# ForeverFancy/GVFDiffusion

Measured on AMD Instinct MI355X. Metric: 4D frames/sec (800x800x24f, 256k Gaussians) + DiT denoise steps/sec, higher is better.
Workload: dtype f32; 1 GPU; BASELINE configs[1]: single-GPU HIP rasteriser, one 4D sample per step = 24 frames x 800x800, 262144 Gaussians + per-frame deltas (fused activations), SH degree 2, mip 2D filter, white bg; gaussians=262144, resolution=800, sh_degree=2, parallelism=sample-sharded x1, samples_in_flight=2

## Files before the change

gvfdiffusion_amd/_lib.py:

```python
import ctypes
import os

_HERE = os.path.dirname(os.path.abspath(__file__))
LIB_PATH = os.path.join(_HERE, "libgvf_hip.so")

GVF_OK, GVF_EINVAL, GVF_ENOSPC, GVF_ELAUNCH = 0, -1, -2, -3
_ERR = {GVF_EINVAL: "GVF_EINVAL (bad argument)", GVF_ENOSPC: "GVF_ENOSPC (workspace too small)",
        GVF_ELAUNCH: "GVF_ELAUNCH (HIP launch/runtime failure)"}

RAST_MODE_MIP, RAST_MODE_DILATE = 0, 1
RAST_BIN_AUTO, RAST_BIN_RADIX, RAST_BIN_BUCKET = 0, 1, 2


class GvfError(RuntimeError):
    pass


class GvfRastFrame(ctypes.Structure):
    _fields_ = [("viewmatrix", ctypes.c_float * 16), ("projmatrix", ctypes.c_float * 16),
                ("campos", ctypes.c_float * 3), ("tanfovx", ctypes.c_float), ("tanfovy", ctypes.c_float),
                ("delta_index", ctypes.c_int32), ("reserved", ctypes.c_int32 * 2)]


class GvfRastSettings(ctypes.Structure):
    _fields_ = [("image_height", ctypes.c_int32), ("image_width", ctypes.c_int32), ("sh_degree", ctypes.c_int32),
                ("mode", ctypes.c_int32), ("kernel_size", ctypes.c_float), ("scale_modifier", ctypes.c_float),
                ("bg", ctypes.c_float * 3), ("prefiltered", ctypes.c_int32), ("debug", ctypes.c_int32),
                ("upstream_binning", ctypes.c_int32), ("bin_algo", ctypes.c_int32)]


class GvfGaussianActivation(ctypes.Structure):
    _fields_ = [("aabb", ctypes.c_float * 6), ("scale_bias", ctypes.c_float), ("opacity_bias", ctypes.c_float),
                ("min_kernel_size", ctypes.c_float), ("scaling_activation", ctypes.c_int32)]


class GvfRastPlan(ctypes.Structure):
    _fields_ = [(n, ctypes.c_int32) for n in ("bucket", "shared", "index_count", "morton", "slot_mode", "rec_gather", "wave_frames",
                                              "order_tiles", "upstream_binning", "n_slices", "layout", "gx", "gy", "ntiles", "nb", "nseg")] + \
               [(n, ctypes.c_int32 * 2) for n in ("pre_grid", "wf_grid", "bin_grid", "binx_grid")] + \
               [(n, ctypes.c_int32) for n in ("scan_blocks", "clear_blocks", "pre_lds_bytes", "wf_lds_bytes")]


_vp, _i, _i64, _sz, _f = ctypes.c_void_p, ctypes.c_int, ctypes.c_int64, ctypes.c_size_t, ctypes.c_float

SIGNATURES = {
    "gvf_version": (ctypes.c_char_p, []),
    "gvf_rast_workspace_bytes": (_i, [_i, _i, _i, _i, _i64, ctypes.POINTER(_sz)]),
    "gvf_rast_forward": (_i, [ctypes.POINTER(GvfRastSettings), ctypes.POINTER(GvfRastFrame), _i, _i,
                              _vp, _vp, _vp, _vp, _vp, _vp, _vp, _vp, _vp, _sz, _i64, _vp, _vp, _vp, _vp, _vp, _vp]),
    "gvf_rast_forward_batched": (_i, [ctypes.POINTER(GvfRastSettings), ctypes.POINTER(GvfRastFrame), _i,
                                      ctypes.POINTER(GvfGaussianActivation), _i, _i, _vp, _vp, _vp, _vp, _vp, _vp,
                                      _i, _vp, _sz, _i64, _vp, _vp, _vp, _vp, _vp, _vp]),
    "gvf_rast_forward_batched_u8": (_i, [ctypes.POINTER(GvfRastSettings), ctypes.POINTER(GvfRastFrame), _i,
                                         ctypes.POINTER(GvfGaussianActivation), _i, _i, _vp, _vp, _vp, _vp, _vp, _vp,
                                         _i, _vp, _sz, _i64, _vp, _vp, _vp]),
    "gvf_rast_backward_scratch_bytes": (_i, [_i, ctypes.POINTER(_sz)]),
    "gvf_rast_backward": (_i, [ctypes.POINTER(GvfRastSettings), ctypes.POINTER(GvfRastFrame), _i, _i,
                               _vp, _vp, _vp, _vp, _vp, _vp, _vp, _vp, _vp, _sz, _i64, _vp, _vp, _vp, _vp, _sz,
                               _vp, _vp, _vp, _vp, _vp, _vp, _vp, _vp, _vp]),
    "gvf_rast_backward_batched_scratch_bytes": (_i, [_i, _i, ctypes.POINTER(_sz)]),
    "gvf_rast_backward_batched": (_i, [ctypes.POINTER(GvfRastSettings), ctypes.POINTER(GvfRastFrame), _i,
                                       ctypes.POINTER(GvfGaussianActivation), _i, _i, _vp, _vp, _vp, _vp, _vp, _vp, _i,
                                       _vp, _sz, _i64, _vp, _vp, _vp, _vp, _sz, _vp, _vp, _vp, _vp, _vp, _vp, _vp]),
    "gvf_gaussian_activate": (_i, [ctypes.POINTER(GvfGaussianActivation), _i, _i, _vp, _vp, _vp, _vp, _vp, _vp,
                                   _vp, _vp, _vp, _vp, _vp, _vp]),
    "gvf_rgb_to_u8": (_i, [_vp, _vp, _i64, _vp]),
    "gvf_rast_sort_class_counts": (_i, [_vp, _sz, _i, _i, _i, _i, _i64, ctypes.POINTER(ctypes.c_uint32), _vp]),
    "gvf_rast_call_plan": (_i, [ctypes.POINTER(GvfRastSettings), ctypes.POINTER(GvfRastFrame), _i, _i, _i, _i, _i, _i, _i, _i, _i, _i64,
                                ctypes.POINTER(GvfRastPlan)]),
    "gvf_rast_bin_record_bytes": (_i, [ctypes.POINTER(GvfRastSettings), ctypes.POINTER(_i)]),
    "gvf_rast_slice_groups": (_i, [ctypes.POINTER(GvfRastFrame), _i, _i, _i, ctypes.POINTER(ctypes.c_int32), ctypes.POINTER(_i)]),
    "gvf_rast_profile_enable": (_i, [_i]),
    "gvf_rast_profile_read": (_i, [ctypes.POINTER(_f), ctypes.POINTER(_i)]),
    "gvf_rast_shared_activation_calls": (_i64, []),
    "gvf_sort_tmp_bytes": (_sz, [_i64]),
    "gvf_sort_pairs_u64": (_i, [_vp, _vp, _vp, _vp, _i64, _i, _vp, _sz, _vp]),
    "gvf_tile_sort_u64": (_i, [_vp, _vp, _i, _vp, _vp, _vp]),
}

_LIB = None


def register(signatures):
    SIGNATURES.update(signatures)
    if _LIB is not None:
        _bind(_LIB, signatures)


def _bind(lib, signatures):
    for name, (res, args) in signatures.items():
        fn = getattr(lib, name)
        fn.restype = res
        fn.argtypes = args


def lib():
    global _LIB
    if _LIB is None:
        if not os.path.exists(LIB_PATH):
            raise GvfError(f"{LIB_PATH} is missing: build it with `python -m gvfdiffusion_amd._build` "
                           "(hipcc, gfx950). There is no CPU fallback.")
        stamp = LIB_PATH + ".srchash"
        if os.path.exists(stamp) and os.environ.get("GVF_ALLOW_STALE_LIB") != "1":
            from . import _build
            if open(stamp).read().strip() != _build.source_hash():
                raise GvfError(f"{LIB_PATH} was built from different sources than the ones in csrc/ and include/: "
                               "rebuild with `python -m gvfdiffusion_amd._build`")
        import torch
        l = ctypes.CDLL(os.environ.get("GVF_LIB") or LIB_PATH)
        _bind(l, SIGNATURES)
        _LIB = l
    return _LIB


def check(rc: int, what: str):
    if rc != GVF_OK:
        raise GvfError(f"{what} failed: {_ERR.get(rc, rc)}")


def ptr(t):
    return None if t is None else ctypes.c_void_p(t.data_ptr())


def current_stream(device):
    import torch
    return ctypes.c_void_p(torch.cuda.current_stream(device).cuda_stream)


def require_cuda(*tensors):
    for t in tensors:
        if t is not None and not t.is_cuda:
            raise GvfError("gvfdiffusion_amd operators run on the MI355X only: got a CPU tensor "
                           "(there is no CPU fallback; the CPU oracle lives in oracle/ for tests)")
```

gvfdiffusion_amd/csrc/rast.hip:

```cpp
#include <atomic>
#include <cstdlib>
#include <vector>
#include "rast_common.h"
#include "gvf_sort.h"

namespace {

constexpr int PROF_MAX_CALLS = 256;
constexpr int PROF_EVENTS = GVF_RAST_NSTAGES + 1;
struct Profiler {
    bool on = false;
    std::atomic<int> calls{0};
    hipEvent_t ev[PROF_MAX_CALLS][PROF_EVENTS];
};
Profiler g_prof;
const hipEvent_t* prof_take_slot() {
    const int slot = g_prof.on ? g_prof.calls.fetch_add(1) : -1;
    return slot >= 0 && slot < PROF_MAX_CALLS ? g_prof.ev[slot] : nullptr;
}

std::atomic<long long> g_shared_calls{0};

bool switch_on(const char* name) {
    const char* v = getenv(name);
    return !(v && v[0] == '0');
}
RastSwitches switches_from_env() {
    RastSwitches sw;
    sw.shared_act = switch_on("GVF_RAST_SHARED_ACT");
    sw.slot_order = switch_on("GVF_RAST_SLOT_ORDER");
    sw.pre_wave_frames = switch_on("GVF_RAST_PRE_WAVE_FRAMES");
    sw.blend_order = switch_on("GVF_RAST_BLEND_ORDER");
    sw.bin_rec8 = switch_on("GVF_RAST_BIN_REC8");
    return sw;
}

int check_shape(const GvfRastSettings& st, int F, int P, int64_t max_rendered) {
    if (st.image_height <= 0 || st.image_width <= 0 || P < 0 || F <= 0 || max_rendered < 0 || max_rendered > 0xFFFFFFFFll) return GVF_EINVAL;
    if (st.sh_degree < 0 || st.sh_degree > 3) return GVF_EINVAL;
    if (st.mode != GVF_RAST_MODE_MIP && st.mode != GVF_RAST_MODE_DILATE) return GVF_EINVAL;
    return GVF_OK;
}

struct RastOutputs { float* color; float* alpha; float* depth; unsigned char* u8; };

int check_call(const RastCall& c, const RastOutputs& out, const void* workspace) {
    const GvfRastSettings& st = *c.st;
    if (check_shape(st, c.F, c.P, c.max_rendered) != GVF_OK) return GVF_EINVAL;
    if ((out.color == nullptr) == (out.u8 == nullptr) || !c.out_num_rendered || !c.frames_host || !workspace) return GVF_EINVAL;
    if (c.P > 0 && c.colors_precomp == nullptr) {
        if (c.sh == nullptr || c.M < (st.sh_degree + 1) * (st.sh_degree + 1) || c.M > MAX_SH_COEFFS) return GVF_EINVAL;
    }
    if ((((uintptr_t)c.sh) & 15) != 0 || (((uintptr_t)workspace) & 255) != 0) return GVF_EINVAL;
    return GVF_OK;
}

PlanInputs plan_inputs(const RastCall& c) {
    PlanInputs in;
    in.F = c.F; in.P = c.P; in.M = c.M; in.fused = c.fused;
    in.has_sh = c.sh != nullptr; in.has_colors_precomp = c.colors_precomp != nullptr; in.has_cov3D_precomp = c.cov3D_precomp != nullptr;
    in.has_delta = c.delta != nullptr; in.has_subpixel_offset = c.subpixel_offset != nullptr;
    in.max_rendered = c.max_rendered;
    return in;
}

int run_pipeline(const RastCall& c, void* workspace, size_t workspace_bytes, const RastOutputs& out, hipStream_t stream) {
    int rc = check_call(c, out, workspace);
    if (rc != GVF_OK) return rc;
    (void)hipGetLastError();
    const GvfRastSettings& st = *c.st;
    const Workspace w = carve(workspace, workspace_bytes, c.P, c.F, st.image_height, st.image_width, c.max_rendered);
    if (!w.ok) return GVF_ENOSPC;
    const RastPlan plan = plan_call(st, c.frames_host, plan_inputs(c), switches_from_env());
    const hipEvent_t* marks = prof_take_slot();
    if ((rc = upload_frames(stream, c, plan, w)) != GVF_OK) return rc;

    if (c.P == 0) {
        if (hipMemsetAsync(c.out_num_rendered, 0, sizeof(uint32_t) * c.F, stream) != hipSuccess) return GVF_ELAUNCH;
    } else {
        uint64_t* keys = w.keys;
        uint32_t* vals = nullptr;
        if (plan.shared) g_shared_calls.fetch_add(1, std::memory_order_relaxed);
        rc = plan.bucket ? front_end_bucket(stream, c, plan, w, marks) : front_end_radix(stream, c, plan, w, marks, &keys, &vals);
        if (rc != GVF_OK) return rc;
        if (c.max_rendered > 0 &&
            (rc = launch_tile_sort(stream, w.ranges, keys, vals, w.ids, w.cls, (uint32_t)plan.nseg, plan.bucket ? 2 : 1)) != GVF_OK)
            return rc;
    }
    rc = launch_blend(stream, st, c.P, c.F, w.ranges, w.ids, w.splats, c.subpixel_offset, out.color, out.alpha, out.depth, out.u8,
                      plan.slot_mode ? w.order_alt : nullptr, plan.order_tiles ? w.cursor : nullptr, marks != nullptr ? marks[6] : nullptr);
    if (rc != GVF_OK) return rc;
    prof_mark(stream, marks, 7);
    return GVF_OK;
}

int check_batched(const GvfRastSettings* st, const GvfRastFrame* frames_host, int F, const GvfGaussianActivation* act, int P,
                  const float* xyz_raw, const float* features_dc, const float* scaling_raw, const float* rotation_raw,
                  const float* opacity_raw, const float* delta, int n_delta) {
    if (!st || !frames_host || !act || F <= 0) return GVF_EINVAL;
    if (P > 0 && (!xyz_raw || !features_dc || !scaling_raw || !rotation_raw || !opacity_raw)) return GVF_EINVAL;
    if (act->scaling_activation != 0 && act->scaling_activation != 1) return GVF_EINVAL;
    for (int f = 0; f < F; ++f) {
        int di = frames_host[f].delta_index;
        if (di >= 0 && (delta == nullptr || di >= n_delta)) return GVF_EINVAL;
    }
    return GVF_OK;
}

}


Workspace gvf_rast::carve(void* ws, size_t bytes, int P, int F, int H, int W, int64_t max_rendered) {
    Workspace w;
    GvfCarver c(ws, bytes);
    const int nb = (P + PRE_THREADS - 1) / PRE_THREADS;
    const int ntiles = ((W + TILE - 1) / TILE) * ((H + TILE - 1) / TILE);
    const size_t FP = (size_t)F * (size_t)(P > 0 ? P : 1);
    const size_t D = (size_t)(max_rendered > 0 ? max_rendered : 1);
    w.frames = c.take<GvfRastFrame>(F);
    w.splats = c.take<float4>(4 * FP);
    w.tiles_touched = c.take<uint32_t>(FP);
    w.radii = c.take<int32_t>(FP);
    w.block_sums = c.take<uint32_t>((size_t)F * (nb > 0 ? nb : 1));
    w.frame_base = c.take<uint32_t>(F + 1);
    w.total = c.take<uint32_t>(1);
    w.keys = c.take<uint64_t>(D);
    w.keys_alt = c.take<uint64_t>(D);
    w.vals = c.take<uint32_t>(D);
    w.vals_alt = c.take<uint32_t>(D);
    w.ids = c.take<uint32_t>(D);
    w.ranges = c.take<uint2>((size_t)F * ntiles);
    w.cls = c.take<uint32_t>(2 + 2 * (size_t)F * ntiles);
    w.tile_count = c.take<uint32_t>((size_t)F * ntiles);
    w.cursor = c.take<uint32_t>((size_t)F * ntiles);
    w.partial = c.take<uint32_t>(((size_t)F * ntiles + SCAN_CHUNK - 1) / SCAN_CHUNK + 1);
    const size_t Pp = (size_t)(P > 0 ? P : 1);
    w.order = c.take<uint32_t>(Pp);
    w.order_alt = c.take<uint32_t>(Pp);
    w.mhist = c.take<uint32_t>(MORTON_BINS);
    w.mm = c.take<uint32_t>(8);
    w.binrec = c.take<uint4>(FP);
    w.sort_tmp_bytes = gvf_sort_tmp_bytes((int64_t)D);
    w.sort_tmp = c.take<char>(w.sort_tmp_bytes);
    w.bytes = gvf_align_up(c.off, 256);
    w.ok = c.ok;
    return w;
}

extern "C" int gvf_rast_workspace_bytes(int P, int F, int H, int W, int64_t max_rendered, size_t* bytes) {
    if (!bytes || P < 0 || F <= 0 || H <= 0 || W <= 0 || max_rendered < 0) return GVF_EINVAL;
    Workspace w = carve(nullptr, (size_t)-1, P, F, H, W, max_rendered);
    *bytes = w.bytes + 256;
    (void)tile_sort_set_lds_limit();
    return GVF_OK;
}

extern "C" int gvf_rast_forward(const GvfRastSettings* st, const GvfRastFrame* frame_host, int P, int M,
                                const float* means3D, const float* shs, const float* colors_precomp,
                                const float* opacities, const float* scales, const float* rotations,
                                const float* cov3D_precomp, const float* subpixel_offset, void* workspace,
                                size_t workspace_bytes, int64_t max_rendered, float* out_color, float* out_alpha,
                                float* out_depth, int32_t* out_radii, uint32_t* out_num_rendered, void* stream) {
    if (!st || !frame_host) return GVF_EINVAL;
    if (P > 0) {
        if (!means3D || !opacities) return GVF_EINVAL;
        if ((shs == nullptr) == (colors_precomp == nullptr)) return GVF_EINVAL;
        const bool have_sr = scales != nullptr && rotations != nullptr;
        if (have_sr == (cov3D_precomp != nullptr)) return GVF_EINVAL;
    }
    const RastCall c = {st, frame_host, 1, P, M, false, nullptr, means3D, scales, rotations, opacities, shs, colors_precomp, cov3D_precomp,
                        nullptr, 0, subpixel_offset, max_rendered, out_radii, out_num_rendered};
    return run_pipeline(c, workspace, workspace_bytes, {out_color, out_alpha, out_depth, nullptr}, (hipStream_t)stream);
}

extern "C" int gvf_rast_forward_batched(const GvfRastSettings* st, const GvfRastFrame* frames_host, int F,
                                        const GvfGaussianActivation* act, int P, int M, const float* xyz_raw,
                                        const float* features_dc, const float* scaling_raw,
                                        const float* rotation_raw, const float* opacity_raw, const float* delta,
                                        int n_delta, void* workspace, size_t workspace_bytes,
                                        int64_t max_rendered, float* out_color, float* out_alpha, float* out_depth,
                                        int32_t* out_radii, uint32_t* out_num_rendered, void* stream) {
    const int rc = check_batched(st, frames_host, F, act, P, xyz_raw, features_dc, scaling_raw, rotation_raw, opacity_raw, delta, n_delta);
    if (rc != GVF_OK) return rc;
    const RastCall c = {st, frames_host, F, P, M, true, act, xyz_raw, scaling_raw, rotation_raw, opacity_raw, features_dc, nullptr, nullptr,
                        delta, n_delta, nullptr, max_rendered, out_radii, out_num_rendered};
    return run_pipeline(c, workspace, workspace_bytes, {out_color, out_alpha, out_depth, nullptr}, (hipStream_t)stream);
}

extern "C" int gvf_rast_forward_batched_u8(const GvfRastSettings* st, const GvfRastFrame* frames_host, int F,
                                           const GvfGaussianActivation* act, int P, int M, const float* xyz_raw,
                                           const float* features_dc, const float* scaling_raw,
                                           const float* rotation_raw, const float* opacity_raw, const float* delta,
                                           int n_delta, void* workspace, size_t workspace_bytes,
                                           int64_t max_rendered, uint8_t* out_rgb_u8, uint32_t* out_num_rendered, void* stream) {
    if (!out_rgb_u8) return GVF_EINVAL;
    const int rc = check_batched(st, frames_host, F, act, P, xyz_raw, features_dc, scaling_raw, rotation_raw, opacity_raw, delta, n_delta);
    if (rc != GVF_OK) return rc;
    const RastCall c = {st, frames_host, F, P, M, true, act, xyz_raw, scaling_raw, rotation_raw, opacity_raw, features_dc, nullptr, nullptr,
                        delta, n_delta, nullptr, max_rendered, nullptr, out_num_rendered};
    return run_pipeline(c, workspace, workspace_bytes, {nullptr, nullptr, nullptr, out_rgb_u8}, (hipStream_t)stream);
}

extern "C" int gvf_rast_call_plan(const GvfRastSettings* st, const GvfRastFrame* frames_host, int F, int P, int M, int fused, int has_sh,
                                  int has_colors_precomp, int has_cov3D_precomp, int has_delta, int has_subpixel_offset,
                                  int64_t max_rendered, GvfRastPlan* out) {
    if (!st || !frames_host || !out || M < 0) return GVF_EINVAL;
    if (check_shape(*st, F, P, max_rendered) != GVF_OK) return GVF_EINVAL;
    PlanInputs in;
    in.F = F; in.P = P; in.M = M; in.fused = fused != 0;
    in.has_sh = has_sh != 0; in.has_colors_precomp = has_colors_precomp != 0; in.has_cov3D_precomp = has_cov3D_precomp != 0;
    in.has_delta = has_delta != 0; in.has_subpixel_offset = has_subpixel_offset != 0;
    in.max_rendered = max_rendered;
    *out = plan_call(*st, frames_host, in, switches_from_env());
    return GVF_OK;
}

extern "C" int gvf_rast_bin_record_bytes(const GvfRastSettings* st, int* bytes) {
    if (!st || !bytes) return GVF_EINVAL;
    if (check_shape(*st, 1, 0, 0) != GVF_OK) return GVF_EINVAL;
    const GvfRastFrame frame = {};
    PlanInputs in = {};
    in.F = 1;
    *bytes = plan_call(*st, &frame, in, switches_from_env()).rec8 ? 8 : 16;
    return GVF_OK;
}

extern "C" int gvf_rast_slice_groups(const GvfRastFrame* frames_host, int F, int has_delta, int max_slices, int32_t* table_host,
                                     int* n_slices) {
    if (!frames_host || !table_host || !n_slices || F <= 0) return GVF_EINVAL;
    std::vector<int32_t> slices, frame_slice;
    if (!group_slices(frames_host, F, has_delta != 0, max_slices, slices, frame_slice)) return GVF_ENOSPC;
    const std::vector<int32_t> tab = slice_table(slices, frame_slice);
    for (size_t k = 0; k < tab.size(); ++k) table_host[k] = tab[k];
    *n_slices = (int)slices.size();
    return GVF_OK;
}

extern "C" int gvf_rast_profile_enable(int on) {
    if (on && !g_prof.on) {
        for (int c = 0; c < PROF_MAX_CALLS; ++c)
            for (int k = 0; k < PROF_EVENTS; ++k)
                if (hipEventCreate(&g_prof.ev[c][k]) != hipSuccess) return GVF_ELAUNCH;
        g_prof.on = true;
        g_prof.calls = 0;
    } else if (!on && g_prof.on) {
        for (int c = 0; c < PROF_MAX_CALLS; ++c)
            for (int k = 0; k < PROF_EVENTS; ++k) (void)hipEventDestroy(g_prof.ev[c][k]);
        g_prof.on = false;
        g_prof.calls = 0;
    }
    return GVF_OK;
}

extern "C" int64_t gvf_rast_shared_activation_calls(void) { return (int64_t)g_shared_calls.load(std::memory_order_relaxed); }

extern "C" int gvf_rast_profile_read(float* ms_sum, int* calls) {
    if (!ms_sum || !calls) return GVF_EINVAL;
    for (int k = 0; k < GVF_RAST_NSTAGES; ++k) ms_sum[k] = 0.f;
    *calls = 0;
    if (!g_prof.on) return GVF_OK;
    const int n_calls = g_prof.calls.load() < PROF_MAX_CALLS ? g_prof.calls.load() : PROF_MAX_CALLS;
    for (int c = 0; c < n_calls; ++c) {
        if (hipEventSynchronize(g_prof.ev[c][PROF_EVENTS - 1]) != hipSuccess) return GVF_ELAUNCH;
        for (int k = 0; k < GVF_RAST_NSTAGES; ++k) {
            float ms = 0.f;
            if (hipEventElapsedTime(&ms, g_prof.ev[c][k], g_prof.ev[c][k + 1]) != hipSuccess) return GVF_ELAUNCH;
            ms_sum[k] += ms;
        }
    }
    *calls = n_calls;
    g_prof.calls = 0;
    return GVF_OK;
}

extern "C" int gvf_rast_sort_class_counts(const void* workspace, size_t workspace_bytes, int P, int F, int H, int W, int64_t max_rendered,
                                          uint32_t* counts_host, void* stream) {
    if (!workspace || !counts_host || H <= 0 || W <= 0 || P < 0 || F <= 0 || max_rendered < 0) return GVF_EINVAL;
    if ((((uintptr_t)workspace) & 255) != 0) return GVF_EINVAL;
    Workspace w = carve(const_cast<void*>(workspace), workspace_bytes, P, F, H, W, max_rendered);
    if (!w.ok) return GVF_ENOSPC;
    if (hipMemcpyAsync(counts_host, w.cls, 2 * sizeof(uint32_t), hipMemcpyDeviceToHost, (hipStream_t)stream) != hipSuccess) return GVF_ELAUNCH;
    if (hipStreamSynchronize((hipStream_t)stream) != hipSuccess) return GVF_ELAUNCH;
    return GVF_OK;
}

extern "C" const char* gvf_version(void) { return "gvf_hip 0.1.0 gfx950"; }
```

gvfdiffusion_amd/csrc/rast_blend.hip:

```cpp
#include "rast_common.h"

namespace {


__global__ __launch_bounds__(1024) void blend_order_kernel(const uint2* __restrict__ ranges, int ntiles, uint32_t* __restrict__ order) {
    __shared__ uint32_t hist[64];
    const int f = blockIdx.x, t = threadIdx.x;
    const uint2* r = ranges + (size_t)f * ntiles;
    if (t < 64) hist[t] = 0u;
    __syncthreads();
    for (int tile = t; tile < ntiles; tile += 1024) {
        const uint32_t n = r[tile].y - r[tile].x;
        atomicAdd(&hist[63u - min(63u, n >> 5)], 1u);
    }
    __syncthreads();
    const bool reorder = hist[0] != 0u;
    __syncthreads();
    if (!reorder) {
        for (int tile = t; tile < ntiles; tile += 1024) order[(size_t)f * ntiles + tile] = (uint32_t)tile;
        return;
    }
    if (t == 0) {
        uint32_t run = 0u;
        for (int c = 0; c < 64; ++c) { const uint32_t h = hist[c]; hist[c] = run; run += h; }
    }
    __syncthreads();
    for (int tile = t; tile < ntiles; tile += 1024) {
        const uint32_t n = r[tile].y - r[tile].x;
        order[(size_t)f * ntiles + atomicAdd(&hist[63u - min(63u, n >> 5)], 1u)] = (uint32_t)tile;
    }
}

#ifdef BLEND_TIMING
__device__ unsigned long long* g_blend_buf;
__device__ unsigned long long g_blend_cap;
extern "C" int gvf_debug_blend_timing(unsigned long long* device_buf, unsigned long long rows) {
    if (hipMemcpyToSymbol(HIP_SYMBOL(g_blend_buf), &device_buf, sizeof(device_buf)) != hipSuccess) return 1;
    if (hipMemcpyToSymbol(HIP_SYMBOL(g_blend_cap), &rows, sizeof(rows)) != hipSuccess) return 1;
    return 0;
}
#define BT_DECL unsigned long long bt_acc[12] = {}; unsigned long long bt_last = __builtin_amdgcn_s_memtime(); const unsigned long long bt_first = bt_last;
#define BT(i) do { const unsigned long long n_ = __builtin_amdgcn_s_memtime(); bt_acc[i] += n_ - bt_last; bt_last = n_; } while (0)
#define BT_VMWAIT() asm volatile("s_waitcnt vmcnt(0)" ::: "memory")
#else
#define BT_DECL
#define BT(i) do { } while (0)
#define BT_VMWAIT() do { } while (0)
#endif

#ifdef BLEND_CONSUMED
__device__ unsigned long long g_blend_cons[4][5];
extern "C" int gvf_debug_blend_consumed(unsigned long long* out12, int reset) {
    if (out12 && hipMemcpyFromSymbol(out12, HIP_SYMBOL(g_blend_cons), sizeof(g_blend_cons)) != hipSuccess) return 1;
    if (reset) { unsigned long long z[20] = {}; if (hipMemcpyToSymbol(HIP_SYMBOL(g_blend_cons), z, sizeof(z)) != hipSuccess) return 1; }
    return 0;
}
#endif


template <bool DEPTH>
__global__ __launch_bounds__(BLEND_THREADS) void blend_kernel(
    int P, int H, int W, int gx, int gy, float bg0, float bg1, float bg2, const uint2* __restrict__ ranges,
    const uint32_t* __restrict__ point_list, const float4* __restrict__ splats,
    const float* __restrict__ subpixel_offset, float* __restrict__ out_color,
    float* __restrict__ out_alpha, float* __restrict__ out_depth,
    const uint32_t* __restrict__ tile_order ,
    const uint32_t* __restrict__ rec_of ,
    unsigned char* __restrict__ out_u8 ) {
    __shared__ float4 sA[BLEND_THREADS];
    __shared__ float4 sB[BLEND_THREADS];
    __shared__ float4 sC[BLEND_THREADS];
    __shared__ unsigned char sMask[BLEND_THREADS];
    __shared__ unsigned sList[4][BLEND_THREADS];

    const int t = threadIdx.x, lane = t & 63, wave = t >> 6;
    const int f = blockIdx.y;
    const int tile = tile_order != nullptr ? (int)tile_order[(size_t)f * gridDim.x + blockIdx.x] : (int)blockIdx.x;
    const int tx = tile % gx, ty = tile / gx;
    const int px = tx * TILE + (wave & 1) * 8 + (lane & 7), py = ty * TILE + (wave >> 1) * 8 + (lane >> 3);
    const bool inside = px < W && py < H;
    const size_t pid = (size_t)py * W + px;
    float pxf = (float)px, pyf = (float)py;
    if (subpixel_offset != nullptr && inside) { pxf += subpixel_offset[2 * pid]; pyf += subpixel_offset[2 * pid + 1]; }

    const uint2 rng = ranges[(size_t)f * gx * gy + tile];
    const size_t gbase = (size_t)f * P;
    const int rounds = (int)((rng.y - rng.x + BLEND_THREADS - 1) / BLEND_THREADS);
    int todo = (int)(rng.y - rng.x);
    const uint64_t lt_mask = (1ull << lane) - 1ull;

    const float pxr = pxf - (float)(tx * TILE), pyr = pyf - (float)(ty * TILE);
    unsigned long long done_m = __builtin_amdgcn_ballot_w64(!inside);
    float T = 1.0f, C0 = 0.f, C1 = 0.f, C2 = 0.f, Dacc = 0.f;

    BT_DECL
#ifdef BLEND_CONSUMED
    int rounds_done = rounds;
#endif
    for (int r = 0; r < rounds; ++r, todo -= BLEND_THREADS) {
        BT(6);
#ifdef BLEND_CONSUMED
        if (r > 0 && __syncthreads_and(done_m == ~0ull)) { rounds_done = r; break; }
#else
        if (r > 0 && __syncthreads_and(done_m == ~0ull)) break;
#endif
        BT(0);
#ifdef BLEND_TIMING
        uint32_t id_ = 0;
        if (t < todo) id_ = point_list[rng.x + (uint32_t)r * BLEND_THREADS + t];
        if (t < todo && rec_of != nullptr) id_ = rec_of[id_];
        BT_VMWAIT(); BT(1);
        float4 a_ = {}, b_ = {}, c_ = {};
        if (t < todo) { const float4* rec = splats + 4 * (gbase + id_); a_ = rec[0]; c_ = rec[2]; b_ = rec[1]; }
        BT_VMWAIT(); BT(2);
        bt_acc[7] += 1;
#endif
        if (t < todo) {
#ifdef BLEND_TIMING
            const float4 a = a_, b = b_, c = c_;
#else
            uint32_t id = point_list[rng.x + (uint32_t)r * BLEND_THREADS + t];
            if (rec_of != nullptr) id = rec_of[id];
            const float4* rec = splats + 4 * (gbase + id);
            const float4 a = rec[0];
            const float4 c = rec[2];
            const float4 b = rec[1];
#endif
            const SplatChol ch = splat_cholesky(a.x, a.y, a.z, a.w, b.x, (float)(tx * TILE), (float)(ty * TILE));
            sA[t] = make_float4(ch.l11, ch.l12, ch.l22, ch.c1);
            sB[t] = make_float4(ch.c2, ch.ok ? __builtin_amdgcn_logf(b.y) : -__builtin_inff(), b.z, b.w);
            sC[t] = make_float4(c.x, c.y, 0.f, 0.f);
            sMask[t] = (unsigned char)quadrant_mask(a.x, a.y, a.z, a.w, b.x, b.y, c.z, (float)(tx * TILE), (float)(ty * TILE), subpixel_offset != nullptr);
#ifdef BLEND_CONSUMED
            {
                const unsigned n_ = rng.y - rng.x;
                const int cls_ = n_ <= 2048u ? 0 : n_ <= 4096u ? 1 : n_ <= 16384u ? 2 : 3;
                if (sMask[t] == 0) atomicAdd(&g_blend_cons[cls_][3], 1ull);
                atomicAdd(&g_blend_cons[cls_][4], (unsigned long long)__popc((unsigned)sMask[t]));
            }
#endif
        }
        BT(3);
        __syncthreads();
        BT(4);
        const int cnt = min(BLEND_THREADS, todo);
        if (done_m == ~0ull) continue;
        int n_w = 0;
#pragma unroll
        for (int k = 0; k < BLEND_THREADS / GVF_WAVE; ++k) {
            const int idx = k * GVF_WAVE + lane;
            const bool hit = idx < cnt && ((sMask[idx] >> wave) & 1u);
            const uint64_t bal = __ballot(hit);
            if (hit) sList[wave][n_w + __popcll(bal & lt_mask)] = (unsigned)idx * 16u;
            n_w += __popcll(bal);
        }
        __builtin_amdgcn_wave_barrier();
        BT(5);
#ifdef BLEND_TIMING
        bt_acc[8] += n_w;
#endif
#define GVF_BLEND_STEP(J)                                                                              \
        {                                                                                              \
            const float4 a = *reinterpret_cast<const float4*>(reinterpret_cast<const unsigned char*>(sA) + (J));          \
            const float4 b = *reinterpret_cast<const float4*>(reinterpret_cast<const unsigned char*>(sB) + (J));          \
            const float4 c4_ = *reinterpret_cast<const float4*>(reinterpret_cast<const unsigned char*>(sC) + (J));        \
            const float2 c = DEPTH ? make_float2(c4_.x, c4_.y) : make_float2(c4_.x, 0.f);              \
            const float nlog = splat_neg_exponent(a.x, a.y, a.z, a.w, b.x, pxr, pyr, b.y);    \
            const float alpha = fminf(0.99f, __builtin_amdgcn_exp2f(-nlog));                           \
            const float w_raw = alpha * T;                                                             \
            const float test_T = T - w_raw;         \
                              \
            const unsigned long long ok_m = __builtin_amdgcn_ballot_w64(!(alpha < 1.0f / 255.0f)) & ~done_m;   \
            const unsigned long long stop_m = ok_m & __builtin_amdgcn_ballot_w64(test_T < 0.0001f);    \
            done_m |= stop_m;                                                                          \
            const bool acc = __builtin_amdgcn_inverse_ballot_w64(ok_m ^ stop_m);                       \
            const float wgt = acc ? w_raw : 0.0f;                                                      \
            C0 = __builtin_fmaf(b.z, wgt, C0);                                                         \
            C1 = __builtin_fmaf(b.w, wgt, C1);                                                         \
            C2 = __builtin_fmaf(c.x, wgt, C2);                                                         \
            if (DEPTH) Dacc = __builtin_fmaf(c.y, wgt, Dacc);                                          \
            T = acc ? test_T : T;                                                                      \
        }
        int jj = 0;
        for (; jj + 3 < n_w; jj += 4) {
            if (done_m == ~0ull) break;
            const unsigned j0 = sList[wave][jj], j1 = sList[wave][jj + 1], j2 = sList[wave][jj + 2], j3 = sList[wave][jj + 3];
            GVF_BLEND_STEP(j0)
            GVF_BLEND_STEP(j1)
            __builtin_amdgcn_sched_barrier(0);
            GVF_BLEND_STEP(j2)
            GVF_BLEND_STEP(j3)
        }
        for (; jj < n_w; ++jj) {
            if (done_m == ~0ull) break;
            const unsigned j0 = sList[wave][jj];
            GVF_BLEND_STEP(j0)
        }
#undef GVF_BLEND_STEP
    }
#ifdef BLEND_CONSUMED
    if (t == 0) {
        const unsigned n = rng.y - rng.x, used = min(n, (unsigned)rounds_done * BLEND_THREADS);
        const int cls = n <= 2048u ? 0 : n <= 4096u ? 1 : n <= 16384u ? 2 : 3;
        atomicAdd(&g_blend_cons[cls][0], 1ull); atomicAdd(&g_blend_cons[cls][1], (unsigned long long)n); atomicAdd(&g_blend_cons[cls][2], (unsigned long long)used);
    }
#endif
    if (inside) {
        const size_t hw = (size_t)H * W;
        const float r0 = __builtin_fmaf(T, bg0, C0), r1 = __builtin_fmaf(T, bg1, C1), r2 = __builtin_fmaf(T, bg2, C2);
        if (out_u8 != nullptr) {
            unsigned char* ob = out_u8 + (size_t)f * 3 * hw;
            ob[0 * hw + pid] = (unsigned char)(fminf(fmaxf(r0, 0.f), 1.f) * 255.0f);
            ob[1 * hw + pid] = (unsigned char)(fminf(fmaxf(r1, 0.f), 1.f) * 255.0f);
            ob[2 * hw + pid] = (unsigned char)(fminf(fmaxf(r2, 0.f), 1.f) * 255.0f);
        } else {
            float* oc = out_color + (size_t)f * 3 * hw;
            oc[0 * hw + pid] = r0;
            oc[1 * hw + pid] = r1;
            oc[2 * hw + pid] = r2;
        }
        if (out_alpha != nullptr) out_alpha[(size_t)f * hw + pid] = 1.0f - T;
        if (out_depth != nullptr) out_depth[(size_t)f * hw + pid] = Dacc;
    }
#ifdef BLEND_TIMING
    BT(6);
    BT_VMWAIT(); BT(11);
    bt_acc[9] = 1; bt_acc[10] = bt_last - bt_first;
    const unsigned long long wid = ((unsigned long long)f * gridDim.x + tile) * 4 + wave;
    if (lane == 0 && g_blend_buf != nullptr && wid < g_blend_cap)
        for (int i = 0; i < 12; ++i) g_blend_buf[wid * 12 + i] = bt_acc[i];
#endif
}

__global__ __launch_bounds__(256) void rgb_to_u8_kernel(const float4* __restrict__ src, uchar4* __restrict__ dst,
                                                        long long n4, const float* __restrict__ tail_src,
                                                        unsigned char* __restrict__ tail_dst, int tail) {
    for (long long i = blockIdx.x * (long long)blockDim.x + threadIdx.x; i < n4; i += (long long)gridDim.x * blockDim.x) {
        const float4 v = src[i];
        uchar4 o;
        o.x = (unsigned char)(fminf(fmaxf(v.x, 0.f), 1.f) * 255.0f);
        o.y = (unsigned char)(fminf(fmaxf(v.y, 0.f), 1.f) * 255.0f);
        o.z = (unsigned char)(fminf(fmaxf(v.z, 0.f), 1.f) * 255.0f);
        o.w = (unsigned char)(fminf(fmaxf(v.w, 0.f), 1.f) * 255.0f);
        dst[i] = o;
    }
    if (blockIdx.x == 0 && (int)threadIdx.x < tail)
        tail_dst[threadIdx.x] = (unsigned char)(fminf(fmaxf(tail_src[threadIdx.x], 0.f), 1.f) * 255.0f);
}

}

int gvf_rast::launch_blend(hipStream_t stream, const GvfRastSettings& st, int P, int F, const uint2* ranges, const uint32_t* point_list,
                           const float4* splats, const float* subpixel_offset, float* out_color, float* out_alpha, float* out_depth,
                           unsigned char* out_u8, const uint32_t* rec_of, uint32_t* tile_order, hipEvent_t ordered) {
    const int H = st.image_height, W = st.image_width;
    const int gx = (W + TILE - 1) / TILE, gy = (H + TILE - 1) / TILE, ntiles = gx * gy;
    if (tile_order != nullptr) hipLaunchKernelGGL(blend_order_kernel, dim3(F), dim3(1024), 0, stream, ranges, ntiles, tile_order);
    if (ordered != nullptr) (void)hipEventRecord(ordered, stream);
    hipLaunchKernelGGL(out_depth != nullptr ? blend_kernel<true> : blend_kernel<false>, dim3(ntiles, F), dim3(BLEND_THREADS), 0, stream, P, H, W,
                       gx, gy, st.bg[0], st.bg[1], st.bg[2], ranges, point_list, splats, subpixel_offset, out_color, out_alpha, out_depth,
                       tile_order, rec_of, out_u8);
    GVF_CHECK_LAUNCH();
    return GVF_OK;
}

extern "C" int gvf_rgb_to_u8(const float* rgb, uint8_t* out, int64_t n, void* stream) {
    if (n < 0) return GVF_EINVAL;
    if (n == 0) return GVF_OK;
    if (!rgb || !out || (((uintptr_t)rgb) & 15) || (((uintptr_t)out) & 3)) return GVF_EINVAL;
    (void)hipGetLastError();
    const long long n4 = n / 4;
    long long blocks = (n4 + 255) / 256;
    if (blocks < 1) blocks = 1;
    if (blocks > 8192) blocks = 8192;
    hipLaunchKernelGGL(rgb_to_u8_kernel, dim3((unsigned)blocks), dim3(256), 0, (hipStream_t)stream,
                       reinterpret_cast<const float4*>(rgb), reinterpret_cast<uchar4*>(out), n4, rgb + n4 * 4,
                       out + n4 * 4, (int)(n - n4 * 4));
    GVF_CHECK_LAUNCH();
    return GVF_OK;
}
```

gvfdiffusion_amd/csrc/rast_common.h:

```cpp
#pragma once
#include "gvf_common.h"
#include "../../include/gvf_rast.h"
#include "rast_plan.h"
using namespace gvf_rast;
static_assert(WAVE == GVF_WAVE, "rast_plan.h sizes its grids for this wave width");

namespace {

constexpr int BLEND_THREADS = TILE * TILE;
constexpr int MAX_SH_COEFFS = 16;
constexpr float CONIC_K1 = -0.7213475204444817f;
constexpr float CONIC_K2 = -1.4426950408889634f;
constexpr float CONIC_IK1 = -1.3862943611198906f;
constexpr float CONIC_IK2 = -0.6931471805599453f;
struct SplatChol { float l11, l12, l22, c1, c2; bool ok; };
__device__ __forceinline__ SplatChol splat_cholesky(float x, float y, float ap, float bp, float cp, float tile_x0, float tile_y0) {
    SplatChol r;
    const float m11 = -ap, m12 = -0.5f * bp, m22 = -cp;
    const float il = __builtin_amdgcn_rsqf(m11);
    r.l11 = m11 * il;
    r.l12 = m12 * il;
    const float d = m22 - r.l12 * r.l12;
    r.l22 = __builtin_amdgcn_sqrtf(d);
    r.ok = m11 > 0.0f && d > 0.0f && m11 < __builtin_inff() && d < __builtin_inff();
    if (!r.ok) { r.l11 = 0.f; r.l12 = 0.f; r.l22 = 0.f; }
    const float xr = x - tile_x0, yr = y - tile_y0;
    r.c1 = r.ok ? __builtin_fmaf(r.l11, xr, r.l12 * yr) : 0.f;
    r.c2 = r.ok ? r.l22 * yr : 0.f;
    return r;
}
__device__ __forceinline__ float splat_neg_exponent(float l11, float l12, float l22, float c1, float c2, float px, float py, float lo = 0.0f) {
    const float s1 = __builtin_fmaf(-l11, px, __builtin_fmaf(-l12, py, c1));
    const float s2 = __builtin_fmaf(-l22, py, c2);
    return __builtin_fmaf(s2, s2, __builtin_fmaf(s1, s1, -lo));
}

__constant__ float SH_C0 = 0.28209479177387814f;
__constant__ float SH_C1 = 0.4886025119029199f;
__constant__ float SH_C2[5] = {1.0925484305920792f, -1.0925484305920792f, 0.31539156525252005f,
                               -1.0925484305920792f, 0.5462742152960396f};
__constant__ float SH_C3[7] = {-0.5900435899266435f, 2.890611442640554f, -0.4570457994644658f,
                               0.3731763325901154f, -0.4570457994644658f, 1.445305721320277f,
                               -0.5900435899266435f};

__device__ __forceinline__ float act_expf(float x) {
    if (x != x) return x;
    if (x > 88.72283f) return __builtin_inff();
    if (x < -103.97208f) return 0.0f;
    const float kf = x * 1.44269502f + (x < 0.0f ? -0.5f : 0.5f);
    const int k = (int)kf;
    const float t = (float)k;
    float r = __builtin_fmaf(t, -0.693145751953125f, x);
    r = __builtin_fmaf(t, -1.42860677e-6f, r);
    float p = 1.98412698e-4f;
    p = __builtin_fmaf(p, r, 1.38888889e-3f);
    p = __builtin_fmaf(p, r, 8.33333377e-3f);
    p = __builtin_fmaf(p, r, 4.16666679e-2f);
    p = __builtin_fmaf(p, r, 1.66666672e-1f);
    p = __builtin_fmaf(p, r, 0.5f);
    p = __builtin_fmaf(p, r, 1.0f);
    p = __builtin_fmaf(p, r, 1.0f);
    const int k1 = k / 2, k2 = k - k1;
    return (p * __uint_as_float((uint32_t)(k1 + 127) << 23)) * __uint_as_float((uint32_t)(k2 + 127) << 23);
}
__device__ __forceinline__ float act_log1pf(float y) {
    if (!(y >= 5.9604645e-8f)) return y;
    if (y > 3.4028235e38f) return y;
    int k = 0;
    float c = 0.0f, f = y;
    if (y >= 0.41421354f) {
        const float u = 1.0f + y;
        uint32_t iu = __float_as_uint(u) + (0x3f800000u - 0x3f3504f3u);
        k = (int)(iu >> 23) - 127;
        if (k < 25) c = (k >= 2 ? 1.0f - (u - y) : y - (u - 1.0f)) / u;
        iu = (iu & 0x007fffffu) + 0x3f3504f3u;
        f = __uint_as_float(iu) - 1.0f;
    }
    const float s = f / (2.0f + f);
    const float z = s * s, w = z * z;
    const float t1 = w * (0.40000972152f + w * 0.24279078841f);
    const float t2 = z * (0.66666662693f + w * 0.28498786688f);
    const float R = t2 + t1;
    const float hfsq = (0.5f * f) * f;
    const float dk = (float)k;
    float acc = s * (hfsq + R);
    acc = acc + (dk * 9.0580006145e-6f + c);
    acc = acc - hfsq;
    acc = acc + f;
    return acc + dk * 6.9313812256e-1f;
}
__device__ __forceinline__ float act_scale(float x, const GvfGaussianActivation& a) {
    float s = a.scaling_activation == 0 ? act_expf(x) : (x > 20.0f ? x : act_log1pf(act_expf(x)));
    return sqrtf(s * s + a.min_kernel_size * a.min_kernel_size);
}

struct ActGaussian {
    float p[3], s[3], q[4], op, drgb[3];
};

struct ActRaw {
    float p[3], s[3], q[4], op;
};
__device__ __forceinline__ ActRaw activate_raw(int i, const GvfGaussianActivation& a,
                                               const float* __restrict__ xyz_raw,
                                               const float* __restrict__ scaling_raw,
                                               const float* __restrict__ rotation_raw,
                                               const float* __restrict__ opacity_raw) {
    ActRaw r;
#pragma unroll
    for (int k = 0; k < 3; ++k) r.p[k] = xyz_raw[3 * (size_t)i + k] * a.aabb[3 + k] + a.aabb[k];
#pragma unroll
    for (int k = 0; k < 3; ++k) r.s[k] = scaling_raw[3 * (size_t)i + k] + a.scale_bias;
#pragma unroll
    for (int k = 0; k < 4; ++k) r.q[k] = rotation_raw[4 * (size_t)i + k] + (k == 0 ? 1.0f : 0.0f);
    r.op = opacity_raw[i] + a.opacity_bias;
    return r;
}
__device__ __forceinline__ ActGaussian activate_finish(const ActRaw& r, const GvfGaussianActivation& a, const float (&dl)[14], bool d) {
    ActGaussian g;
#pragma unroll
    for (int k = 0; k < 3; ++k) g.p[k] = d ? r.p[k] + dl[k] : r.p[k];
#pragma unroll
    for (int k = 0; k < 3; ++k) {
        float x = r.s[k];
        if (d) x = x + dl[3 + k];
        g.s[k] = act_scale(x, a);
    }
    float q[4];
#pragma unroll
    for (int k = 0; k < 4; ++k) {
        q[k] = r.q[k];
        if (d) q[k] = q[k] + dl[6 + k];
    }
    float n = sqrtf(q[0] * q[0] + q[1] * q[1] + q[2] * q[2] + q[3] * q[3]);
    n = fmaxf(n, 1e-12f);
#pragma unroll
    for (int k = 0; k < 4; ++k) g.q[k] = q[k] / n;
    float x = r.op;
    if (d) x = x + dl[13];
    g.op = 1.0f / (1.0f + act_expf(-x));
    g.drgb[0] = dl[10]; g.drgb[1] = dl[11]; g.drgb[2] = dl[12];
    return g;
}
__device__ __forceinline__ ActGaussian activate_vals(int i, const GvfGaussianActivation& a,
                                                     const float* __restrict__ xyz_raw,
                                                     const float* __restrict__ scaling_raw,
                                                     const float* __restrict__ rotation_raw,
                                                     const float* __restrict__ opacity_raw,
                                                     const float (&dl)[14], bool d) {
    return activate_finish(activate_raw(i, a, xyz_raw, scaling_raw, rotation_raw, opacity_raw), a, dl, d);
}
__device__ __forceinline__ ActGaussian activate_one(int i, const GvfGaussianActivation& a,
                                                    const float* __restrict__ xyz_raw,
                                                    const float* __restrict__ scaling_raw,
                                                    const float* __restrict__ rotation_raw,
                                                    const float* __restrict__ opacity_raw,
                                                    const float* __restrict__ d ) {
    float dl[14];
#pragma unroll
    for (int k = 0; k < 14; ++k) dl[k] = d ? d[k] : 0.0f;
    return activate_vals(i, a, xyz_raw, scaling_raw, rotation_raw, opacity_raw, dl, d != nullptr);
}

__device__ __forceinline__ void xform43(const float* m, const float* p, float* o) {
    o[0] = m[0] * p[0] + m[4] * p[1] + m[8] * p[2] + m[12];
    o[1] = m[1] * p[0] + m[5] * p[1] + m[9] * p[2] + m[13];
    o[2] = m[2] * p[0] + m[6] * p[1] + m[10] * p[2] + m[14];
}
__device__ __forceinline__ void xform44(const float* m, const float* p, float* o) {
    o[0] = m[0] * p[0] + m[4] * p[1] + m[8] * p[2] + m[12];
    o[1] = m[1] * p[0] + m[5] * p[1] + m[9] * p[2] + m[13];
    o[2] = m[2] * p[0] + m[6] * p[1] + m[10] * p[2] + m[14];
    o[3] = m[3] * p[0] + m[7] * p[1] + m[11] * p[2] + m[15];
}

__device__ __forceinline__ void cov3d_from_scale_rot(const float* s, float mod, const float* q, float* c6) {
    float sx = mod * s[0], sy = mod * s[1], sz = mod * s[2];
    float r = q[0], x = q[1], y = q[2], z = q[3];
    float R00 = 1.f - 2.f * (y * y + z * z), R01 = 2.f * (x * y - r * z), R02 = 2.f * (x * z + r * y);
    float R10 = 2.f * (x * y + r * z), R11 = 1.f - 2.f * (x * x + z * z), R12 = 2.f * (y * z - r * x);
    float R20 = 2.f * (x * z - r * y), R21 = 2.f * (y * z + r * x), R22 = 1.f - 2.f * (x * x + y * y);
    float L00 = R00 * sx, L01 = R01 * sy, L02 = R02 * sz;
    float L10 = R10 * sx, L11 = R11 * sy, L12 = R12 * sz;
    float L20 = R20 * sx, L21 = R21 * sy, L22 = R22 * sz;
    c6[0] = L00 * L00 + L01 * L01 + L02 * L02;
    c6[1] = L00 * L10 + L01 * L11 + L02 * L12;
    c6[2] = L00 * L20 + L01 * L21 + L02 * L22;
    c6[3] = L10 * L10 + L11 * L11 + L12 * L12;
    c6[4] = L10 * L20 + L11 * L21 + L12 * L22;
    c6[5] = L20 * L20 + L21 * L21 + L22 * L22;
}

__device__ __forceinline__ void sh_to_rgb(int deg, const float* sh, const float* dadd, const float* p,
                                          const float* cam, float* rgb) {
    float dx = p[0] - cam[0], dy = p[1] - cam[1], dz = p[2] - cam[2];
    float len = sqrtf(dx * dx + dy * dy + dz * dz);
    float x = dx / len, y = dy / len, z = dz / len;
#pragma unroll
    for (int c = 0; c < 3; ++c) {
        const float da = dadd[c];
        float res = SH_C0 * (sh[0 * 3 + c] + da);
        if (deg > 0) {
            res = res - SH_C1 * y * (sh[1 * 3 + c] + da) + SH_C1 * z * (sh[2 * 3 + c] + da) -
                  SH_C1 * x * (sh[3 * 3 + c] + da);
            if (deg > 1) {
                float xx = x * x, yy = y * y, zz = z * z, xy = x * y, yz = y * z, xz = x * z;
                res = res + SH_C2[0] * xy * (sh[4 * 3 + c] + da) + SH_C2[1] * yz * (sh[5 * 3 + c] + da) +
                      SH_C2[2] * (2.0f * zz - xx - yy) * (sh[6 * 3 + c] + da) +
                      SH_C2[3] * xz * (sh[7 * 3 + c] + da) + SH_C2[4] * (xx - yy) * (sh[8 * 3 + c] + da);
                if (deg > 2) {
                    res = res + SH_C3[0] * y * (3.0f * xx - yy) * (sh[9 * 3 + c] + da) +
                          SH_C3[1] * xy * z * (sh[10 * 3 + c] + da) +
                          SH_C3[2] * y * (4.0f * zz - xx - yy) * (sh[11 * 3 + c] + da) +
                          SH_C3[3] * z * (2.0f * zz - 3.0f * xx - 3.0f * yy) * (sh[12 * 3 + c] + da) +
                          SH_C3[4] * x * (4.0f * zz - xx - yy) * (sh[13 * 3 + c] + da) +
                          SH_C3[5] * z * (xx - yy) * (sh[14 * 3 + c] + da) +
                          SH_C3[6] * x * (xx - 3.0f * yy) * (sh[15 * 3 + c] + da);
                }
            }
        }
        res += 0.5f;
        rgb[c] = res < 0.f ? 0.f : res;
    }
}

struct TileRect { int x0, y0, x1, y1; };
__device__ __forceinline__ TileRect get_rect(float px, float py, float radius, int gx, int gy) {
    TileRect r;
    r.x0 = min(gx, max(0, (int)((px - radius) / (float)TILE)));
    r.y0 = min(gy, max(0, (int)((py - radius) / (float)TILE)));
    r.x1 = min(gx, max(0, (int)((px + radius + (float)(TILE - 1)) / (float)TILE)));
    r.y1 = min(gy, max(0, (int)((py + radius + (float)(TILE - 1)) / (float)TILE)));
    return r;
}

#ifndef GVF_SORT_SMALL_N
#define GVF_SORT_SMALL_N 1536
#endif
constexpr int SORT_SMALL_N = GVF_SORT_SMALL_N;
static_assert(SORT_SMALL_N == 1536 || SORT_SMALL_N == 2048, "register class of the per-tile sort: 6 or 8 keys per thread");
constexpr int SORT_LARGE_N = 16384;
constexpr int SORT_LARGE_BLOCKS = 256, SORT_HUGE_BLOCKS = 64;
constexpr int SORT_MEDIUM_N = 4096, SORT_MEDIUM_BLOCKS = 768;

__device__ __forceinline__ float edge_max(float qa, float qb, float qc, float kv, float fixed, float lo, float hi) {
    const float t = fminf(fmaxf(kv * fixed, lo), hi);
    return __builtin_fmaf(__builtin_fmaf(qc, t, qb * fixed), t, (qa * fixed) * fixed);
}
__device__ __forceinline__ unsigned quadrant_mask(float x, float y, float ap, float bp, float cp, float op, float hx,
                                                  float tile_x0, float tile_y0, bool no_cull) {
    if (hx < 0.0f) return 0u;
    if (no_cull || !(hx < __builtin_inff())) return 0xFu;
    const float lim = -(__log2f(255.0f * op) + 0.02f);
    const float kx = -0.5f * bp * __builtin_amdgcn_rcpf(cp), ky = -0.5f * bp * __builtin_amdgcn_rcpf(ap);
    const float xr = x - tile_x0, yr = y - tile_y0;
    unsigned m = 0u;
#pragma unroll
    for (int q = 0; q < 4; ++q) {
        const float ox = (float)((q & 1) * 8), oy = (float)((q >> 1) * 8);
        const float dxl = xr - (ox + 7.0f), dxh = xr - ox, dyl = yr - (oy + 7.0f), dyh = yr - oy;
        const bool inside = dxl <= 0.0f && dxh >= 0.0f && dyl <= 0.0f && dyh >= 0.0f;
        float e = edge_max(ap, bp, cp, kx, dxl, dyl, dyh);
        e = fmaxf(e, edge_max(ap, bp, cp, kx, dxh, dyl, dyh));
        e = fmaxf(e, edge_max(cp, bp, ap, ky, dyl, dxl, dxh));
        e = fmaxf(e, edge_max(cp, bp, ap, ky, dyh, dxl, dxh));
        m |= (inside || e >= lim) ? (1u << q) : 0u;
    }
    return m;
}

constexpr int BWD_ACC = 10;

}

namespace gvf_rast {

struct Workspace {
    GvfRastFrame* frames;
    float4* splats;
    uint32_t* tiles_touched; int32_t* radii;
    uint32_t* block_sums; uint32_t* frame_base; uint32_t* total;
    uint64_t* keys; uint64_t* keys_alt; uint32_t* vals; uint32_t* vals_alt; uint32_t* ids;
    uint2* ranges; uint32_t* cls;
    uint32_t* tile_count; uint32_t* cursor;
    uint32_t* partial;
    uint32_t* order; uint32_t* order_alt; uint32_t* mhist; uint32_t* mm;
    uint4* binrec;
    void* sort_tmp; size_t sort_tmp_bytes;
    size_t bytes; bool ok;
};

Workspace carve(void* ws, size_t bytes, int P, int F, int H, int W, int64_t max_rendered);

struct RastCall {
    const GvfRastSettings* st; const GvfRastFrame* frames_host; int F, P, M;
    bool fused; const GvfGaussianActivation* act;
    const float *a0, *a1, *a2, *a3, *sh, *colors_precomp, *cov3D_precomp, *delta; int n_delta;
    const float* subpixel_offset;
    int64_t max_rendered;
    int32_t* out_radii; uint32_t* out_num_rendered;
};

inline void prof_mark(hipStream_t s, const hipEvent_t* marks, int k) {
    if (marks != nullptr) (void)hipEventRecord(marks[k], s);
}

int upload_frames(hipStream_t stream, const RastCall& c, const RastPlan& plan, const Workspace& w);
int front_end_bucket(hipStream_t stream, const RastCall& c, const RastPlan& plan, const Workspace& w, const hipEvent_t* marks);
int front_end_radix(hipStream_t stream, const RastCall& c, const RastPlan& plan, const Workspace& w, const hipEvent_t* marks,
                    uint64_t** keys_sorted, uint32_t** vals_by_tile);

int launch_tile_sort(hipStream_t stream, const uint2* ranges, uint64_t* keys, const uint32_t* vals, uint32_t* ids, uint32_t* cls,
                     uint32_t nseg, int cls_state);
int tile_sort_set_lds_limit();

int launch_blend(hipStream_t stream, const GvfRastSettings& st, int P, int F, const uint2* ranges, const uint32_t* point_list,
                 const float4* splats, const float* subpixel_offset, float* out_color, float* out_alpha, float* out_depth,
                 unsigned char* out_u8, const uint32_t* rec_of, uint32_t* tile_order, hipEvent_t ordered);
}
using namespace gvf_rast;
```

gvfdiffusion_amd/csrc/rast_front.hip:

```cpp
#include "rast_common.h"
#include "gvf_sort.h"

namespace {


struct PreParams {
    int P, M, deg, H, W, mode;
    int gx, gy;
    float kernel_size, scale_modifier;
    int fused;
    GvfGaussianActivation act;
    int n_delta;
    int upstream_binning;
    int F;
    int delta_lds;
};

__global__ __launch_bounds__(256) void activate_kernel(GvfGaussianActivation a, int P, int M,
                                                       const float* __restrict__ xyz_raw,
                                                       const float* __restrict__ features_dc,
                                                       const float* __restrict__ scaling_raw,
                                                       const float* __restrict__ rotation_raw,
                                                       const float* __restrict__ opacity_raw,
                                                       const float* __restrict__ delta, float* __restrict__ means3D,
                                                       float* __restrict__ scales, float* __restrict__ rotations,
                                                       float* __restrict__ shs, float* __restrict__ opacities) {
    int i = blockIdx.x * blockDim.x + threadIdx.x;
    if (i >= P) return;
    const float* d = delta ? delta + 14 * (size_t)i : nullptr;
    ActGaussian g = activate_one(i, a, xyz_raw, scaling_raw, rotation_raw, opacity_raw, d);
    for (int k = 0; k < 3; ++k) { means3D[3 * (size_t)i + k] = g.p[k]; scales[3 * (size_t)i + k] = g.s[k]; }
    for (int k = 0; k < 4; ++k) rotations[4 * (size_t)i + k] = g.q[k];
    opacities[i] = g.op;
    for (int m = 0; m < M; ++m)
        for (int c = 0; c < 3; ++c) {
            float v = features_dc[((size_t)i * M + m) * 3 + c];
            shs[((size_t)i * M + m) * 3 + c] = d ? v + g.drgb[c] : v;
        }
}

struct ActSlices { int n; int di[ACT_MAX_SLICES]; };
__global__ __launch_bounds__(256) void activate_cov_kernel(GvfGaussianActivation a, float scale_modifier, int P, ActSlices sl,
                                                           const float* __restrict__ xyz_raw, const float* __restrict__ scaling_raw,
                                                           const float* __restrict__ rotation_raw, const float* __restrict__ opacity_raw,
                                                           const float* __restrict__ delta, float4* __restrict__ rec3d,
                                                           const uint32_t* __restrict__ slot_of ,
                                                           const float* __restrict__ sh, int sh_floats, float* __restrict__ sh_by_slot) {
    const int i = blockIdx.x * blockDim.x + threadIdx.x;
    if (i >= P) return;
    const size_t dst = slot_of != nullptr ? (size_t)slot_of[i] : (size_t)i;
    if (sh_by_slot != nullptr && blockIdx.y == 0)
        for (int k = 0; k < sh_floats; ++k) sh_by_slot[dst * sh_floats + k] = sh[(size_t)i * sh_floats + k];
    const int di = sl.di[blockIdx.y];
    const float* d = (delta != nullptr && di >= 0) ? delta + ((size_t)di * P + i) * 14 : nullptr;
    const ActGaussian g = activate_one(i, a, xyz_raw, scaling_raw, rotation_raw, opacity_raw, d);
    float c6[6];
    cov3d_from_scale_rot(g.s, scale_modifier, g.q, c6);
    float4* r = rec3d + 4 * ((size_t)blockIdx.y * P + dst);
    r[0] = make_float4(g.p[0], g.p[1], g.p[2], g.op);
    r[1] = make_float4(c6[0], c6[1], c6[2], c6[3]);
    r[2] = make_float4(c6[4], c6[5], g.drgb[0], g.drgb[1]);
    r[3] = make_float4(g.drgb[2], 0.f, 0.f, 0.f);
}

__device__ __forceinline__ float ln_upper(float z) {
    const uint32_t b = __float_as_uint(z);
    const int e = (int)(b >> 23) - 127;
    const float m = __uint_as_float((b & 0x7fffffu) | 0x3f800000u);
    float L = (m - 1.0f) * 1.4426951f;
    L = fminf(L, 0.32192809f + (m - 1.25f) * 1.1541561f);
    L = fminf(L, 0.5849625f + (m - 1.5f) * 0.96179669f);
    L = fminf(L, 0.80735492f + (m - 1.75f) * 0.8243972f);
    L = fminf(L, 1.0f + (m - 2.0f) * 0.72134752f);
    return ((float)e + (L + 1e-5f)) * 0.69314724f;
}

__device__ __forceinline__ float2 cull_extent(float ca, float cb, float cc, float op) {
    if (op < 1.0f / 255.0f) return make_float2(-1.0f, -1.0f);
    const float det = ca * cc - cb * cb;
    const float inf = __builtin_inff();
    if (!(det > 0.0f) || !(ca > 0.0f) || !(cc > 0.0f)) return make_float2(inf, inf);
    const float tau = 2.0f * ln_upper(255.0f * op) * 1.001f + 1e-3f;
    const float inv = 1.0f / det;
    return make_float2(sqrtf(tau * cc * inv) * 1.001f + 0.01f, sqrtf(tau * ca * inv) * 1.001f + 0.01f);
}

__device__ __forceinline__ void tight_range(float c, float h, int lo, int hi, int n, int& t0, int& t1) {
    if (h < 0.0f) { t0 = lo; t1 = lo; return; }
    const float a = fminf(fmaxf(ceilf((c - h - (float)(TILE - 1)) / (float)TILE), 0.0f), (float)n);
    const float b = fminf(fmaxf(floorf((c + h) / (float)TILE) + 1.0f, 0.0f), (float)n);
    t0 = max((int)a, lo);
    t1 = min((int)b, hi);
    if (t1 < t0) t1 = t0;
}

__device__ __forceinline__ TileRect tight_rect(TileRect r, float px, float py, float hx, float hy, int gx, int gy) {
    TileRect t;
    tight_range(px, hx, r.x0, r.x1, gx, t.x0, t.x1);
    tight_range(py, hy, r.y0, r.y1, gy, t.y0, t.y1);
    return t;
}

typedef uint4 BinRec16;
typedef uint2 BinRec8;
template <typename REC> __device__ __forceinline__ REC binrec_pack(TileRect r, uint32_t depth_bits);
template <> __device__ __forceinline__ BinRec16 binrec_pack<BinRec16>(TileRect r, uint32_t depth_bits) {
    return make_uint4((uint32_t)r.x0 | ((uint32_t)r.y0 << 16), (uint32_t)r.x1 | ((uint32_t)r.y1 << 16), depth_bits, 0u);
}
template <> __device__ __forceinline__ BinRec8 binrec_pack<BinRec8>(TileRect r, uint32_t depth_bits) {
    return make_uint2((uint32_t)r.x0 | ((uint32_t)r.y0 << 8) | ((uint32_t)r.x1 << 16) | ((uint32_t)r.y1 << 24), depth_bits);
}
__device__ __forceinline__ TileRect binrec_rect16(uint32_t w0, uint32_t w1) {
    return TileRect{(int)(w0 & 0xffffu), (int)(w0 >> 16), (int)(w1 & 0xffffu), (int)(w1 >> 16)};
}
__device__ __forceinline__ TileRect binrec_rect8(uint32_t w) {
    return TileRect{(int)(w & 0xffu), (int)((w >> 8) & 0xffu), (int)((w >> 16) & 0xffu), (int)(w >> 24)};
}
__device__ __forceinline__ TileRect binrec_rect(const BinRec16& b) { return binrec_rect16(b.x, b.y); }
__device__ __forceinline__ TileRect binrec_rect(const BinRec8& b) { return binrec_rect8(b.x); }
__device__ __forceinline__ uint32_t binrec_depth(const BinRec16& b) { return b.z; }
__device__ __forceinline__ uint32_t binrec_depth(const BinRec8& b) { return b.y; }

template <bool SHARED, bool WAVE_FRAMES = false, typename REC = BinRec16>
__global__ __launch_bounds__(PRE_THREADS) void preprocess_kernel(
    PreParams pp, const GvfRastFrame* __restrict__ frames, const float* __restrict__ a0,
    const float* __restrict__ a1, const float* __restrict__ a2, const float* __restrict__ a3,
    const float* __restrict__ sh, const float* __restrict__ colors_precomp,
    const float* __restrict__ cov3D_precomp, const float* __restrict__ delta, float4* __restrict__ splats,
    uint32_t* __restrict__ tiles_touched,
    int32_t* __restrict__ radii, uint32_t* __restrict__ block_sums, REC* __restrict__ binrec,
    const uint32_t* __restrict__ bin_slot ) {
    static_assert(!(SHARED && WAVE_FRAMES), "the shared-activation launch keeps the 256-Gaussian mapping");
    extern __shared__ __attribute__((aligned(16))) float sh_lds[];
    constexpr int PRE_GPB = WAVE_FRAMES ? GVF_WAVE : PRE_THREADS;
    const int t = threadIdx.x;
    const int P = pp.P, M = pp.M;
    const int nbx = (P + PRE_THREADS - 1) / PRE_THREADS;
    const int bx = blockIdx.x, by = blockIdx.y;
    const int row = WAVE_FRAMES ? (t & (GVF_WAVE - 1)) : t;
    const int i = bx * PRE_GPB + row;

    const int sh_stride = M * 3;
    if (sh != nullptr) {
        const size_t span0 = (size_t)bx * PRE_GPB * sh_stride;
        const int nvalid = min(PRE_GPB, P - bx * PRE_GPB);
        const int total = nvalid * sh_stride;
        const float4* src4 = reinterpret_cast<const float4*>(sh + span0);
        float4* dst4 = reinterpret_cast<float4*>(sh_lds);
        const int n4 = total >> 2;
        for (int k = t; k < n4; k += PRE_THREADS) dst4[k] = src4[k];
        for (int k = (n4 << 2) + t; k < total; k += PRE_THREADS) sh_lds[k] = sh[span0 + k];
    }
    __syncthreads();

  const uint32_t my_slot = (bin_slot != nullptr && i < P) ? bin_slot[i] : (uint32_t)i;
  ActRaw raw = {};
  if (WAVE_FRAMES && pp.fused && i < P) raw = activate_raw(i, pp.act, a0, a1, a2, a3);
  const int f_first = WAVE_FRAMES ? by * (PRE_WAVES * PRE_WAVE_FB) + __builtin_amdgcn_readfirstlane(t >> 6) : by * PRE_FB;
  constexpr int F_STEP = WAVE_FRAMES ? PRE_WAVES : 1, F_COUNT = WAVE_FRAMES ? PRE_WAVE_FB : PRE_FB;
#pragma unroll 1
  for (int ff = 0; ff < F_COUNT; ++ff) {
    const int f = f_first + ff * F_STEP;
    if (f >= pp.F) break;
    const GvfRastFrame* fr = frames + f;
    uint32_t touched = 0;
    int radius_out = 0;
    float4 gA = make_float4(0.f, 0.f, 0.f, 0.f), gB = gA, gC = gA;
    TileRect rect = {0, 0, 0, 0};

    if (i < P) {
        float p[3], s[3], q[4], op, dadd[3] = {0.f, 0.f, 0.f};
        float c6s[6];
        if (SHARED) {
            const float4* r3 = reinterpret_cast<const float4*>(a0) + 4 * ((size_t)fr->reserved[0] * P + i);
            const float4 r0 = r3[0], r1 = r3[1], r2 = r3[2], r3v = r3[3];
            p[0] = r0.x; p[1] = r0.y; p[2] = r0.z; op = r0.w;
            c6s[0] = r1.x; c6s[1] = r1.y; c6s[2] = r1.z; c6s[3] = r1.w; c6s[4] = r2.x; c6s[5] = r2.y;
            dadd[0] = r2.z; dadd[1] = r2.w; dadd[2] = r3v.x;
        } else if (pp.fused) {
            const int di = fr->delta_index;
            const float* d = (delta != nullptr && di >= 0) ? delta + ((size_t)di * P + i) * 14 : nullptr;
            ActGaussian g;
            if (WAVE_FRAMES) {
                float dl[14];
#pragma unroll
                for (int k = 0; k < 14; ++k) dl[k] = d ? d[k] : 0.0f;
                g = activate_finish(raw, pp.act, dl, d != nullptr);
            } else {
                g = activate_one(i, pp.act, a0, a1, a2, a3, d);
            }
#pragma unroll
            for (int k = 0; k < 3; ++k) { p[k] = g.p[k]; s[k] = g.s[k]; dadd[k] = g.drgb[k]; }
#pragma unroll
            for (int k = 0; k < 4; ++k) q[k] = g.q[k];
            op = g.op;
        } else {
#pragma unroll
            for (int k = 0; k < 3; ++k) p[k] = a0[3 * (size_t)i + k];
            if (cov3D_precomp == nullptr) {
#pragma unroll
                for (int k = 0; k < 3; ++k) s[k] = a1[3 * (size_t)i + k];
#pragma unroll
                for (int k = 0; k < 4; ++k) q[k] = a2[4 * (size_t)i + k];
            }
            op = a3[i];
        }

        float pv[3];
        xform43(fr->viewmatrix, p, pv);
        bool vis = pv[2] > 0.2f;
        if (vis) {
            float ph[4];
            xform44(fr->projmatrix, p, ph);
            float pw = 1.0f / (ph[3] + 0.0000001f);
            float projx = ph[0] * pw, projy = ph[1] * pw;

            float c6[6];
            if (SHARED) {
#pragma unroll
                for (int k = 0; k < 6; ++k) c6[k] = c6s[k];
            } else if (!pp.fused && cov3D_precomp != nullptr) {
#pragma unroll
                for (int k = 0; k < 6; ++k) c6[k] = cov3D_precomp[6 * (size_t)i + k];
            } else {
                cov3d_from_scale_rot(s, pp.scale_modifier, q, c6);
            }

            const float tanfovx = fr->tanfovx, tanfovy = fr->tanfovy;
            float focal_x = (float)pp.W / (2.0f * tanfovx);
            float focal_y = (float)pp.H / (2.0f * tanfovy);
            float limx = 1.3f * tanfovx, limy = 1.3f * tanfovy;
            float txtz = pv[0] / pv[2], tytz = pv[1] / pv[2];
            float tx = fminf(limx, fmaxf(-limx, txtz)) * pv[2];
            float ty = fminf(limy, fmaxf(-limy, tytz)) * pv[2];
            float tz = pv[2];
            float J00 = focal_x / tz, J02 = -(focal_x * tx) / (tz * tz);
            float J11 = focal_y / tz, J12 = -(focal_y * ty) / (tz * tz);
            float A0[3], A1[3];
#pragma unroll
            for (int c = 0; c < 3; ++c) {
                float w0 = fr->viewmatrix[c * 4 + 0], w1 = fr->viewmatrix[c * 4 + 1], w2 = fr->viewmatrix[c * 4 + 2];
                A0[c] = J00 * w0 + J02 * w2;
                A1[c] = J11 * w1 + J12 * w2;
            }
            float S[3][3] = {{c6[0], c6[1], c6[2]}, {c6[1], c6[3], c6[4]}, {c6[2], c6[4], c6[5]}};
            float B0[3], B1[3];
#pragma unroll
            for (int c = 0; c < 3; ++c) {
                B0[c] = A0[0] * S[0][c] + A0[1] * S[1][c] + A0[2] * S[2][c];
                B1[c] = A1[0] * S[0][c] + A1[1] * S[1][c] + A1[2] * S[2][c];
            }
            float cxx = B0[0] * A0[0] + B0[1] * A0[1] + B0[2] * A0[2];
            float cxy = B0[0] * A1[0] + B0[1] * A1[1] + B0[2] * A1[2];
            float cyy = B1[0] * A1[0] + B1[1] * A1[1] + B1[2] * A1[2];

            float coef = 1.0f;
            if (pp.mode == GVF_RAST_MODE_MIP) {
                float det0 = fmaxf(1e-6f, cxx * cyy - cxy * cxy);
                float det1 = fmaxf(1e-6f, (cxx + pp.kernel_size) * (cyy + pp.kernel_size) - cxy * cxy);
                coef = sqrtf(det0 / (det1 + 1e-6f) + 1e-6f);
                if (det0 <= 1e-6f || det1 <= 1e-6f) coef = 0.0f;
                cxx += pp.kernel_size;
                cyy += pp.kernel_size;
            } else {
                cxx += 0.3f;
                cyy += 0.3f;
            }
            float det = cxx * cyy - cxy * cxy;
            if (det != 0.0f) {
                float det_inv = 1.f / det;
                float ca = cyy * det_inv, cb = -cxy * det_inv, cc = cxx * det_inv;
                float mid = 0.5f * (cxx + cyy);
                float lam1 = mid + sqrtf(fmaxf(0.1f, mid * mid - det));
                float lam2 = mid - sqrtf(fmaxf(0.1f, mid * mid - det));
                float my_radius = ceilf(3.f * sqrtf(fmaxf(lam1, lam2)));
                float px = ((projx + 1.0f) * (float)pp.W - 1.0f) * 0.5f;
                float py = ((projy + 1.0f) * (float)pp.H - 1.0f) * 0.5f;
                TileRect r = get_rect(px, py, my_radius, pp.gx, pp.gy);
                uint32_t cnt = (uint32_t)((r.x1 - r.x0) * (r.y1 - r.y0));
                if (cnt != 0) {
                    float rgb[3];
                    if (colors_precomp != nullptr) {
                        rgb[0] = colors_precomp[3 * (size_t)i + 0];
                        rgb[1] = colors_precomp[3 * (size_t)i + 1];
                        rgb[2] = colors_precomp[3 * (size_t)i + 2];
                    } else {
                        sh_to_rgb(pp.deg, sh_lds + row * sh_stride, dadd, p, fr->campos, rgb);
                    }
                    radius_out = (int)my_radius;
                    const float2 ext = cull_extent(ca, cb, cc, op * coef);
                    if (!pp.upstream_binning) {
                        r = tight_rect(r, px, py, ext.x, ext.y, pp.gx, pp.gy);
                        cnt = (uint32_t)((r.x1 - r.x0) * (r.y1 - r.y0));
                    }
                    touched = cnt;
                    rect = r;
                    gA = make_float4(px, py, ca * CONIC_K1, cb * CONIC_K2);
                    gB = make_float4(cc * CONIC_K1, op * coef, rgb[0], rgb[1]);
                    gC = make_float4(rgb[2], pv[2], ext.x, ext.y);
                }
            }
        }
        const size_t o = (size_t)f * P + i;
        if (!WAVE_FRAMES && tiles_touched != nullptr) tiles_touched[o] = touched;
        if (radii != nullptr) {
            const uint32_t* gid_of = SHARED ? reinterpret_cast<const uint32_t*>(a1) : nullptr;
            radii[gid_of != nullptr ? (size_t)f * P + gid_of[i] : o] = radius_out;
        }
        if (binrec != nullptr) binrec[(size_t)f * P + my_slot] = binrec_pack<REC>(rect, __float_as_uint(gC.y));
    }

    const int lj = t & 3;
    float4* qbase = splats + 4 * ((size_t)f * P + (size_t)(i & ~3));
#define GVF_QB(v_, k_) __builtin_bit_cast(float, __builtin_amdgcn_mov_dpp(__builtin_bit_cast(int, (v_)), (k_) * 0x55, 0xF, 0xF, true))
#define GVF_QSTORE(k_)                                                                                          \
    {                                                                                                       \
        const int tk = __builtin_amdgcn_mov_dpp((int)touched, (k_) * 0x55, 0xF, 0xF, true);                 \
        float4 o4;                                                                                          \
        { const float a = GVF_QB(gA.x, k_), b = GVF_QB(gB.x, k_), c = GVF_QB(gC.x, k_); o4.x = lj == 0 ? a : (lj == 1 ? b : (lj == 2 ? c : 0.f)); } \
        { const float a = GVF_QB(gA.y, k_), b = GVF_QB(gB.y, k_), c = GVF_QB(gC.y, k_); o4.y = lj == 0 ? a : (lj == 1 ? b : (lj == 2 ? c : 0.f)); } \
        { const float a = GVF_QB(gA.z, k_), b = GVF_QB(gB.z, k_), c = GVF_QB(gC.z, k_); o4.z = lj == 0 ? a : (lj == 1 ? b : (lj == 2 ? c : 0.f)); } \
        { const float a = GVF_QB(gA.w, k_), b = GVF_QB(gB.w, k_), c = GVF_QB(gC.w, k_); o4.w = lj == 0 ? a : (lj == 1 ? b : (lj == 2 ? c : 0.f)); } \
        if (tk != 0) qbase[4 * (k_) + lj] = o4;                                                             \
    }
    GVF_QSTORE(0) GVF_QSTORE(1) GVF_QSTORE(2) GVF_QSTORE(3)
#undef GVF_QSTORE
#undef GVF_QB

    if (!WAVE_FRAMES && block_sums != nullptr) {
        const unsigned lane = t & 63, w = t >> 6;
        uint32_t incl = gvf_wave_incl_scan(touched, lane);
        __shared__ uint32_t wsum[PRE_THREADS / GVF_WAVE];
        __syncthreads();
        if (lane == 63) wsum[w] = incl;
        __syncthreads();
        if (t == 0) block_sums[(size_t)f * nbx + bx] = wsum[0] + wsum[1] + wsum[2] + wsum[3];
    }
  }
}

__global__ __launch_bounds__(1024) void scan_sums_kernel(uint32_t* __restrict__ block_sums, int nb, int F,
                                                         uint32_t* __restrict__ frame_base ,
                                                         uint32_t* __restrict__ num_rendered ,
                                                         uint32_t* __restrict__ total_out, uint32_t max_rendered) {
    __shared__ uint32_t wsum[16];
    __shared__ uint32_t carry_s;
    const int t = threadIdx.x;
    const unsigned lane = t & 63, w = t >> 6;
    const int n = nb * F;
    if (t == 0) carry_s = 0;
    __syncthreads();
    for (int base = 0; base < n; base += 1024) {
        int j = base + t;
        uint32_t v = j < n ? block_sums[j] : 0u;
        uint32_t incl = gvf_wave_incl_scan(v, lane);
        if (lane == 63) wsum[w] = incl;
        __syncthreads();
        uint32_t wbase = 0, tot = 0;
        for (unsigned k = 0; k < 16; ++k) { if (k < w) wbase += wsum[k]; tot += wsum[k]; }
        uint32_t carry = carry_s;
        uint32_t excl = carry + wbase + incl - v;
        if (j < n) {
            block_sums[j] = excl;
            if (j % nb == 0) frame_base[j / nb] = excl;
        }
        __syncthreads();
        if (t == 0) carry_s = carry + tot;
        __syncthreads();
    }
    if (t == 0) { frame_base[F] = carry_s; *total_out = carry_s > max_rendered ? 0u : carry_s; }
    __syncthreads();
    for (int f = t; f < F; f += 1024) num_rendered[f] = frame_base[f + 1] - frame_base[f];
}

__global__ __launch_bounds__(PRE_THREADS) void duplicate_kernel(
    int P, int gx, int gy, const float4* __restrict__ splats,
    const uint32_t* __restrict__ tiles_touched, const int32_t* __restrict__ radii_ws,
    const uint32_t* __restrict__ block_base, uint64_t* __restrict__ keys, uint32_t* __restrict__ vals,
    uint32_t max_rendered, int upstream_binning) {
    __shared__ uint32_t wsum[PRE_THREADS / GVF_WAVE];
    const int t = threadIdx.x, f = blockIdx.y;
    const int i = blockIdx.x * PRE_THREADS + t;
    const unsigned lane = t & 63, w = t >> 6;
    const size_t o = (size_t)f * P + i;
    uint32_t touched = i < P ? tiles_touched[o] : 0u;
    uint32_t incl = gvf_wave_incl_scan(touched, lane);
    if (lane == 63) wsum[w] = incl;
    __syncthreads();
    uint32_t wbase = 0;
    for (unsigned k = 0; k < w; ++k) wbase += wsum[k];
    uint32_t off = block_base[(size_t)f * gridDim.x + blockIdx.x] + wbase + incl - touched;
    if (touched == 0) return;
    if ((uint64_t)off + touched > (uint64_t)max_rendered) return;
    const float4 a = splats[4 * o];
    const float4 c = splats[4 * o + 2];
    const float depth = c.y;
    TileRect r = get_rect(a.x, a.y, (float)radii_ws[o], gx, gy);
    if (!upstream_binning) r = tight_rect(r, a.x, a.y, c.z, c.w, gx, gy);
    const uint64_t tile0 = (uint64_t)f * (uint32_t)(gx * gy);
    const uint32_t dbits = __float_as_uint(depth);
    for (int y = r.y0; y < r.y1; ++y)
        for (int x = r.x0; x < r.x1; ++x) {
            uint64_t key = ((tile0 + (uint32_t)(y * gx + x)) << 32) | dbits;
            keys[off] = key;
            vals[off] = (uint32_t)i;
            ++off;
        }
}

__device__ __forceinline__ uint32_t float_ordered(float f) {
    const uint32_t u = __float_as_uint(f);
    return (u & 0x80000000u) ? ~u : (u | 0x80000000u);
}
__device__ __forceinline__ float float_unordered(uint32_t o) {
    return __uint_as_float((o & 0x80000000u) ? (o & 0x7fffffffu) : ~o);
}

__global__ __launch_bounds__(1024) void seg_sums_kernel(const uint32_t* __restrict__ cnt, int n, uint32_t* __restrict__ partial) {
    __shared__ uint32_t wsum[16];
    const int t = threadIdx.x, j0 = blockIdx.x * SCAN_CHUNK + 4 * t;
    uint32_t s = 0;
#pragma unroll
    for (int k = 0; k < 4; ++k) s += j0 + k < n ? cnt[j0 + k] : 0u;
#pragma unroll
    for (int d = 32; d >= 1; d >>= 1) s += __shfl_xor(s, d, 64);
    if ((t & 63) == 0) wsum[t >> 6] = s;
    __syncthreads();
    if (t == 0) { uint32_t tot = 0; for (int k = 0; k < 16; ++k) tot += wsum[k]; partial[blockIdx.x] = tot; }
}

__global__ __launch_bounds__(1024) void seg_scan_kernel(const uint32_t* __restrict__ cnt, int n, int ntiles, int F,
                                                        const uint32_t* __restrict__ partial, int nblocks,
                                                        uint2* __restrict__ ranges, uint32_t* __restrict__ cursor,
                                                        uint32_t* __restrict__ frame_base ,
                                                        uint32_t* __restrict__ num_rendered ,
                                                        uint32_t* __restrict__ total_out, uint32_t max_rendered,
                                                        uint32_t* __restrict__ cls ) {
    __shared__ uint32_t wsum[16], wtot[16];
    __shared__ uint32_t s_base, s_total;
    const int t = threadIdx.x;
    const unsigned lane = t & 63, w = t >> 6;
    uint32_t before = 0, all = 0;
    for (int k = t; k < nblocks; k += 1024) { const uint32_t p = partial[k]; all += p; if (k < (int)blockIdx.x) before += p; }
#pragma unroll
    for (int d = 32; d >= 1; d >>= 1) { before += __shfl_xor(before, d, 64); all += __shfl_xor(all, d, 64); }
    if (lane == 0) { wsum[w] = before; wtot[w] = all; }
    __syncthreads();
    if (t == 0) {
        uint32_t b = 0, a = 0;
        for (int k = 0; k < 16; ++k) { b += wsum[k]; a += wtot[k]; }
        s_base = b; s_total = a;
    }
    __syncthreads();
    const uint32_t total = s_total;
    const bool overflow = total > max_rendered;
    const int j0 = blockIdx.x * SCAN_CHUNK + 4 * t;
    uint32_t c[4], s = 0;
#pragma unroll
    for (int k = 0; k < 4; ++k) { c[k] = j0 + k < n ? cnt[j0 + k] : 0u; s += c[k]; }
    const uint32_t incl = gvf_wave_incl_scan(s, lane);
    __syncthreads();
    if (lane == 63) wsum[w] = incl;
    __syncthreads();
    uint32_t run = s_base + incl - s;
    for (unsigned k = 0; k < w; ++k) run += wsum[k];
#pragma unroll
    for (int k = 0; k < 4; ++k) {
        const int j = j0 + k;
        if (j < n) {
            ranges[j] = overflow ? make_uint2(0u, 0u) : make_uint2(run, run + c[k]);
            cursor[j] = run;
            if (!overflow && c[k] > (uint32_t)SORT_SMALL_N) {
                if (c[k] > (uint32_t)SORT_LARGE_N) cls[2 + n + atomicAdd(&cls[1], 1u)] = (uint32_t)j;
                else cls[2 + atomicAdd(&cls[0], 1u)] = (uint32_t)j | (c[k] > (uint32_t)SORT_MEDIUM_N ? 0x80000000u : 0u);
            }
            if (j % ntiles == 0) frame_base[j / ntiles] = run;
        }
        run += c[k];
    }
    if (blockIdx.x == 0 && t == 0) { frame_base[F] = total; *total_out = overflow ? 0u : total; }
}

__global__ void frame_counts_kernel(const uint32_t* __restrict__ frame_base, int F, uint32_t* __restrict__ num_rendered) {
    const int f = blockIdx.x * blockDim.x + threadIdx.x;
    if (f < F) num_rendered[f] = frame_base[f + 1] - frame_base[f];
}

constexpr int WIN_MAX = 2048;

template <bool SCATTER, typename REC>
__global__ __launch_bounds__(PRE_THREADS) void bin_kernel(int P, int gx, int gy, const REC* __restrict__ binrec,
                                                          const uint32_t* __restrict__ order,
                                                          uint32_t* __restrict__ tile_count ,
                                                          uint32_t* __restrict__ cursor ,
                                                          const uint32_t* __restrict__ total,
                                                          uint64_t* __restrict__ payload,
                                                          const uint32_t* __restrict__ frame_base, uint32_t* __restrict__ num_rendered,
                                                          int rec_by_id, int xcd_frames, int F) {
    __shared__ uint32_t s_tab[WIN_MAX];
    __shared__ uint32_t s_run[SCATTER ? WIN_MAX : 1];
    __shared__ int s_box[4];
    int blk = (int)blockIdx.x, f = (int)blockIdx.y;
    if (xcd_frames) {
        const int nblk = (P + BIN_SLOTS - 1) / BIN_SLOTS, k = (int)(blockIdx.x >> 3);
        f = (k / nblk) * 8 + (int)(blockIdx.x & 7u);
        blk = k - (k / nblk) * nblk;
        if (f >= F) return;
    }
    if (SCATTER && num_rendered != nullptr && blk == 0 && threadIdx.x == 0)
        num_rendered[f] = frame_base[f + 1] - frame_base[f];
    if (SCATTER && *total == 0u) return;
    const int t = threadIdx.x, lane = t & 63;
    if (t == 0) { s_box[0] = 0x7fffffff; s_box[1] = 0x7fffffff; s_box[2] = 0; s_box[3] = 0; }
    int x0[BIN_SPT], y0[BIN_SPT], x1[BIN_SPT], y1[BIN_SPT];
    uint64_t key[BIN_SPT];
    int bx0 = 0x7fffffff, by0 = 0x7fffffff, bx1 = 0, by1 = 0;
#pragma unroll
    for (int k = 0; k < BIN_SPT; ++k) {
        const int s = blk * BIN_SLOTS + k * PRE_THREADS + t;
        x0[k] = y0[k] = x1[k] = y1[k] = 0; key[k] = 0;
        if (s < P) {
            const uint32_t id = order != nullptr ? order[s] : (uint32_t)s;
            const REC br = binrec[(size_t)f * P + (rec_by_id ? id : (uint32_t)s)];
            const TileRect r = binrec_rect(br);
            x0[k] = r.x0; y0[k] = r.y0; x1[k] = r.x1; y1[k] = r.y1;
            key[k] = ((uint64_t)binrec_depth(br) << 32) | id;
            if (x1[k] > x0[k] && y1[k] > y0[k]) {
                bx0 = min(bx0, x0[k]); by0 = min(by0, y0[k]); bx1 = max(bx1, x1[k]); by1 = max(by1, y1[k]);
            } else {
                x1[k] = x0[k];
            }
        }
    }
#pragma unroll
    for (int d = 32; d >= 1; d >>= 1) {
        bx0 = min(bx0, __shfl_xor(bx0, d, 64)); by0 = min(by0, __shfl_xor(by0, d, 64));
        bx1 = max(bx1, __shfl_xor(bx1, d, 64)); by1 = max(by1, __shfl_xor(by1, d, 64));
    }
    __syncthreads();
    if (lane == 0 && bx1 > bx0) {
        atomicMin(&s_box[0], bx0); atomicMin(&s_box[1], by0); atomicMax(&s_box[2], bx1); atomicMax(&s_box[3], by1);
    }
    __syncthreads();
    const int wx0 = s_box[0], wy0 = s_box[1], ww = s_box[2] - s_box[0], wh = s_box[3] - s_box[1];
    if (ww <= 0 || wh <= 0) return;
    uint32_t* gtab = (SCATTER ? cursor : tile_count) + (size_t)f * gx * gy;
    if (ww * wh <= WIN_MAX) {
        const int area = ww * wh;
        for (int e = t; e < area; e += PRE_THREADS) { s_tab[e] = 0u; if (SCATTER) s_run[e] = 0u; }
        __syncthreads();
#pragma unroll
        for (int k = 0; k < BIN_SPT; ++k)
            for (int y = y0[k]; y < y1[k]; ++y)
                for (int x = x0[k]; x < x1[k]; ++x) atomicAdd(&s_tab[(y - wy0) * ww + (x - wx0)], 1u);
        __syncthreads();
        for (int e = t; e < area; e += PRE_THREADS) {
            const uint32_t c = s_tab[e];
            if (c != 0u) {
                const int seg = (wy0 + e / ww) * gx + wx0 + e % ww;
                if (SCATTER) s_tab[e] = atomicAdd(&gtab[seg], c);
                else atomicAdd(&gtab[seg], c);
            }
        }
        if (SCATTER) {
            __syncthreads();
#pragma unroll
            for (int k = 0; k < BIN_SPT; ++k)
                for (int y = y0[k]; y < y1[k]; ++y)
                    for (int x = x0[k]; x < x1[k]; ++x) {
                        const int e = (y - wy0) * ww + (x - wx0);
                        payload[s_tab[e] + atomicAdd(&s_run[e], 1u)] = key[k];
                    }
        }
    } else {
#pragma unroll
        for (int k = 0; k < BIN_SPT; ++k)
            for (int y = y0[k]; y < y1[k]; ++y)
                for (int x = x0[k]; x < x1[k]; ++x) {
                    const uint32_t pos = atomicAdd(&gtab[y * gx + x], 1u);
                    if (SCATTER) payload[pos] = key[k];
                }
    }
}

constexpr int BINX_THREADS = 512;
constexpr int BINX_SPT = 4;

__device__ __forceinline__ void binx_count(uint32_t* s_tab, int gx, TileRect r) {
    for (int y = r.y0; y < r.y1; ++y)
        for (int x = r.x0; x < r.x1; ++x) atomicAdd(&s_tab[y * gx + x], 1u);
}

template <typename REC>
__global__ __launch_bounds__(BINX_THREADS) void bin_index_kernel(int P, int gx, const REC* __restrict__ binrec,
                                                                 uint32_t* __restrict__ tile_count,
                                                                 uint32_t* __restrict__ cursor,
                                                                 const uint32_t* __restrict__ total,
                                                                 uint64_t* __restrict__ payload, int ntiles,
                                                                 const uint32_t* __restrict__ frame_base, uint32_t* __restrict__ num_rendered) {
    __shared__ uint32_t s_tab[BINX_TAB];
    const int t = threadIdx.x, f = blockIdx.y;
    const int g0 = (int)blockIdx.x * BINX_PER_WG, g1 = min(P, g0 + BINX_PER_WG);
    for (int e = t; e < ntiles; e += BINX_THREADS) s_tab[e] = 0u;
    __syncthreads();
    if constexpr (sizeof(REC) == 16) {
        const uint4* rec = binrec + (size_t)f * P;
        for (int base = g0; base < g1; base += BINX_SPT * BINX_THREADS) {
            uint4 br[BINX_SPT];
#pragma unroll
            for (int k = 0; k < BINX_SPT; ++k) {
                const int s = base + k * BINX_THREADS + t;
                br[k] = s < g1 ? rec[s] : make_uint4(0u, 0u, 0u, 0u);
            }
#pragma unroll
            for (int k = 0; k < BINX_SPT; ++k) binx_count(s_tab, gx, binrec_rect16(br[k].x, br[k].y));
        }
    } else {
        const size_t a0 = (size_t)f * P + g0, a1 = (size_t)f * P + g1;
        const uint4* pairs = reinterpret_cast<const uint4*>(binrec);
        for (size_t jbase = a0 >> 1; 2 * jbase < a1; jbase += BINX_SPT * BINX_THREADS) {
            uint4 br[BINX_SPT];
#pragma unroll
            for (int k = 0; k < BINX_SPT; ++k) {
                const size_t j = jbase + k * BINX_THREADS + t;
                br[k] = 2 * j < a1 ? pairs[j] : make_uint4(0u, 0u, 0u, 0u);
            }
#pragma unroll
            for (int k = 0; k < BINX_SPT; ++k) {
                const size_t a = 2 * (jbase + k * BINX_THREADS + t);
                binx_count(s_tab, gx, binrec_rect8(a >= a0 ? br[k].x : 0u));
                binx_count(s_tab, gx, binrec_rect8(a + 1 < a1 ? br[k].z : 0u));
            }
        }
    }
    __syncthreads();
    uint32_t* gtab = tile_count + (size_t)f * ntiles;
    for (int e = t; e < ntiles; e += BINX_THREADS) {
        const uint32_t c = s_tab[e];
        if (c != 0u) atomicAdd(&gtab[e], c);
    }
}

__global__ __launch_bounds__(256) void bbox_kernel(int P, const float* __restrict__ xyz, uint32_t* __restrict__ mm) {
    __shared__ uint32_t s_mm[6];
    if (threadIdx.x < 6) s_mm[threadIdx.x] = threadIdx.x < 3 ? 0xffffffffu : 0u;
    __syncthreads();
    uint32_t lo[3] = {0xffffffffu, 0xffffffffu, 0xffffffffu}, hi[3] = {0u, 0u, 0u};
    for (int i = blockIdx.x * blockDim.x + threadIdx.x; i < P; i += gridDim.x * blockDim.x) {
#pragma unroll
        for (int k = 0; k < 3; ++k) {
            const float v = xyz[3 * (size_t)i + k];
            if (v == v && fabsf(v) < 3.0e38f) {
                const uint32_t o = float_ordered(v);
                lo[k] = min(lo[k], o); hi[k] = max(hi[k], o);
            }
        }
    }
#pragma unroll
    for (int k = 0; k < 3; ++k) {
#pragma unroll
        for (int d = 32; d >= 1; d >>= 1) {
            lo[k] = min(lo[k], (uint32_t)__shfl_xor((int)lo[k], d, 64));
            hi[k] = max(hi[k], (uint32_t)__shfl_xor((int)hi[k], d, 64));
        }
        if ((threadIdx.x & 63) == 0) { atomicMin(&s_mm[k], lo[k]); atomicMax(&s_mm[3 + k], hi[k]); }
    }
    __syncthreads();
    if (threadIdx.x < 3) atomicMin(&mm[threadIdx.x], s_mm[threadIdx.x]);
    else if (threadIdx.x < 6) atomicMax(&mm[threadIdx.x], s_mm[threadIdx.x]);
}

__device__ __forceinline__ uint32_t spread5(uint32_t v) {
    return (v & 1u) | ((v & 2u) << 2) | ((v & 4u) << 4) | ((v & 8u) << 6) | ((v & 16u) << 8);
}


__device__ __forceinline__ uint32_t morton15(int i, const float* __restrict__ xyz, const uint32_t* __restrict__ mm) {
    uint32_t code = 0;
#pragma unroll
    for (int k = 0; k < 3; ++k) {
        const float lo = float_unordered(mm[k]), hi = float_unordered(mm[3 + k]);
        const float v = xyz[3 * (size_t)i + k];
        float q = (v - lo) / fmaxf(hi - lo, 1e-30f) * 32.0f;
        q = (q == q) ? fminf(fmaxf(q, 0.0f), 31.0f) : 0.0f;
        code |= spread5((uint32_t)q) << k;
    }
    return code;
}

__global__ __launch_bounds__(256) void morton_count_kernel(int P, const float* __restrict__ xyz,
                                                           const uint32_t* __restrict__ mm, uint32_t* __restrict__ codes,
                                                           uint32_t* __restrict__ hist) {
    const int i = blockIdx.x * blockDim.x + threadIdx.x;
    if (i >= P) return;
    const uint32_t c = morton15(i, xyz, mm);
    codes[i] = c;
    atomicAdd(&hist[c], 1u);
}

__global__ __launch_bounds__(1024) void morton_scan_kernel(uint32_t* __restrict__ hist) {
    __shared__ uint32_t wsum[16];
    const int t = threadIdx.x;
    const unsigned lane = t & 63, w = t >> 6;
    constexpr int PER = MORTON_BINS / 1024;
    uint32_t v[PER], s = 0;
#pragma unroll
    for (int k = 0; k < PER; ++k) { v[k] = hist[t * PER + k]; s += v[k]; }
    const uint32_t incl = gvf_wave_incl_scan(s, lane);
    if (lane == 63) wsum[w] = incl;
    __syncthreads();
    uint32_t run = incl - s;
    for (unsigned k = 0; k < w; ++k) run += wsum[k];
#pragma unroll
    for (int k = 0; k < PER; ++k) { hist[t * PER + k] = run; run += v[k]; }
}

__global__ __launch_bounds__(256) void morton_scatter_kernel(int P, uint32_t* codes_rank, uint32_t* __restrict__ hist,
                                                             uint32_t* __restrict__ order) {
    const int i = blockIdx.x * blockDim.x + threadIdx.x;
    if (i >= P) return;
    const uint32_t slot = atomicAdd(&hist[codes_rank[i]], 1u);
    order[slot] = (uint32_t)i;
    codes_rank[i] = slot;
}

__global__ __launch_bounds__(256) void ranges_kernel(const uint64_t* __restrict__ keys,
                                                     const uint32_t* __restrict__ n_ptr, uint32_t n_cap,
                                                     uint2* __restrict__ ranges, uint32_t n_ranges) {
    uint32_t n = *n_ptr;
    n = n < n_cap ? n : n_cap;
    for (uint32_t k = blockIdx.x * blockDim.x + threadIdx.x; k < n; k += gridDim.x * blockDim.x) {
        uint32_t cur = (uint32_t)(keys[k] >> 32);
        if (cur >= n_ranges) continue;
        if (k == 0) ranges[cur].x = 0;
        else {
            uint32_t prev = (uint32_t)(keys[k - 1] >> 32);
            if (cur != prev) { if (prev < n_ranges) ranges[prev].y = k; ranges[cur].x = k; }
        }
        if (k == n - 1) ranges[cur].y = n;
    }
}

struct FrameChunk { GvfRastFrame f[16]; };
struct CallTables {
    uint32_t* ranges; uint32_t n_ranges;
    uint32_t* tile_count; uint32_t n_tile_count;
    uint32_t* mhist; uint32_t n_mhist;
    uint32_t* cls;
    uint32_t* mm;
    uint32_t layout;
};
__global__ void upload_frames_kernel(FrameChunk c, int count, GvfRastFrame* __restrict__ dst, CallTables tab) {
    if (blockIdx.x == 0) {
        const int words = (int)(sizeof(GvfRastFrame) / 4) * count;
        const uint32_t* src = reinterpret_cast<const uint32_t*>(&c);
        for (int k = threadIdx.x; k < words; k += blockDim.x) reinterpret_cast<uint32_t*>(dst)[k] = src[k];
        if (tab.cls != nullptr && threadIdx.x < 2) tab.cls[threadIdx.x] = 0u;
        if (tab.mm != nullptr && threadIdx.x < 6) tab.mm[threadIdx.x] = threadIdx.x < 3 ? 0xffffffffu : 0u;
        if (tab.mm != nullptr && threadIdx.x == LAYOUT_WORD) tab.mm[LAYOUT_WORD] = tab.layout;
        return;
    }
    const uint32_t t = (blockIdx.x - 1) * blockDim.x + threadIdx.x, nt = (gridDim.x - 1) * blockDim.x;
    for (uint32_t k = t; k < tab.n_ranges; k += nt) tab.ranges[k] = 0u;
    for (uint32_t k = t; k < tab.n_tile_count; k += nt) tab.tile_count[k] = 0u;
    for (uint32_t k = t; k < tab.n_mhist; k += nt) tab.mhist[k] = 0u;
}

PreParams pre_params(const RastCall& c, const RastPlan& plan) {
    const GvfRastSettings& st = *c.st;
    PreParams pp;
    pp.P = c.P; pp.M = c.colors_precomp ? 0 : c.M; pp.deg = st.sh_degree; pp.H = st.image_height; pp.W = st.image_width; pp.mode = st.mode;
    pp.gx = plan.gx; pp.gy = plan.gy; pp.kernel_size = st.kernel_size; pp.scale_modifier = st.scale_modifier;
    pp.fused = c.fused ? 1 : 0; pp.n_delta = c.n_delta; pp.F = c.F;
    pp.upstream_binning = plan.upstream_binning;
    if (c.fused) pp.act = *c.act; else pp.act = GvfGaussianActivation{};
    pp.delta_lds = 0;
    return pp;
}

struct PreArgs {
    const float *a0 = nullptr, *a1 = nullptr, *a2 = nullptr, *a3 = nullptr;
    const float *sh = nullptr, *colors_precomp = nullptr, *cov3D_precomp = nullptr, *delta = nullptr;
    uint32_t* tiles_touched = nullptr;
    int32_t* radii = nullptr;
    uint32_t* block_sums = nullptr;
    uint4* binrec = nullptr;
    const uint32_t* bin_slot = nullptr;
};
template <bool SHARED, bool WAVE_FRAMES = false>
void launch_preprocess(hipStream_t stream, const RastPlan& plan, const PreParams& pp, const Workspace& w, const PreArgs& a) {
    const int32_t* g = WAVE_FRAMES ? plan.wf_grid : plan.pre_grid;
    const size_t lds = (size_t)(WAVE_FRAMES ? plan.wf_lds_bytes : plan.pre_lds_bytes);
    if (plan.rec8)
        hipLaunchKernelGGL((preprocess_kernel<SHARED, WAVE_FRAMES, BinRec8>), dim3(g[0], g[1]), dim3(PRE_THREADS), lds, stream, pp, w.frames,
                           a.a0, a.a1, a.a2, a.a3, a.sh, a.colors_precomp, a.cov3D_precomp, a.delta, w.splats, a.tiles_touched, a.radii,
                           a.block_sums, reinterpret_cast<BinRec8*>(a.binrec), a.bin_slot);
    else
        hipLaunchKernelGGL((preprocess_kernel<SHARED, WAVE_FRAMES, BinRec16>), dim3(g[0], g[1]), dim3(PRE_THREADS), lds, stream, pp, w.frames,
                           a.a0, a.a1, a.a2, a.a3, a.sh, a.colors_precomp, a.cov3D_precomp, a.delta, w.splats, a.tiles_touched, a.radii,
                           a.block_sums, a.binrec, a.bin_slot);
}

template <typename REC>
void launch_bin_count(hipStream_t stream, const RastCall& c, const RastPlan& plan, const Workspace& w, const uint32_t* order) {
    const REC* rec = reinterpret_cast<const REC*>(w.binrec);
    const int gather = plan.rec_gather ? 1 : 0;
    if (plan.index_count)
        hipLaunchKernelGGL((bin_index_kernel<REC>), dim3(plan.binx_grid[0], plan.binx_grid[1]), dim3(BINX_THREADS), 0, stream, c.P, plan.gx, rec,
                           w.tile_count, w.cursor, w.total, w.keys, plan.ntiles, nullptr, nullptr);
    else
        hipLaunchKernelGGL((bin_kernel<false, REC>), dim3(plan.bin_grid[0], plan.bin_grid[1]), dim3(PRE_THREADS), 0, stream, c.P, plan.gx, plan.gy,
                           rec, order, w.tile_count, w.cursor, w.total, w.keys, nullptr, nullptr, gather, gather, c.F);
}
template <typename REC>
void launch_bin_scatter(hipStream_t stream, const RastCall& c, const RastPlan& plan, const Workspace& w, const uint32_t* order) {
    const int gather = plan.rec_gather ? 1 : 0;
    hipLaunchKernelGGL((bin_kernel<true, REC>), dim3(plan.bin_grid[0], plan.bin_grid[1]), dim3(PRE_THREADS), 0, stream, c.P, plan.gx, plan.gy,
                       reinterpret_cast<const REC*>(w.binrec), order, w.tile_count, w.cursor, w.total, w.keys, w.frame_base,
                       c.out_num_rendered, gather, gather, c.F);
}

PreArgs input_args(const RastCall& c) {
    PreArgs a;
    a.a0 = c.a0; a.a1 = c.a1; a.a2 = c.a2; a.a3 = c.a3;
    a.sh = c.colors_precomp ? nullptr : c.sh; a.colors_precomp = c.colors_precomp; a.cov3D_precomp = c.cov3D_precomp; a.delta = c.delta;
    return a;
}

void launch_morton_order(hipStream_t stream, const RastCall& c, const Workspace& w) {
    int bb = (c.P + 255) / 256; if (bb > 128) bb = 128;
    const int pb = (c.P + 255) / 256;
    hipLaunchKernelGGL(bbox_kernel, dim3(bb), dim3(256), 0, stream, c.P, c.a0, w.mm);
    hipLaunchKernelGGL(morton_count_kernel, dim3(pb), dim3(256), 0, stream, c.P, c.a0, w.mm, w.order_alt, w.mhist);
    hipLaunchKernelGGL(morton_scan_kernel, dim3(1), dim3(1024), 0, stream, w.mhist);
    hipLaunchKernelGGL(morton_scatter_kernel, dim3(pb), dim3(256), 0, stream, c.P, w.order_alt, w.mhist, w.order);
}

void launch_shared_preprocess(hipStream_t stream, const RastCall& c, const RastPlan& plan, const PreParams& pp, const Workspace& w,
                              const uint32_t* order) {
    const int P = c.P;
    ActSlices slices;
    slices.n = plan.n_slices;
    for (int k = 0; k < plan.n_slices; ++k) slices.di[k] = plan.di[k];
    float4* rec3d = reinterpret_cast<float4*>(w.keys_alt);
    float* sh_by_slot = plan.slot_mode ? reinterpret_cast<float*>(rec3d + 4 * (size_t)plan.n_slices * (size_t)P) : nullptr;
    hipLaunchKernelGGL(activate_cov_kernel, dim3((P + 255) / 256, plan.n_slices), dim3(256), 0, stream, *c.act, c.st->scale_modifier, P, slices,
                       c.a0, c.a1, c.a2, c.a3, c.delta, rec3d, plan.slot_mode ? w.order_alt : nullptr, c.sh, pp.M * 3, sh_by_slot);
    PreArgs a;
    a.a0 = reinterpret_cast<const float*>(rec3d);
    a.radii = c.out_radii == nullptr ? nullptr : w.radii;
    a.binrec = w.binrec;
    if (plan.slot_mode) {
        a.a1 = reinterpret_cast<const float*>(order);
        a.sh = sh_by_slot;
    } else {
        a.sh = c.colors_precomp ? nullptr : c.sh;
        a.colors_precomp = c.colors_precomp;
        a.bin_slot = order != nullptr ? w.order_alt : nullptr;
    }
    launch_preprocess<true>(stream, plan, pp, w, a);
}

int key_end_bit(int F, int ntiles) {
    uint64_t m = (uint64_t)F * (uint64_t)ntiles;
    int bits = 0;
    while (((uint64_t)1 << bits) < m) ++bits;
    return 32 + bits;
}

}

int gvf_rast::upload_frames(hipStream_t stream, const RastCall& c, const RastPlan& plan, const Workspace& w) {
    for (int f0 = 0; f0 < c.F; f0 += 16) {
        FrameChunk ch;
        const int cnt = c.F - f0 < 16 ? c.F - f0 : 16;
        for (int k = 0; k < cnt; ++k) {
            ch.f[k] = c.frames_host[f0 + k];
            ch.f[k].reserved[0] = plan.frame_slice[(size_t)(f0 + k)];
        }
        CallTables tab = {};
        if (f0 == 0) {
            tab.ranges = reinterpret_cast<uint32_t*>(w.ranges); tab.n_ranges = 2u * (uint32_t)plan.nseg;
            tab.tile_count = w.tile_count; tab.n_tile_count = (uint32_t)plan.nseg;
            tab.mhist = w.mhist; tab.n_mhist = plan.morton ? (uint32_t)MORTON_BINS : 0u;
            tab.cls = w.cls; tab.mm = w.mm; tab.layout = (uint32_t)plan.layout;
        }
        hipLaunchKernelGGL(upload_frames_kernel, dim3(1 + (f0 == 0 ? plan.clear_blocks : 0)), dim3(256), 0, stream, ch, cnt, w.frames + f0, tab);
    }
    GVF_CHECK_LAUNCH();
    return GVF_OK;
}

int gvf_rast::front_end_bucket(hipStream_t stream, const RastCall& c, const RastPlan& plan, const Workspace& w, const hipEvent_t* marks) {
    const int P = c.P, F = c.F;
    prof_mark(stream, marks, 0);
    const uint32_t* order = nullptr;
    if (plan.morton) {
        launch_morton_order(stream, c, w);
        order = w.order;
        GVF_CHECK_LAUNCH();
    }
    prof_mark(stream, marks, 1);
    const PreParams pp = pre_params(c, plan);
    if (plan.shared) {
        launch_shared_preprocess(stream, c, plan, pp, w, order);
    } else {
        PreArgs a = input_args(c);
        a.radii = c.out_radii == nullptr ? nullptr : w.radii;
        a.binrec = w.binrec;
        if (plan.wave_frames) launch_preprocess<false, true>(stream, plan, pp, w, a);
        else launch_preprocess<false>(stream, plan, pp, w, a);
    }
    if (plan.rec8) launch_bin_count<BinRec8>(stream, c, plan, w, order);
    else launch_bin_count<BinRec16>(stream, c, plan, w, order);
    GVF_CHECK_LAUNCH();
    prof_mark(stream, marks, 2);
    hipLaunchKernelGGL(seg_sums_kernel, dim3(plan.scan_blocks), dim3(1024), 0, stream, w.tile_count, plan.nseg, w.partial);
    hipLaunchKernelGGL(seg_scan_kernel, dim3(plan.scan_blocks), dim3(1024), 0, stream, w.tile_count, plan.nseg, plan.ntiles, F,
                       w.partial, plan.scan_blocks, w.ranges, w.cursor, w.frame_base, c.out_num_rendered, w.total,
                       (uint32_t)c.max_rendered, w.cls);
    if (c.max_rendered <= 0)
        hipLaunchKernelGGL(frame_counts_kernel, dim3((F + 63) / 64), dim3(64), 0, stream, w.frame_base, F, c.out_num_rendered);
    GVF_CHECK_LAUNCH();
    prof_mark(stream, marks, 3);
    if (c.max_rendered > 0) {
        if (plan.rec8) launch_bin_scatter<BinRec8>(stream, c, plan, w, order);
        else launch_bin_scatter<BinRec16>(stream, c, plan, w, order);
        GVF_CHECK_LAUNCH();
    }
    if (c.out_radii != nullptr &&
        hipMemcpyAsync(c.out_radii, w.radii, sizeof(int32_t) * (size_t)F * P, hipMemcpyDeviceToDevice, stream) != hipSuccess)
        return GVF_ELAUNCH;
    prof_mark(stream, marks, 4);
    prof_mark(stream, marks, 5);
    return GVF_OK;
}

int gvf_rast::front_end_radix(hipStream_t stream, const RastCall& c, const RastPlan& plan, const Workspace& w, const hipEvent_t* marks,
                              uint64_t** keys_sorted, uint32_t** vals_by_tile) {
    const int P = c.P, F = c.F;
    prof_mark(stream, marks, 0);
    prof_mark(stream, marks, 1);
    const PreParams pp = pre_params(c, plan);
    PreArgs a = input_args(c);
    a.tiles_touched = w.tiles_touched; a.radii = w.radii; a.block_sums = w.block_sums;
    launch_preprocess<false>(stream, plan, pp, w, a);
    GVF_CHECK_LAUNCH();
    prof_mark(stream, marks, 2);
    hipLaunchKernelGGL(scan_sums_kernel, dim3(1), dim3(1024), 0, stream, w.block_sums, plan.nb, F, w.frame_base,
                       c.out_num_rendered, w.total, (uint32_t)c.max_rendered);
    GVF_CHECK_LAUNCH();
    prof_mark(stream, marks, 3);
    if (c.max_rendered > 0) {
        hipLaunchKernelGGL(duplicate_kernel, dim3(plan.nb, F), dim3(PRE_THREADS), 0, stream, P, plan.gx, plan.gy, w.splats,
                           w.tiles_touched, w.radii, w.block_sums, w.keys, w.vals, (uint32_t)c.max_rendered, pp.upstream_binning);
        GVF_CHECK_LAUNCH();
    }
    if (c.out_radii != nullptr &&
        hipMemcpyAsync(c.out_radii, w.radii, sizeof(int32_t) * (size_t)F * P, hipMemcpyDeviceToDevice, stream) != hipSuccess)
        return GVF_ELAUNCH;
    prof_mark(stream, marks, 4);
    *keys_sorted = w.keys; *vals_by_tile = w.vals;
    if (c.max_rendered > 0) {
        int in_alt = 0;
        const int rc = gvf_sort_pairs_device_n(w.keys, w.keys_alt, w.vals, w.vals_alt, w.total, c.max_rendered, 32,
                                               key_end_bit(F, plan.ntiles), w.sort_tmp, w.sort_tmp_bytes, stream, &in_alt);
        if (rc != GVF_OK) return rc;
        if (in_alt) { *keys_sorted = w.keys_alt; *vals_by_tile = w.vals_alt; }
        int rblocks = (int)((c.max_rendered + 255) / 256);
        if (rblocks > 4096) rblocks = 4096;
        hipLaunchKernelGGL(ranges_kernel, dim3(rblocks), dim3(256), 0, stream, *keys_sorted, w.total, (uint32_t)c.max_rendered, w.ranges,
                           (uint32_t)plan.nseg);
        GVF_CHECK_LAUNCH();
    }
    prof_mark(stream, marks, 5);
    return GVF_OK;
}

extern "C" int gvf_gaussian_activate(const GvfGaussianActivation* act, int P, int M, const float* xyz_raw,
                                     const float* features_dc, const float* scaling_raw, const float* rotation_raw,
                                     const float* opacity_raw, const float* delta, float* means3D, float* scales,
                                     float* rotations, float* shs, float* opacities, void* stream) {
    if (!act || P < 0 || M < 1) return GVF_EINVAL;
    if (P == 0) return GVF_OK;
    if (!xyz_raw || !features_dc || !scaling_raw || !rotation_raw || !opacity_raw || !means3D || !scales ||
        !rotations || !shs || !opacities)
        return GVF_EINVAL;
    (void)hipGetLastError();
    hipLaunchKernelGGL(activate_kernel, dim3((P + 255) / 256), dim3(256), 0, (hipStream_t)stream, *act, P, M, xyz_raw,
                       features_dc, scaling_raw, rotation_raw, opacity_raw, delta, means3D, scales, rotations, shs,
                       opacities);
    GVF_CHECK_LAUNCH();
    return GVF_OK;
}
```

gvfdiffusion_amd/csrc/rast_plan.h:

```cpp
#pragma once
#include <cstddef>
#include <cstdint>
#include <vector>
#include "../../include/gvf_rast.h"

namespace gvf_rast {

constexpr int TILE = GVF_TILE;
constexpr int WAVE = 64;
constexpr int PRE_THREADS = 256;
#ifndef GVF_PRE_FB
#define GVF_PRE_FB 4
#endif
constexpr int PRE_FB = GVF_PRE_FB;
#ifndef GVF_PRE_WAVE_FB
#define GVF_PRE_WAVE_FB 6
#endif
constexpr int PRE_WAVES = PRE_THREADS / WAVE;
constexpr int PRE_WAVE_FB = GVF_PRE_WAVE_FB;
constexpr int ACT_MAX_SLICES = 16;
constexpr int SCAN_CHUNK = 4096;
constexpr int BIN_SPT = 4;
constexpr int BIN_SLOTS = PRE_THREADS * BIN_SPT;
constexpr int BINX_TAB = 4096;
constexpr int BINX_PER_WG = 8192;
constexpr int BIN_REC8_MAX_GRID = 255;
constexpr int MORTON_BINS = 1 << 15;
constexpr int ORDER_TILES_MIN_SEGS = 2048;

constexpr int LAYOUT_WORD = 6;
constexpr uint32_t LAYOUT_SLOT_ORDER = 1u;

inline bool group_slices(const GvfRastFrame* frames_host, int F, bool has_delta, int cap, std::vector<int32_t>& slices,
                         std::vector<int32_t>& frame_slice) {
    slices.clear();
    frame_slice.assign((size_t)(F > 0 ? F : 0), 0);
    for (int f = 0; f < F; ++f) {
        const int32_t di = (has_delta && frames_host[f].delta_index >= 0) ? frames_host[f].delta_index : -1;
        size_t k = 0;
        while (k < slices.size() && slices[k] != di) ++k;
        if (k == slices.size()) {
            if (cap > 0 && (int)slices.size() == cap) return false;
            slices.push_back(di);
        }
        frame_slice[(size_t)f] = (int32_t)k;
    }
    return true;
}

inline std::vector<int32_t> slice_table(const std::vector<int32_t>& slices, const std::vector<int32_t>& frame_slice) {
    const size_t F = frame_slice.size(), ns = slices.size();
    std::vector<int32_t> tab, starts;
    tab.reserve(F + 2 * ns + 1);
    for (size_t k = 0; k < ns; ++k) {
        starts.push_back((int32_t)tab.size());
        for (size_t f = 0; f < F; ++f)
            if (frame_slice[f] == (int32_t)k) tab.push_back((int32_t)f);
    }
    starts.push_back((int32_t)tab.size());
    tab.insert(tab.end(), starts.begin(), starts.end());
    tab.insert(tab.end(), slices.begin(), slices.end());
    return tab;
}

struct RastSwitches {
    bool shared_act = true;
    bool slot_order = true;
    bool pre_wave_frames = true;
    bool blend_order = true;
    bool bin_rec8 = true;
};

struct PlanInputs {
    int F, P, M;
    bool fused, has_sh, has_colors_precomp, has_cov3D_precomp, has_delta, has_subpixel_offset;
    int64_t max_rendered;
};

struct RastPlan : GvfRastPlan {
    int32_t di[ACT_MAX_SLICES];
    std::vector<int32_t> frame_slice;
    bool rec8;
};

inline int ceil_div(int a, int b) { return (a + b - 1) / b; }
inline int pre_lds_bytes(int rows, int M) { return (int)(((size_t)rows * M * 3 * sizeof(float) + 15) / 16 * 16 + 16); }

inline RastPlan plan_call(const GvfRastSettings& st, const GvfRastFrame* frames_host, const PlanInputs& in, const RastSwitches& sw) {
    RastPlan p = {};
    const int F = in.F, P = in.P;
    const size_t room = (size_t)(in.max_rendered > 0 ? in.max_rendered : 0) * 8u;
    p.gx = ceil_div(st.image_width, TILE); p.gy = ceil_div(st.image_height, TILE); p.ntiles = p.gx * p.gy;
    p.nb = ceil_div(P, PRE_THREADS);
    p.nseg = (int32_t)((size_t)F * p.ntiles);
    p.bucket = st.bin_algo != GVF_RAST_BIN_RADIX;
    p.upstream_binning = st.upstream_binning != 0 || in.has_subpixel_offset;

    std::vector<int32_t> slices;
    const bool few = group_slices(frames_host, F, in.has_delta, ACT_MAX_SLICES, slices, p.frame_slice);
    p.n_slices = (int32_t)slices.size();
    for (size_t k = 0; k < slices.size(); ++k) p.di[k] = slices[k];
    const size_t rec_bytes = (size_t)p.n_slices * (size_t)P * 64u;
    p.shared = sw.shared_act && in.fused && !in.has_cov3D_precomp && p.bucket && P > 0 && F >= 2 && few && F >= 2 * p.n_slices &&
               rec_bytes <= room;
    if (!p.shared) p.frame_slice.assign((size_t)F, 0);

    p.index_count = p.bucket && !p.shared && p.ntiles <= BINX_TAB;
    p.morton = p.bucket && F >= 4 && P >= 4096;
    const int M = in.has_colors_precomp ? 0 : in.M;
    p.slot_mode = p.shared && sw.slot_order && p.morton && p.nb > 0 && !in.has_colors_precomp && in.has_sh &&
                  rec_bytes + (size_t)P * (size_t)M * 3u * 4u <= room;
    p.layout = p.slot_mode ? LAYOUT_SLOT_ORDER : 0u;
    p.rec_gather = p.bucket && !p.shared && p.morton;
    p.wave_frames = !p.shared && p.bucket && sw.pre_wave_frames;
    p.rec8 = p.bucket && sw.bin_rec8 && p.gx <= BIN_REC8_MAX_GRID && p.gy <= BIN_REC8_MAX_GRID;
    p.order_tiles = sw.blend_order && P > 0 && p.nb > 0 && in.max_rendered > 0 && (size_t)F * p.ntiles >= (size_t)ORDER_TILES_MIN_SEGS;

    p.pre_grid[0] = p.nb; p.pre_grid[1] = ceil_div(F, PRE_FB);
    p.wf_grid[0] = ceil_div(P, WAVE); p.wf_grid[1] = ceil_div(F, PRE_WAVES * PRE_WAVE_FB);
    p.pre_lds_bytes = pre_lds_bytes(PRE_THREADS, M);
    p.wf_lds_bytes = pre_lds_bytes(WAVE, M);
    const int bnb = ceil_div(P, BIN_SLOTS);
    p.bin_grid[0] = p.rec_gather ? ceil_div(F, 8) * 8 * bnb : bnb; p.bin_grid[1] = p.rec_gather ? 1 : F;
    p.binx_grid[0] = ceil_div(P, BINX_PER_WG); p.binx_grid[1] = F;
    p.scan_blocks = (int32_t)(((size_t)p.nseg + SCAN_CHUNK - 1) / SCAN_CHUNK);
    const size_t clear_words = 2 * (size_t)p.nseg + (size_t)p.nseg + (p.morton ? (size_t)MORTON_BINS : 0u);
    const size_t clear_blocks = (clear_words + 4095) / 4096;
    p.clear_blocks = (int32_t)(clear_blocks < 256 ? clear_blocks : 256);
    return p;
}

}
```

gvfdiffusion_amd/csrc/rast_sort.hip:

```cpp
#include "rast_common.h"

namespace {

template <typename Ptr>
__device__ __forceinline__ void bitonic_sort_asc(Ptr keys, int n, int tid, int nthreads) {
    int npad = 2;
    while (npad < n) npad <<= 1;
    const int half = npad >> 1;
    for (int k = 2; k <= npad; k <<= 1) {
        for (int i = tid; i < half; i += nthreads) {
            const int blk = i / (k >> 1), off = i % (k >> 1);
            const int lo = blk * k + off, hi = blk * k + k - 1 - off;
            if (hi < n) {
                const uint64_t a = keys[lo], b = keys[hi];
                if (a > b) { keys[lo] = b; keys[hi] = a; }
            }
        }
        __syncthreads();
        for (int j = k >> 2; j > 0; j >>= 1) {
            for (int i = tid; i < half; i += nthreads) {
                const int lo = 2 * i - (i & (j - 1));
                const int hi = lo + j;
                if (hi < n) {
                    const uint64_t a = keys[lo], b = keys[hi];
                    if (a > b) { keys[lo] = b; keys[hi] = a; }
                }
            }
            __syncthreads();
        }
    }
}

template <int E, int NP, bool OUT_LDS = false>
__device__ __forceinline__ void tile_sort_regs(const uint64_t* __restrict__ k, const uint32_t* __restrict__ v,
                                               uint32_t* __restrict__ ids, int n, uint64_t* __restrict__ lds) {
    const int tid = threadIdx.x;
    const bool live = (tid & ~63) * E < n;
    uint64_t key[E];
#pragma unroll
    for (int r = 0; r < E; ++r) {
        const int e = tid * E + r;
        key[r] = e < n ? (v != nullptr ? ((k[e] << 32) | v[e]) : k[e]) : ~0ull;
    }
#pragma unroll
    for (int k2 = 2; k2 <= NP; k2 <<= 1) {
#pragma unroll
        for (int step = 0, j = k2 >> 1; j > 0; ++step, j >>= 1) {
            const int m = step == 0 ? k2 - 1 : j;
            const int mr = m & (E - 1), mt = m / E;
            if (mt == 0) {
                if (live) {
#pragma unroll
                    for (int r = 0; r < E; ++r) {
                        if (r < (r ^ mr)) {
                            const uint64_t a = key[r], b = key[r ^ mr];
                            if (a > b) { key[r] = b; key[r ^ mr] = a; }
                        }
                    }
                }
            } else if (mt < 64) {
                if (live) {
                    const int hb = step == 0 ? (k2 / E) >> 1 : mt;
                    const bool lower = (tid & hb) == 0;
                    uint64_t other[E];
#pragma unroll
                    for (int r = 0; r < E; ++r) {
                        const uint64_t src = key[r ^ mr];
                        const unsigned lo = __shfl_xor((unsigned)src, mt, 64);
                        const unsigned hi = __shfl_xor((unsigned)(src >> 32), mt, 64);
                        other[r] = ((uint64_t)hi << 32) | lo;
                    }
#pragma unroll
                    for (int r = 0; r < E; ++r)
                        key[r] = lower ? (other[r] < key[r] ? other[r] : key[r]) : (other[r] > key[r] ? other[r] : key[r]);
                }
            } else {
                __syncthreads();
                if (live) {
#pragma unroll
                    for (int r = 0; r < E; ++r) lds[tid * E + r] = key[r];
                }
                __syncthreads();
                if (live) {
#pragma unroll
                    for (int r = 0; r < E; ++r) {
                        const int e = tid * E + r, pe = e ^ m;
                        if (pe < n) {
                            const uint64_t other = lds[pe];
                            key[r] = e < pe ? (other < key[r] ? other : key[r]) : (other > key[r] ? other : key[r]);
                        }
                    }
                }
            }
        }
    }
    if (OUT_LDS) {
        __syncthreads();
#pragma unroll
        for (int r = 0; r < E; ++r) {
            const int e = tid * E + r;
            if (e < n) lds[e] = key[r];
        }
        return;
    }
#pragma unroll
    for (int r = 0; r < E; ++r) {
        const int e = tid * E + r;
        if (e < n) ids[e] = (uint32_t)key[r];
    }
}

constexpr int BKT_MAX_RUN = 40;
constexpr int BKT_AUX = 64;
constexpr int BKT_LARGE_NB = 4096;

#ifdef SORT_STATS
__device__ unsigned long long g_sort_stats[16];
extern "C" int gvf_debug_sort_stats(unsigned long long* out16, int reset) {
    if (out16 != nullptr && hipMemcpyFromSymbol(out16, HIP_SYMBOL(g_sort_stats), sizeof(g_sort_stats)) != hipSuccess) return 1;
    if (reset) { unsigned long long z[16] = {}; if (hipMemcpyToSymbol(HIP_SYMBOL(g_sort_stats), z, sizeof(z)) != hipSuccess) return 1; }
    return 0;
}
#endif
template <int E, int T, int C>
__device__ __forceinline__ bool tile_sort_buckets(const uint64_t* __restrict__ k, const uint32_t* __restrict__ v,
                                                  uint32_t* __restrict__ ids, int n, uint64_t* __restrict__ s_keys ,
                                                  uint32_t* __restrict__ s_hist ) {
    constexpr int NB = T * C, NW = T / 64;
    const int tid = threadIdx.x, lane = tid & 63, wave = tid >> 6;
    uint32_t* s_aux = s_hist + NB + 1;
    uint64_t key[E];
    uint32_t dmin = ~0u, dmax = 0u;
#pragma unroll
    for (int r = 0; r < E; ++r) {
        const int e = tid + T * r;
        key[r] = e < n ? (v != nullptr ? ((k[e] << 32) | v[e]) : k[e]) : 0ull;
        if (e < n) {
            const uint32_t d = (uint32_t)(key[r] >> 32);
            dmin = min(dmin, d);
            dmax = max(dmax, d);
        }
    }
#pragma unroll
    for (int i = 0; i < C; ++i) s_hist[tid + T * i] = 0u;
    dmin = gvf_wave_umin(dmin);
    dmax = gvf_wave_umax(dmax);
    if (lane == 0) { s_aux[wave] = dmin; s_aux[NW + wave] = dmax; }
    __syncthreads();
#pragma unroll
    for (int w = 0; w < NW; ++w) { dmin = min(dmin, s_aux[w]); dmax = max(dmax, s_aux[NW + w]); }
    const float scale = dmax > dmin ? (float)NB / (float)(dmax - dmin) : 0.0f;
    uint32_t bkt[E], slot[E];
#pragma unroll
    for (int r = 0; r < E; ++r) {
        if (tid + T * r < n) {
            bkt[r] = (uint32_t)min(NB - 1, (int)((float)((uint32_t)(key[r] >> 32) - dmin) * scale));
            slot[r] = atomicAdd(&s_hist[bkt[r]], 1u);
        }
    }
    __syncthreads();
    uint32_t cnt[C], tot = 0u, run = 0u;
#pragma unroll
    for (int i = 0; i < C; ++i) {
        cnt[i] = s_hist[tid * C + i];
        tot += cnt[i];
        run = max(run, cnt[i]);
    }
    const uint32_t incl = gvf_wave_incl_scan_dpp(tot);
    run = gvf_wave_umax(run);
    if (lane == 63) s_aux[2 * NW + wave] = incl;
    if (lane == 0) s_aux[3 * NW + wave] = run;
    __syncthreads();
    uint32_t base = incl - tot, longest = 0u;
#pragma unroll
    for (int w = 0; w < NW; ++w) {
        base += w < wave ? s_aux[2 * NW + w] : 0u;
        longest = max(longest, s_aux[3 * NW + w]);
    }
#ifdef SORT_STATS
    if (tid == 0) {
        atomicAdd(&g_sort_stats[0], 1ull); atomicAdd(&g_sort_stats[2], (unsigned long long)n);
        if (longest > (uint32_t)BKT_MAX_RUN) { atomicAdd(&g_sort_stats[1], 1ull); atomicAdd(&g_sort_stats[3], (unsigned long long)n); }
        atomicAdd(&g_sort_stats[4 + min(11u, longest >> 3)], 1ull);
    }
#endif
    if (longest > (uint32_t)BKT_MAX_RUN) return false;
#pragma unroll
    for (int i = 0; i < C; ++i) {
        s_hist[tid * C + i] = base;
        base += cnt[i];
    }
    if (tid == T - 1) s_hist[NB] = (uint32_t)n;
    __syncthreads();
#pragma unroll
    for (int r = 0; r < E; ++r)
        if (tid + T * r < n) s_keys[s_hist[bkt[r]] + slot[r]] = key[r];
    __syncthreads();
#pragma unroll
    for (int r = 0; r < E; ++r) {
        const int p = tid + T * r;
        if (p < n) {
            const uint64_t mine = s_keys[p];
            const int b = min(NB - 1, (int)((float)((uint32_t)(mine >> 32) - dmin) * scale));
            const uint32_t lo = s_hist[b], hi = s_hist[b + 1];
            uint32_t rank = lo;
#pragma unroll
            for (uint32_t j = 0; j < 4; ++j)
                rank += (lo + j < hi && s_keys[min(lo + j, (uint32_t)(T * E) - 1u)] < mine) ? 1u : 0u;
            for (uint32_t j = lo + 4; j < hi; ++j) rank += s_keys[j] < mine ? 1u : 0u;
            ids[rank] = (uint32_t)mine;
        }
    }
    return true;
}

__device__ __forceinline__ int lower_bound_u64(const uint64_t* a, int n, uint64_t x) {
    int lo = 0, hi = n;
    while (lo < hi) {
        const int mid = (lo + hi) >> 1;
        if (a[mid] < x) lo = mid + 1; else hi = mid;
    }
    return lo;
}

__global__ __launch_bounds__(256) void classify_kernel(const uint2* __restrict__ ranges, uint32_t nseg,
                                                       uint32_t* __restrict__ cls ) {
    const uint32_t i = blockIdx.x * blockDim.x + threadIdx.x;
    if (i >= nseg) return;
    const uint2 r = ranges[i];
    const uint32_t n = r.y - r.x;
    if (n > (uint32_t)SORT_LARGE_N) cls[2 + nseg + atomicAdd(&cls[1], 1u)] = i;
    else if (n > (uint32_t)SORT_SMALL_N) cls[2 + atomicAdd(&cls[0], 1u)] = i | (n > (uint32_t)SORT_MEDIUM_N ? 0x80000000u : 0u);
}

template <int MODE>
__global__ __launch_bounds__(MODE == 3 ? 512 : 1024, MODE == 3 ? 2 : 1) void tile_sort_kernel(const uint2* __restrict__ ranges, uint64_t* __restrict__ keys,
                                 const uint32_t* __restrict__ vals, uint32_t* __restrict__ ids,
                                 const uint32_t* __restrict__ cls, uint32_t nseg, uint32_t split = 0u ) {
    __shared__ uint64_t s_small[MODE == 0 ? SORT_SMALL_N : 1];
    __shared__ uint32_t s_hist[MODE == 0 ? SORT_SMALL_N + 1 + BKT_AUX : (MODE == 1 || MODE == 3 ? BKT_LARGE_NB + 1 + BKT_AUX : 1)];
    extern __shared__ __attribute__((aligned(16))) uint64_t s_large[];
    if (MODE == 0) {
        const uint2 rng = ranges[blockIdx.x];
        const int n = (int)(rng.y - rng.x);
        if (n <= 0 || n > SORT_SMALL_N) return;
        const uint64_t* k = keys + rng.x;
        const uint32_t* v = vals != nullptr ? vals + rng.x : nullptr;
        uint32_t* o = ids + rng.x;
        if (n > 128) {
            bool done;
            if (n <= 256) done = tile_sort_buckets<1, 256, 1>(k, v, o, n, s_small, s_hist);
            else if (n <= 512) done = tile_sort_buckets<2, 256, 2>(k, v, o, n, s_small, s_hist);
            else if (n <= 768) done = tile_sort_buckets<3, 256, 3>(k, v, o, n, s_small, s_hist);
            else if (n <= 1024) done = tile_sort_buckets<4, 256, 4>(k, v, o, n, s_small, s_hist);
            else if (n <= 1280) done = tile_sort_buckets<5, 256, 5>(k, v, o, n, s_small, s_hist);
            else if (n <= 1536 || SORT_SMALL_N == 1536) done = tile_sort_buckets<6, 256, 6>(k, v, o, n, s_small, s_hist);
            else done = tile_sort_buckets<SORT_SMALL_N / 256, 256, SORT_SMALL_N / 256>(k, v, o, n, s_small, s_hist);
            if (done) return;
            __syncthreads();
        }
        if (n <= 64) tile_sort_regs<1, 64>(k, v, o, n, s_small);
        else if (n <= 128) tile_sort_regs<1, 128>(k, v, o, n, s_small);
        else if (n <= 256) tile_sort_regs<1, 256>(k, v, o, n, s_small);
        else if (n <= 512) tile_sort_regs<2, 512>(k, v, o, n, s_small);
        else if (n <= 1024) tile_sort_regs<4, 1024>(k, v, o, n, s_small);
        else {
            const int nb = n - 1024;
            const uint32_t* vb = v != nullptr ? v + 1024 : nullptr;
            tile_sort_regs<4, 1024, true>(k, v, o, 1024, s_small);
            if (nb <= 64) tile_sort_regs<1, 64, true>(k + 1024, vb, o, nb, s_small + 1024);
            else if (nb <= 128) tile_sort_regs<1, 128, true>(k + 1024, vb, o, nb, s_small + 1024);
            else if (nb <= 256) tile_sort_regs<1, 256, true>(k + 1024, vb, o, nb, s_small + 1024);
            else if (nb <= 512 || SORT_SMALL_N == 1536) tile_sort_regs<2, 512, true>(k + 1024, vb, o, nb, s_small + 1024);
            else tile_sort_regs<4, 1024, true>(k + 1024, vb, o, nb, s_small + 1024);
            __syncthreads();
            for (int e = threadIdx.x; e < n; e += 256) {
                const uint64_t key = s_small[e];
                const int pos = e < 1024 ? e + lower_bound_u64(s_small + 1024, nb, key)
                                         : (e - 1024) + lower_bound_u64(s_small, 1024, key);
                o[pos] = (uint32_t)key;
            }
        }
        return;
    }
    const bool huge = MODE == 2 || (MODE == 1 && blockIdx.x >= (uint32_t)SORT_LARGE_BLOCKS);
    const uint32_t bid = (MODE == 1 && huge) ? blockIdx.x - SORT_LARGE_BLOCKS : blockIdx.x;
    const uint32_t stride = MODE == 1 ? (huge ? (uint32_t)SORT_HUGE_BLOCKS : (uint32_t)SORT_LARGE_BLOCKS) : gridDim.x;
    const uint32_t count = cls[huge ? 1 : 0];
    const uint32_t* list = cls + 2 + (huge ? nseg : 0u);
    const int tid = threadIdx.x, nt = blockDim.x;
    for (uint32_t li = bid; li < count; li += stride) {
        const uint32_t ent = list[li];
        const bool upper = !huge && (ent >> 31) != 0u;
        if (!huge && ((MODE == 3 && upper) || (MODE == 1 && split != 0u && !upper))) continue;
        const uint2 rng = ranges[huge ? ent : (ent & 0x7fffffffu)];
        const int n = (int)(rng.y - rng.x);
        uint64_t* k = keys + rng.x;
        const uint32_t* v = vals != nullptr ? vals + rng.x : nullptr;
        if (huge) {
            if (v != nullptr)
                for (int i = tid; i < n; i += nt) k[i] = (k[i] << 32) | v[i];
            __syncthreads();
            bitonic_sort_asc(k, n, tid, nt);
            for (int i = tid; i < n; i += nt) ids[rng.x + i] = (uint32_t)k[i];
        } else {
            if (MODE == 3) {
                const bool sorted = tile_sort_buckets<8, 512, BKT_LARGE_NB / 512>(k, v, ids + rng.x, n, s_large, s_hist);
                __syncthreads();
                if (sorted) continue;
            }
            if (MODE == 1) {
                bool sorted;
                if (n <= 4096) sorted = tile_sort_buckets<4, 1024, BKT_LARGE_NB / 1024>(k, v, ids + rng.x, n, s_large, s_hist);
                else if (n <= 8192) sorted = tile_sort_buckets<8, 1024, BKT_LARGE_NB / 1024>(k, v, ids + rng.x, n, s_large, s_hist);
                else sorted = tile_sort_buckets<16, 1024, BKT_LARGE_NB / 1024>(k, v, ids + rng.x, n, s_large, s_hist);
                __syncthreads();
                if (sorted) continue;
            }
            for (int i = tid; i < n; i += nt) s_large[i] = v != nullptr ? ((k[i] << 32) | v[i]) : k[i];
            __syncthreads();
            bitonic_sort_asc(s_large, n, tid, nt);
            for (int i = tid; i < n; i += nt) ids[rng.x + i] = (uint32_t)s_large[i];
        }
        __syncthreads();
    }
}

}

int gvf_rast::tile_sort_set_lds_limit() {
    static GvfPerDeviceOnce once;
    return gvf_once_per_device(once, [] {
        return hipFuncSetAttribute(reinterpret_cast<const void*>(&tile_sort_kernel<1>), hipFuncAttributeMaxDynamicSharedMemorySize, SORT_LARGE_N * 8) ==
               hipSuccess;
    }) ? GVF_OK : GVF_ELAUNCH;
}

int gvf_rast::launch_tile_sort(hipStream_t stream, const uint2* ranges, uint64_t* keys, const uint32_t* vals, uint32_t* ids, uint32_t* cls,
                               uint32_t nseg, int cls_state) {
    if (cls_state == 0 && hipMemsetAsync(cls, 0, 2 * sizeof(uint32_t), stream) != hipSuccess) return GVF_ELAUNCH;
    if (cls_state < 2)
        hipLaunchKernelGGL(classify_kernel, dim3((nseg + 255) / 256), dim3(256), 0, stream, ranges, nseg, cls);
    hipLaunchKernelGGL(tile_sort_kernel<0>, dim3(nseg), dim3(256), 0, stream, ranges, keys, vals, ids, cls, nseg);
    if (tile_sort_set_lds_limit() != GVF_OK) return GVF_ELAUNCH;
    hipLaunchKernelGGL(tile_sort_kernel<3>, dim3(SORT_MEDIUM_BLOCKS), dim3(512), SORT_MEDIUM_N * 8, stream, ranges, keys, vals, ids, cls,
                       nseg, 0u);
    hipLaunchKernelGGL(tile_sort_kernel<1>, dim3(SORT_LARGE_BLOCKS + SORT_HUGE_BLOCKS), dim3(1024), SORT_LARGE_N * 8, stream, ranges, keys,
                       vals, ids, cls, nseg, 1u);
    GVF_CHECK_LAUNCH();
    return GVF_OK;
}

extern "C" int gvf_tile_sort_u64(uint64_t* keys, const uint32_t* ranges, int nseg, uint32_t* ids, uint32_t* scratch, void* stream) {
    if (nseg < 0) return GVF_EINVAL;
    if (nseg == 0) return GVF_OK;
    if (!keys || !ranges || !ids || !scratch) return GVF_EINVAL;
    (void)hipGetLastError();
    return launch_tile_sort((hipStream_t)stream, reinterpret_cast<const uint2*>(ranges), keys, nullptr, ids, scratch, (uint32_t)nseg, 0);
}
```

gvfdiffusion_amd/rasterizer.py:

```python
import ctypes
import os
from typing import Optional

import torch

from . import _lib

_WORKSPACES = {}


def _workspace(device, nbytes: int) -> torch.Tensor:
    dev_index = device.index if device.index is not None else torch.cuda.current_device()
    key = (dev_index, int(torch.cuda.current_stream(device).cuda_stream))
    ws = _WORKSPACES.get(key)
    if ws is None or ws.numel() < nbytes:
        ws = None
        _WORKSPACES.pop(key, None)
        ws = torch.empty(int(nbytes * 1.25) + 4096, dtype=torch.uint8, device=device)
        _WORKSPACES[key] = ws
    return ws


def workspace_bytes(P: int, F: int, H: int, W: int, max_rendered: int) -> int:
    out = ctypes.c_size_t(0)
# ... 65 lines not shown
        raise Exception("Please provide excatly one of either SHs or precomputed colors!")
    if ((scales is None or rotations is None) and cov3D_precomp is None) or \
            ((scales is not None or rotations is not None) and cov3D_precomp is not None):
        raise Exception("Please provide exactly one of either scale/rotation pair or precomputed 3D covariance!")
    dev = means3D.device
    means3D = _f32c(means3D, "means3D")
    P = means3D.shape[0]
    opacities = _f32c(opacities, "opacities").reshape(-1)
    shs = _f32c(shs, "shs")
    M = 0 if shs is None else shs.shape[1]
    colors_precomp = _f32c(colors_precomp, "colors_precomp")
    scales, rotations = _f32c(scales, "scales"), _f32c(rotations, "rotations")
    cov3D_precomp = _f32c(cov3D_precomp, "cov3D_precomp")
    if subpixel_offset is not None:
        subpixel_offset = _f32c(subpixel_offset, "subpixel_offset")
    H, W = settings.image_height, settings.image_width

    color = torch.empty((3, H, W), dtype=torch.float32, device=dev)
    alpha = torch.empty((H, W), dtype=torch.float32, device=dev) if want_alpha_depth else None
    depth = torch.empty((H, W), dtype=torch.float32, device=dev) if want_alpha_depth else None
    radii = torch.empty((P,), dtype=torch.int32, device=dev)
    nr = torch.zeros((1,), dtype=torch.int32, device=dev)

    key = (P, H, W, 1)
    cap = _CAP_HINT.get(key, max(4 * P, 1 << 16))
    while True:
        nbytes = workspace_bytes(P, 1, H, W, cap)
        ws = torch.empty(nbytes + 256, dtype=torch.uint8, device=dev) if private_workspace else _workspace(dev, nbytes + 256)
        base = (ws.data_ptr() + 255) // 256 * 256
        rc = _lib.lib().gvf_rast_forward(
            ctypes.byref(settings), ctypes.byref(frame), P, M, _lib.ptr(means3D), _lib.ptr(shs),
            _lib.ptr(colors_precomp), _lib.ptr(opacities), _lib.ptr(scales), _lib.ptr(rotations),
            _lib.ptr(cov3D_precomp), _lib.ptr(subpixel_offset), ctypes.c_void_p(base), nbytes, cap,
            _lib.ptr(color), _lib.ptr(alpha), _lib.ptr(depth), _lib.ptr(radii), _lib.ptr(nr),
            _lib.current_stream(dev))
        _lib.check(rc, "gvf_rast_forward")
        n = int(nr.item()) & 0xFFFFFFFF
        if n <= cap:
            break
        cap = int(n * 1.25) + 1024
    _CAP_HINT[key] = cap
    out = dict(color=color, alpha=alpha, depth=depth, radii=radii, num_rendered=n)
    if private_workspace:
        out.update(workspace=ws, workspace_bytes=nbytes, max_rendered=cap)
    return out


class _RasterizeFn(torch.autograd.Function):

    @staticmethod
    def forward(ctx, settings, frame, want_ad, subpixel_offset, means3D, means2D, shs, colors_precomp, opacities, scales,
                rotations, cov3D_precomp):
        ctx.in_dtypes = tuple(None if t is None else t.dtype for t in
                              (means3D, means2D, shs, colors_precomp, opacities, scales, rotations, cov3D_precomp))
        means3D, shs, colors_precomp, opacities, scales, rotations, cov3D_precomp = (
            _f32c(t, "input") for t in (means3D, shs, colors_precomp, opacities, scales, rotations, cov3D_precomp))
        out = _rasterize_impl(settings, frame, means3D, opacities, shs, colors_precomp, scales, rotations, cov3D_precomp,
                              subpixel_offset, want_ad, private_workspace=True)
        ctx.settings, ctx.frame, ctx.want_ad = settings, frame, want_ad
        ctx.ws, ctx.ws_bytes, ctx.cap = out["workspace"], out["workspace_bytes"], out["max_rendered"]
        ctx.has = (shs is not None, colors_precomp is not None, scales is not None, cov3D_precomp is not None,
                   means2D is not None)
        ctx.save_for_backward(*[t if t is not None else torch.empty(0) for t in
                                (means3D, shs, colors_precomp, opacities, scales, rotations, cov3D_precomp, subpixel_offset)])
        ctx.shapes = (opacities.shape, None if means2D is None else means2D.shape)
        dev = means3D.device
        H, W = settings.image_height, settings.image_width
        alpha = out["alpha"] if want_ad else torch.zeros((H, W), device=dev)
        depth = out["depth"] if want_ad else torch.zeros((H, W), device=dev)
        ctx.mark_non_differentiable(out["radii"])
        ctx.num_rendered = out["num_rendered"]
        return out["color"], alpha, depth, out["radii"]

    @staticmethod
    def backward(ctx, g_color, g_alpha, g_depth, _g_radii):
        means3D, shs, colors_precomp, opacities, scales, rotations, cov3D_precomp, sub = \
            [t if t.numel() > 0 or k == 0 else None for k, t in enumerate(ctx.saved_tensors)]
        has_shs, has_col, has_sr, has_cov, has_m2 = ctx.has
        shs = shs if has_shs else None
        colors_precomp = colors_precomp if has_col else None
        scales, rotations = (scales, rotations) if has_sr else (None, None)
        cov3D_precomp = cov3D_precomp if has_cov else None
        sub = sub if (sub is not None and sub.numel() > 0) else None
        dev = means3D.device
        P = means3D.shape[0]
        M = 0 if shs is None else shs.shape[1]
        f32 = dict(dtype=torch.float32, device=dev)
        g_color = _f32c(g_color if g_color is not None else torch.zeros((3, ctx.settings.image_height, ctx.settings.image_width), **f32), "g")
        g_alpha = _f32c(g_alpha, "g") if ctx.want_ad and g_alpha is not None else None
        g_depth = _f32c(g_depth, "g") if ctx.want_ad and g_depth is not None else None
        nb = ctypes.c_size_t(0)
        _lib.check(_lib.lib().gvf_rast_backward_scratch_bytes(P, ctypes.byref(nb)), "gvf_rast_backward_scratch_bytes")
        scratch = torch.empty(int(nb.value) + 16, dtype=torch.uint8, device=dev)
        sbase = (scratch.data_ptr() + 15) // 16 * 16
        d_m3 = torch.empty((P, 3), **f32)
        d_m2 = torch.empty((P, 2), **f32)
        d_shs = torch.empty((P, M, 3), **f32) if shs is not None else None
        d_col = torch.empty((P, 3), **f32) if colors_precomp is not None else None
        d_op = torch.empty((P,), **f32)
        d_sc = torch.empty((P, 3), **f32) if scales is not None else None
        d_ro = torch.empty((P, 4), **f32) if rotations is not None else None
        d_c6 = torch.empty((P, 6), **f32) if cov3D_precomp is not None else None
        base = (ctx.ws.data_ptr() + 255) // 256 * 256
        rc = _lib.lib().gvf_rast_backward(
            ctypes.byref(ctx.settings), ctypes.byref(ctx.frame), P, M, _lib.ptr(means3D), _lib.ptr(shs), _lib.ptr(colors_precomp),
            _lib.ptr(opacities), _lib.ptr(scales), _lib.ptr(rotations), _lib.ptr(cov3D_precomp), _lib.ptr(sub),
            ctypes.c_void_p(base), ctx.ws_bytes, ctx.cap, _lib.ptr(g_color), _lib.ptr(g_alpha), _lib.ptr(g_depth),
            ctypes.c_void_p(sbase), int(nb.value), _lib.ptr(d_m3), _lib.ptr(d_m2), _lib.ptr(d_shs), _lib.ptr(d_col),
            _lib.ptr(d_op), _lib.ptr(d_sc), _lib.ptr(d_ro), _lib.ptr(d_c6), _lib.current_stream(dev))
        _lib.check(rc, "gvf_rast_backward")
        op_shape, m2_shape = ctx.shapes
        g_m2 = None
        if has_m2:
            g_m2 = torch.zeros(m2_shape, **f32)
            g_m2[:, :2] = d_m2
        grads = (d_m3, g_m2, d_shs, d_col, d_op.reshape(op_shape), d_sc, d_ro, d_c6)
        grads = tuple(g if g is None or dt is None or g.dtype == dt else g.to(dt) for g, dt in zip(grads, ctx.in_dtypes))
        return (None, None, None, None) + grads


def rasterize_batched(settings, frames, act, xyz_raw, features_dc, scaling_raw, rotation_raw, opacity_raw,
                      delta=None, want_alpha_depth=False, want_radii=False, max_rendered=None, sync=True, color_u8=False):
    diff = (torch.is_grad_enabled() and not color_u8 and
            any(t is not None and t.requires_grad for t in (xyz_raw, features_dc, scaling_raw, rotation_raw, opacity_raw, delta)))
    if diff:
        _lib.require_cuda(xyz_raw, features_dc, scaling_raw, rotation_raw, opacity_raw, delta)
        arr = (_lib.GvfRastFrame * len(frames))(*frames)
        color, alpha, depth, radii, nr, cap = _RasterizeBatchedFn.apply(
            settings, arr, act, bool(want_alpha_depth), bool(want_radii), max_rendered,
            xyz_raw, features_dc, scaling_raw, rotation_raw, opacity_raw, delta)
        return dict(color=color, alpha=alpha if want_alpha_depth else None, depth=depth if want_alpha_depth else None,
                    radii=radii if want_radii else None, num_rendered=nr, max_rendered=int(cap))
    return _rasterize_batched_impl(settings, frames, act, xyz_raw, features_dc, scaling_raw, rotation_raw, opacity_raw, delta,
                                   want_alpha_depth, want_radii, max_rendered, sync, color_u8)


def _rasterize_batched_impl(settings, frames, act, xyz_raw, features_dc, scaling_raw, rotation_raw, opacity_raw,
                            delta=None, want_alpha_depth=False, want_radii=False, max_rendered=None, sync=True, color_u8=False,
                            private_workspace=False):
    _lib.require_cuda(xyz_raw, features_dc, scaling_raw, rotation_raw, opacity_raw, delta)
    dev = xyz_raw.device
    xyz_raw, features_dc = _f32c(xyz_raw, "xyz"), _f32c(features_dc, "features_dc")
    scaling_raw, rotation_raw = _f32c(scaling_raw, "scaling"), _f32c(rotation_raw, "rotation")
    opacity_raw = _f32c(opacity_raw, "opacity").reshape(-1)
    P, M = xyz_raw.shape[0], features_dc.shape[1]
    n_delta = 0
    if delta is not None:
        delta = _f32c(delta, "delta")
        if delta.dim() == 2:
            delta = delta[None]
        assert delta.shape[1] == P and delta.shape[2] == 14, "delta must be (n,P,14) [xyz3|scale3|rot4|rgb3|op1]"
        n_delta = delta.shape[0]
    F = len(frames)
    arr = frames if isinstance(frames, ctypes.Array) else (_lib.GvfRastFrame * F)(*frames)
    H, W = settings.image_height, settings.image_width
    if color_u8 and (want_alpha_depth or want_radii):
        raise _lib.GvfError("color_u8: the uint8 entry point has no alpha / depth / radii outputs")
    color = torch.empty((F, 3, H, W), dtype=torch.uint8 if color_u8 else torch.float32, device=dev)
    alpha = torch.empty((F, H, W), dtype=torch.float32, device=dev) if want_alpha_depth else None
    depth = torch.empty((F, H, W), dtype=torch.float32, device=dev) if want_alpha_depth else None
    radii = torch.empty((F, P), dtype=torch.int32, device=dev) if want_radii else None
    nr = torch.zeros((F,), dtype=torch.int32, device=dev)
    key = (P, H, W, F)
    cap = max_rendered if max_rendered is not None else _CAP_HINT.get(key, max(4 * P * F, 1 << 16))
    while True:
        nbytes = workspace_bytes(P, F, H, W, cap)
        ws = torch.empty(nbytes + 256, dtype=torch.uint8, device=dev) if private_workspace else _workspace(dev, nbytes + 256)
        base = (ws.data_ptr() + 255) // 256 * 256
        if color_u8:
            rc = _lib.lib().gvf_rast_forward_batched_u8(
                ctypes.byref(settings), arr, F, ctypes.byref(act), P, M, _lib.ptr(xyz_raw), _lib.ptr(features_dc),
                _lib.ptr(scaling_raw), _lib.ptr(rotation_raw), _lib.ptr(opacity_raw), _lib.ptr(delta), n_delta,
                ctypes.c_void_p(base), nbytes, cap, _lib.ptr(color), _lib.ptr(nr), _lib.current_stream(dev))
        else:
            rc = _lib.lib().gvf_rast_forward_batched(
                ctypes.byref(settings), arr, F, ctypes.byref(act), P, M, _lib.ptr(xyz_raw), _lib.ptr(features_dc),
                _lib.ptr(scaling_raw), _lib.ptr(rotation_raw), _lib.ptr(opacity_raw), _lib.ptr(delta), n_delta,
                ctypes.c_void_p(base), nbytes, cap, _lib.ptr(color), _lib.ptr(alpha), _lib.ptr(depth),
                _lib.ptr(radii), _lib.ptr(nr), _lib.current_stream(dev))
        _lib.check(rc, "gvf_rast_forward_batched")
        if private_workspace:
            private = (ws, nbytes)
        else:
            _LAST_CARVE[(dev.index if dev.index is not None else torch.cuda.current_device(), int(torch.cuda.current_stream(dev).cuda_stream))] = \
                (ws, base, nbytes, P, F, H, W, cap)
        if not sync and not private_workspace:
            break
        n = int(nr.to(torch.int64).bitwise_and(0xFFFFFFFF).sum().item())
        if n <= cap:
            break
        if max_rendered is not None:
            raise _lib.GvfError(f"max_rendered={max_rendered} too small: {n} instances")
        cap = int(n * 1.25) + 1024
    if sync or private_workspace:
        _CAP_HINT[key] = cap
    out = dict(color=color, alpha=alpha, depth=depth, radii=radii, num_rendered=nr, max_rendered=cap)
    if private_workspace:
        out.update(workspace=private[0], workspace_bytes=private[1])
    return out


class _RasterizeBatchedFn(torch.autograd.Function):

    @staticmethod
    def forward(ctx, settings, frames, act, want_ad, want_radii, max_rendered, xyz_raw, features_dc, scaling_raw, rotation_raw,
                opacity_raw, delta):
        inputs = (xyz_raw, features_dc, scaling_raw, rotation_raw, opacity_raw, delta)
        ctx.in_meta = tuple(None if t is None else (t.dtype, t.shape) for t in inputs)
        xyz_raw, features_dc, scaling_raw, rotation_raw = (_f32c(t, "input") for t in (xyz_raw, features_dc, scaling_raw, rotation_raw))
        opacity_raw = _f32c(opacity_raw, "input").reshape(-1)
        if delta is not None:
            delta = _f32c(delta, "input")
            if delta.dim() == 2:
                delta = delta[None]
        out = _rasterize_batched_impl(settings, frames, act, xyz_raw, features_dc, scaling_raw, rotation_raw, opacity_raw, delta,
                                      want_ad, want_radii, max_rendered, True, False, private_workspace=True)
        ctx.settings, ctx.frames, ctx.act, ctx.want_ad = settings, frames, act, want_ad
        ctx.ws, ctx.ws_bytes, ctx.cap = out["workspace"], out["workspace_bytes"], out["max_rendered"]
        ctx.has_delta = delta is not None
        ctx.save_for_backward(xyz_raw, features_dc, scaling_raw, rotation_raw, opacity_raw,
                              delta if delta is not None else torch.empty(0))
        dev = xyz_raw.device
        empty = lambda dt=torch.float32: torch.empty((0,), dtype=dt, device=dev)
        alpha = out["alpha"] if want_ad else empty()
        depth = out["depth"] if want_ad else empty()
        radii = out["radii"] if want_radii else empty(torch.int32)
        cap = torch.tensor(out["max_rendered"], dtype=torch.int64)
        ctx.mark_non_differentiable(radii, out["num_rendered"], cap)
        return out["color"], alpha, depth, radii, out["num_rendered"], cap

    @staticmethod
    def backward(ctx, g_color, g_alpha, g_depth, _g_radii, _g_nr, _g_cap):
        need = ctx.needs_input_grad[6:12]
        if not any(need):
            return (None,) * 12
        xyz_raw, features_dc, scaling_raw, rotation_raw, opacity_raw, delta = ctx.saved_tensors
        delta = delta if ctx.has_delta else None
        dev = xyz_raw.device
        P, M = xyz_raw.shape[0], features_dc.shape[1]
        st = ctx.settings
        F = len(ctx.frames)
        H, W = st.image_height, st.image_width
        n_delta = 0 if delta is None else delta.shape[0]
        f32 = dict(dtype=torch.float32, device=dev)
        g_color = _f32c(g_color, "g") if g_color is not None else torch.zeros((F, 3, H, W), **f32)
        g_alpha = _f32c(g_alpha, "g") if ctx.want_ad and g_alpha is not None else None
        g_depth = _f32c(g_depth, "g") if ctx.want_ad and g_depth is not None else None
        nb = ctypes.c_size_t(0)
        _lib.check(_lib.lib().gvf_rast_backward_batched_scratch_bytes(P, F, ctypes.byref(nb)), "gvf_rast_backward_batched_scratch_bytes")
        scratch = torch.empty(int(nb.value) + 16, dtype=torch.uint8, device=dev)
        sbase = (scratch.data_ptr() + 15) // 16 * 16
        outs = [torch.empty(shape, **f32) if n else None for n, shape in
                zip(need, ((P, 3), (P, M, 3), (P, 3), (P, 4), (P,), (n_delta, P, 14)))]
        base = (ctx.ws.data_ptr() + 255) // 256 * 256
        rc = _lib.lib().gvf_rast_backward_batched(
            ctypes.byref(st), ctx.frames, F, ctypes.byref(ctx.act), P, M, _lib.ptr(xyz_raw), _lib.ptr(features_dc),
            _lib.ptr(scaling_raw), _lib.ptr(rotation_raw), _lib.ptr(opacity_raw), _lib.ptr(delta), n_delta,
            ctypes.c_void_p(base), ctx.ws_bytes, ctx.cap, _lib.ptr(g_color), _lib.ptr(g_alpha), _lib.ptr(g_depth),
            ctypes.c_void_p(sbase), int(nb.value), *[_lib.ptr(t) for t in outs], _lib.current_stream(dev))
        _lib.check(rc, "gvf_rast_backward_batched")
        grads = []
        for g, meta in zip(outs, ctx.in_meta):
            if g is not None:
                dt, shape = meta
                g = g.reshape(shape)
                if g.dtype != dt:
                    g = g.to(dt)
            grads.append(g)
        return (None,) * 6 + tuple(grads)


_LAST_CARVE = {}


def sort_class_counts(device=None):
    device = torch.device("cuda", torch.cuda.current_device()) if device is None else torch.device(device)
    key = (device.index if device.index is not None else torch.cuda.current_device(), int(torch.cuda.current_stream(device).cuda_stream))
    if key not in _LAST_CARVE:
        raise _lib.GvfError("no batched rasteriser call on this stream yet")
    _ws, base, nbytes, P, F, H, W, cap = _LAST_CARVE[key]
    out = (ctypes.c_uint32 * 2)()
    _lib.check(_lib.lib().gvf_rast_sort_class_counts(ctypes.c_void_p(base), nbytes, P, F, H, W, cap, out, _lib.current_stream(device)),
               "gvf_rast_sort_class_counts")
    return int(out[0]), int(out[1])


def call_plan(settings, frames, P, M, max_rendered, fused=True, has_sh=True, has_colors_precomp=False, has_cov3D_precomp=False,
              has_delta=True, has_subpixel_offset=False):
    F = len(frames)
    arr = frames if isinstance(frames, ctypes.Array) else (_lib.GvfRastFrame * F)(*frames)
    out = _lib.GvfRastPlan()
    _lib.check(_lib.lib().gvf_rast_call_plan(ctypes.byref(settings), arr, F, int(P), int(M), int(fused), int(has_sh), int(has_colors_precomp),
                                             int(has_cov3D_precomp), int(has_delta), int(has_subpixel_offset), int(max_rendered),
                                             ctypes.byref(out)), "gvf_rast_call_plan")
    return out


def bin_record_bytes(settings):
    out = ctypes.c_int(0)
    _lib.check(_lib.lib().gvf_rast_bin_record_bytes(ctypes.byref(settings), ctypes.byref(out)), "gvf_rast_bin_record_bytes")
    return int(out.value)


def gaussian_activate(act, xyz_raw, features_dc, scaling_raw, rotation_raw, opacity_raw, delta=None):
    _lib.require_cuda(xyz_raw)
    dev = xyz_raw.device
    xyz_raw, features_dc = _f32c(xyz_raw, "xyz"), _f32c(features_dc, "features_dc")
    scaling_raw, rotation_raw = _f32c(scaling_raw, "scaling"), _f32c(rotation_raw, "rotation")
    opacity_raw = _f32c(opacity_raw, "opacity").reshape(-1)
    delta = _f32c(delta, "delta")
    P, M = xyz_raw.shape[0], features_dc.shape[1]
    out = dict(means3D=torch.empty((P, 3), device=dev), scales=torch.empty((P, 3), device=dev),
               rotations=torch.empty((P, 4), device=dev), shs=torch.empty((P, M, 3), device=dev),
               opacities=torch.empty((P, 1), device=dev))
    rc = _lib.lib().gvf_gaussian_activate(ctypes.byref(act), P, M, _lib.ptr(xyz_raw), _lib.ptr(features_dc),
                                          _lib.ptr(scaling_raw), _lib.ptr(rotation_raw), _lib.ptr(opacity_raw),
                                          _lib.ptr(delta), _lib.ptr(out["means3D"]), _lib.ptr(out["scales"]),
                                          _lib.ptr(out["rotations"]), _lib.ptr(out["shs"]),
                                          _lib.ptr(out["opacities"]), _lib.current_stream(dev))
    _lib.check(rc, "gvf_gaussian_activate")
    return out


def sort_pairs_u64(keys: torch.Tensor, values: torch.Tensor, end_bit: int = 64):
    _lib.require_cuda(keys, values)
    assert keys.dtype == torch.int64 and values.dtype == torch.int32 and keys.numel() == values.numel()
    dev = keys.device
    k, v = keys.clone().contiguous(), values.clone().contiguous()
    ka, va = torch.empty_like(k), torch.empty_like(v)
    n = k.numel()
    tb = int(_lib.lib().gvf_sort_tmp_bytes(n))
    tmp = torch.empty(tb + 256, dtype=torch.uint8, device=dev)
    base = (tmp.data_ptr() + 255) // 256 * 256
    rc = _lib.lib().gvf_sort_pairs_u64(_lib.ptr(k), _lib.ptr(ka), _lib.ptr(v), _lib.ptr(va), n, end_bit,
                                       ctypes.c_void_p(base), tb, _lib.current_stream(dev))
    _lib.check(rc, "gvf_sort_pairs_u64")
    return k, v


def tile_sort_u64(keys: torch.Tensor, ranges: torch.Tensor) -> torch.Tensor:
    _lib.require_cuda(keys, ranges)
    assert keys.dtype == torch.int64 and ranges.dtype == torch.int32 and ranges.dim() == 2 and ranges.shape[1] == 2
    k, r = keys.clone().contiguous(), ranges.contiguous()
    ids = torch.full((k.numel(),), -1, dtype=torch.int32, device=k.device)
    scratch = torch.empty((2 + 2 * r.shape[0],), dtype=torch.int32, device=k.device)
    _lib.check(_lib.lib().gvf_tile_sort_u64(_lib.ptr(k), _lib.ptr(r), r.shape[0], _lib.ptr(ids), _lib.ptr(scratch),
                                            _lib.current_stream(k.device)), "gvf_tile_sort_u64")
    return ids


def frames_to_uint8(rgb: torch.Tensor, out: torch.Tensor = None) -> torch.Tensor:
    _lib.require_cuda(rgb)
    rgb = _f32c(rgb, "rgb")
    if out is None:
        out = torch.empty(rgb.shape, dtype=torch.uint8, device=rgb.device)
    _lib.check(_lib.lib().gvf_rgb_to_u8(_lib.ptr(rgb), _lib.ptr(out), rgb.numel(), _lib.current_stream(rgb.device)),
               "gvf_rgb_to_u8")
    return out
```

include/gvf_rast.h:

```cpp
#ifndef GVF_RAST_H
#define GVF_RAST_H

#include <stddef.h>
#include <stdint.h>

#ifdef __cplusplus
extern "C" {
#endif

#define GVF_OK        0
#define GVF_EINVAL   (-1)
#define GVF_ENOSPC   (-2)
#define GVF_ELAUNCH  (-3)

#define GVF_RAST_MODE_MIP      0
#define GVF_RAST_MODE_DILATE   1

#define GVF_TILE 16

typedef struct GvfRastFrame {
    float viewmatrix[16];
    float projmatrix[16];
    float campos[3];
    float tanfovx;
    float tanfovy;
    int32_t delta_index;
    int32_t reserved[2];
} GvfRastFrame;

typedef struct GvfRastSettings {
    int32_t image_height;
    int32_t image_width;
    int32_t sh_degree;
    int32_t mode;
    float   kernel_size;
    float   scale_modifier;
    float   bg[3];
    int32_t prefiltered;
    int32_t debug;
    int32_t upstream_binning;
    int32_t bin_algo;
} GvfRastSettings;

#define GVF_RAST_BIN_AUTO   0
#define GVF_RAST_BIN_RADIX  1
#define GVF_RAST_BIN_BUCKET 2

typedef struct GvfGaussianActivation {
    float   aabb[6];
    float   scale_bias;
    float   opacity_bias;
    float   min_kernel_size;
    int32_t scaling_activation;
} GvfGaussianActivation;

int gvf_rast_workspace_bytes(int P, int F, int H, int W, int64_t max_rendered, size_t* bytes);

int gvf_rast_forward(const GvfRastSettings* settings_host, const GvfRastFrame* frame_host,
                     int P, int M,
                     const float* means3D, const float* shs, const float* colors_precomp,
                     const float* opacities, const float* scales, const float* rotations,
                     const float* cov3D_precomp, const float* subpixel_offset,
                     void* workspace, size_t workspace_bytes, int64_t max_rendered,
                     float* out_color, float* out_alpha, float* out_depth,
                     int32_t* out_radii, uint32_t* out_num_rendered,
                     void* stream);

int gvf_rast_backward_scratch_bytes(int P, size_t* bytes);
int gvf_rast_backward(const GvfRastSettings* settings_host, const GvfRastFrame* frame_host, int P, int M,
                      const float* means3D, const float* shs, const float* colors_precomp,
                      const float* opacities, const float* scales, const float* rotations,
                      const float* cov3D_precomp, const float* subpixel_offset,
                      const void* workspace, size_t workspace_bytes, int64_t max_rendered,
                      const float* dL_dcolor, const float* dL_dalpha, const float* dL_ddepth,
                      void* scratch, size_t scratch_bytes,
                      float* dL_dmeans3D, float* dL_dmeans2D, float* dL_dshs, float* dL_dcolors,
                      float* dL_dopacities, float* dL_dscales, float* dL_drotations, float* dL_dcov3D,
                      void* stream);

int gvf_rast_forward_batched(const GvfRastSettings* settings_host, const GvfRastFrame* frames_host, int F,
                             const GvfGaussianActivation* act_host,
                             int P, int M,
                             const float* xyz_raw, const float* features_dc, const float* scaling_raw,
                             const float* rotation_raw, const float* opacity_raw,
                             const float* delta, int n_delta,
                             void* workspace, size_t workspace_bytes, int64_t max_rendered,
                             float* out_color, float* out_alpha, float* out_depth,
                             int32_t* out_radii, uint32_t* out_num_rendered,
                             void* stream);

int gvf_rast_forward_batched_u8(const GvfRastSettings* settings_host, const GvfRastFrame* frames_host, int F,
                                const GvfGaussianActivation* act_host,
                                int P, int M,
                                const float* xyz_raw, const float* features_dc, const float* scaling_raw,
                                const float* rotation_raw, const float* opacity_raw,
                                const float* delta, int n_delta,
                                void* workspace, size_t workspace_bytes, int64_t max_rendered,
                                uint8_t* out_rgb_u8, uint32_t* out_num_rendered,
                                void* stream);

int gvf_rast_backward_batched_scratch_bytes(int P, int F, size_t* bytes);
int gvf_rast_backward_batched(const GvfRastSettings* settings_host, const GvfRastFrame* frames_host, int F,
                              const GvfGaussianActivation* act_host, int P, int M,
                              const float* xyz_raw, const float* features_dc, const float* scaling_raw,
                              const float* rotation_raw, const float* opacity_raw,
                              const float* delta, int n_delta,
                              const void* workspace, size_t workspace_bytes, int64_t max_rendered,
                              const float* dL_dcolor, const float* dL_dalpha, const float* dL_ddepth,
                              void* scratch, size_t scratch_bytes,
                              float* dL_dxyz_raw, float* dL_dfeatures_dc, float* dL_dscaling_raw,
                              float* dL_drotation_raw, float* dL_dopacity_raw, float* dL_ddelta,
                              void* stream);

int gvf_gaussian_activate(const GvfGaussianActivation* act_host, int P, int M,
                          const float* xyz_raw, const float* features_dc, const float* scaling_raw,
                          const float* rotation_raw, const float* opacity_raw, const float* delta,
                          float* means3D, float* scales, float* rotations, float* shs, float* opacities,
                          void* stream);

size_t gvf_sort_tmp_bytes(int64_t n);
int gvf_sort_pairs_u64(uint64_t* keys, uint64_t* keys_alt, uint32_t* values, uint32_t* values_alt,
                       int64_t n, int end_bit, void* tmp, size_t tmp_bytes, void* stream);

int gvf_tile_sort_u64(uint64_t* keys, const uint32_t* ranges, int nseg, uint32_t* ids, uint32_t* scratch, void* stream);

int gvf_rgb_to_u8(const float* rgb, uint8_t* out, int64_t n, void* stream);

#define GVF_RAST_NSTAGES 7
int gvf_rast_profile_enable(int on);
int gvf_rast_profile_read(float* ms_sum , int* calls);

int64_t gvf_rast_shared_activation_calls(void);

int gvf_rast_sort_class_counts(const void* workspace, size_t workspace_bytes, int P, int F, int H, int W, int64_t max_rendered,
                               uint32_t* counts_host , void* stream);

typedef struct GvfRastPlan {
    int32_t bucket, shared, index_count, morton, slot_mode, rec_gather, wave_frames, order_tiles, upstream_binning;
    int32_t n_slices, layout;
    int32_t gx, gy, ntiles, nb, nseg;
    int32_t pre_grid[2], wf_grid[2], bin_grid[2], binx_grid[2];
    int32_t scan_blocks, clear_blocks;
    int32_t pre_lds_bytes, wf_lds_bytes;
} GvfRastPlan;
int gvf_rast_call_plan(const GvfRastSettings* settings_host, const GvfRastFrame* frames_host, int F, int P, int M, int fused,
                       int has_sh, int has_colors_precomp, int has_cov3D_precomp, int has_delta, int has_subpixel_offset,
                       int64_t max_rendered, GvfRastPlan* out);

int gvf_rast_bin_record_bytes(const GvfRastSettings* settings_host, int* bytes);

int gvf_rast_slice_groups(const GvfRastFrame* frames_host, int F, int has_delta, int max_slices, int32_t* table_host, int* n_slices);

const char* gvf_version(void);

#ifdef __cplusplus
}
#endif
#endif
```

Before: 22270 frames/s.

## Fold Morton ordering and blend tile ordering into existing kernels as rider blocks

The separate Morton-order stages (bbox, code, histogram scan, scatter) now run as extra 'rider' blocks appended to the preprocess, seg-sum and scan kernel launches. The per-frame blend tile-order kernel is likewise folded into the small tile-sort launch as extra blocks. The aim is to cut kernel launches and serial gaps in the fused batched path. In exchange, the existing kernels gain more branching and shared-memory pressure, and the extra blocks compete for CUs with the main work. A debug API for reading back the Morton order is also added.

```diff
diff --git a/gvfdiffusion_amd/_lib.py b/gvfdiffusion_amd/_lib.py
--- a/gvfdiffusion_amd/_lib.py
+++ b/gvfdiffusion_amd/_lib.py
@@ -69,6 +69,9 @@
     "gvf_rast_call_plan": (_i, [ctypes.POINTER(GvfRastSettings), ctypes.POINTER(GvfRastFrame), _i, _i, _i, _i, _i, _i, _i, _i, _i, _i64,
                                 ctypes.POINTER(GvfRastPlan)]),
     "gvf_rast_bin_record_bytes": (_i, [ctypes.POINTER(GvfRastSettings), ctypes.POINTER(_i)]),
+    "gvf_rast_order_riders": (_i, [ctypes.POINTER(GvfRastSettings), ctypes.POINTER(GvfRastFrame), _i, _i, _i, _i, _i, _i, _i, _i, _i, _i64,
+                                   ctypes.POINTER(_i)]),
+    "gvf_rast_morton_order": (_i, [_vp, _sz, _i, _i, _i, _i, _i64, ctypes.POINTER(ctypes.c_uint32), _vp]),
     "gvf_rast_slice_groups": (_i, [ctypes.POINTER(GvfRastFrame), _i, _i, _i, ctypes.POINTER(ctypes.c_int32), ctypes.POINTER(_i)]),
     "gvf_rast_profile_enable": (_i, [_i]),
     "gvf_rast_profile_read": (_i, [ctypes.POINTER(_f), ctypes.POINTER(_i)]),
diff --git a/gvfdiffusion_amd/csrc/rast.hip b/gvfdiffusion_amd/csrc/rast.hip
--- a/gvfdiffusion_amd/csrc/rast.hip
+++ b/gvfdiffusion_amd/csrc/rast.hip
@@ -32,6 +32,7 @@
     sw.pre_wave_frames = switch_on("GVF_RAST_PRE_WAVE_FRAMES");
     sw.blend_order = switch_on("GVF_RAST_BLEND_ORDER");
     sw.bin_rec8 = switch_on("GVF_RAST_BIN_REC8");
+    sw.order_riders = switch_on("GVF_RAST_ORDER_RIDERS");
     return sw;
 }
 
@@ -84,11 +85,13 @@
         rc = plan.bucket ? front_end_bucket(stream, c, plan, w, marks) : front_end_radix(stream, c, plan, w, marks, &keys, &vals);
         if (rc != GVF_OK) return rc;
         if (c.max_rendered > 0 &&
-            (rc = launch_tile_sort(stream, w.ranges, keys, vals, w.ids, w.cls, (uint32_t)plan.nseg, plan.bucket ? 2 : 1)) != GVF_OK)
+            (rc = launch_tile_sort(stream, w.ranges, keys, vals, w.ids, w.cls, (uint32_t)plan.nseg, plan.bucket ? 2 : 1,
+                                   plan.tile_order_rider ? w.cursor : nullptr, plan.ntiles, c.F)) != GVF_OK)
             return rc;
     }
     rc = launch_blend(stream, st, c.P, c.F, w.ranges, w.ids, w.splats, c.subpixel_offset, out.color, out.alpha, out.depth, out.u8,
-                      plan.slot_mode ? w.order_alt : nullptr, plan.order_tiles ? w.cursor : nullptr, marks != nullptr ? marks[6] : nullptr);
+                      plan.slot_mode ? w.order_alt : nullptr, plan.order_tiles ? w.cursor : nullptr, plan.tile_order_rider,
+                      marks != nullptr ? marks[6] : nullptr);
     if (rc != GVF_OK) return rc;
     prof_mark(stream, marks, 7);
     return GVF_OK;
@@ -104,6 +107,20 @@
         int di = frames_host[f].delta_index;
         if (di >= 0 && (delta == nullptr || di >= n_delta)) return GVF_EINVAL;
     }
+    return GVF_OK;
+}
+
+int plan_from_flags(const GvfRastSettings* st, const GvfRastFrame* frames_host, int F, int P, int M, int fused, int has_sh,
+                    int has_colors_precomp, int has_cov3D_precomp, int has_delta, int has_subpixel_offset, int64_t max_rendered,
+                    RastPlan* plan) {
+    if (!st || !frames_host || M < 0) return GVF_EINVAL;
+    if (check_shape(*st, F, P, max_rendered) != GVF_OK) return GVF_EINVAL;
+    PlanInputs in;
+    in.F = F; in.P = P; in.M = M; in.fused = fused != 0;
+    in.has_sh = has_sh != 0; in.has_colors_precomp = has_colors_precomp != 0; in.has_cov3D_precomp = has_cov3D_precomp != 0;
+    in.has_delta = has_delta != 0; in.has_subpixel_offset = has_subpixel_offset != 0;
+    in.max_rendered = max_rendered;
+    *plan = plan_call(*st, frames_host, in, switches_from_env());
     return GVF_OK;
 }
 
@@ -204,15 +221,23 @@
 extern "C" int gvf_rast_call_plan(const GvfRastSettings* st, const GvfRastFrame* frames_host, int F, int P, int M, int fused, int has_sh,
                                   int has_colors_precomp, int has_cov3D_precomp, int has_delta, int has_subpixel_offset,
                                   int64_t max_rendered, GvfRastPlan* out) {
-    if (!st || !frames_host || !out || M < 0) return GVF_EINVAL;
-    if (check_shape(*st, F, P, max_rendered) != GVF_OK) return GVF_EINVAL;
-    PlanInputs in;
-    in.F = F; in.P = P; in.M = M; in.fused = fused != 0;
-    in.has_sh = has_sh != 0; in.has_colors_precomp = has_colors_precomp != 0; in.has_cov3D_precomp = has_cov3D_precomp != 0;
-    in.has_delta = has_delta != 0; in.has_subpixel_offset = has_subpixel_offset != 0;
-    in.max_rendered = max_rendered;
-    *out = plan_call(*st, frames_host, in, switches_from_env());
-    return GVF_OK;
+    if (!out) return GVF_EINVAL;
+    RastPlan plan;
+    const int rc = plan_from_flags(st, frames_host, F, P, M, fused, has_sh, has_colors_precomp, has_cov3D_precomp, has_delta,
+                                   has_subpixel_offset, max_rendered, &plan);
+    if (rc == GVF_OK) *out = plan;
+    return rc;
+}
+
+extern "C" int gvf_rast_order_riders(const GvfRastSettings* st, const GvfRastFrame* frames_host, int F, int P, int M, int fused, int has_sh,
+                                     int has_colors_precomp, int has_cov3D_precomp, int has_delta, int has_subpixel_offset,
+                                     int64_t max_rendered, int* riding) {
+    if (!riding) return GVF_EINVAL;
+    RastPlan plan;
+    const int rc = plan_from_flags(st, frames_host, F, P, M, fused, has_sh, has_colors_precomp, has_cov3D_precomp, has_delta,
+                                   has_subpixel_offset, max_rendered, &plan);
+    if (rc == GVF_OK) *riding = plan.order_riders ? 1 : 0;
+    return rc;
 }
 
 extern "C" int gvf_rast_bin_record_bytes(const GvfRastSettings* st, int* bytes) {
@@ -284,4 +309,16 @@
     return GVF_OK;
 }
 
+extern "C" int gvf_rast_morton_order(const void* workspace, size_t workspace_bytes, int P, int F, int H, int W, int64_t max_rendered,
+                                     uint32_t* order_host, void* stream) {
+    if (!workspace || !order_host || H <= 0 || W <= 0 || P <= 0 || F <= 0 || max_rendered < 0) return GVF_EINVAL;
+    if ((((uintptr_t)workspace) & 255) != 0) return GVF_EINVAL;
+    Workspace w = carve(const_cast<void*>(workspace), workspace_bytes, P, F, H, W, max_rendered);
+    if (!w.ok) return GVF_ENOSPC;
+    if (hipMemcpyAsync(order_host, w.order, (size_t)P * sizeof(uint32_t), hipMemcpyDeviceToHost, (hipStream_t)stream) != hipSuccess)
+        return GVF_ELAUNCH;
+    if (hipStreamSynchronize((hipStream_t)stream) != hipSuccess) return GVF_ELAUNCH;
+    return GVF_OK;
+}
+
 extern "C" const char* gvf_version(void) { return "gvf_hip 0.1.0 gfx950"; }
diff --git a/gvfdiffusion_amd/csrc/rast_blend.hip b/gvfdiffusion_amd/csrc/rast_blend.hip
--- a/gvfdiffusion_amd/csrc/rast_blend.hip
+++ b/gvfdiffusion_amd/csrc/rast_blend.hip
@@ -5,30 +5,8 @@
 
 __global__ __launch_bounds__(1024) void blend_order_kernel(const uint2* __restrict__ ranges, int ntiles, uint32_t* __restrict__ order) {
     __shared__ uint32_t hist[64];
-    const int f = blockIdx.x, t = threadIdx.x;
-    const uint2* r = ranges + (size_t)f * ntiles;
-    if (t < 64) hist[t] = 0u;
-    __syncthreads();
-    for (int tile = t; tile < ntiles; tile += 1024) {
-        const uint32_t n = r[tile].y - r[tile].x;
-        atomicAdd(&hist[63u - min(63u, n >> 5)], 1u);
-    }
-    __syncthreads();
-    const bool reorder = hist[0] != 0u;
-    __syncthreads();
-    if (!reorder) {
-        for (int tile = t; tile < ntiles; tile += 1024) order[(size_t)f * ntiles + tile] = (uint32_t)tile;
-        return;
-    }
-    if (t == 0) {
-        uint32_t run = 0u;
-        for (int c = 0; c < 64; ++c) { const uint32_t h = hist[c]; hist[c] = run; run += h; }
-    }
-    __syncthreads();
-    for (int tile = t; tile < ntiles; tile += 1024) {
-        const uint32_t n = r[tile].y - r[tile].x;
-        order[(size_t)f * ntiles + atomicAdd(&hist[63u - min(63u, n >> 5)], 1u)] = (uint32_t)tile;
-    }
+    const size_t f = blockIdx.x;
+    blend_order_block<1024>(ranges + f * ntiles, ntiles, order + f * ntiles, hist);
 }
 
 #ifdef BLEND_TIMING
@@ -252,10 +230,10 @@
 
 int gvf_rast::launch_blend(hipStream_t stream, const GvfRastSettings& st, int P, int F, const uint2* ranges, const uint32_t* point_list,
                            const float4* splats, const float* subpixel_offset, float* out_color, float* out_alpha, float* out_depth,
-                           unsigned char* out_u8, const uint32_t* rec_of, uint32_t* tile_order, hipEvent_t ordered) {
+                           unsigned char* out_u8, const uint32_t* rec_of, uint32_t* tile_order, bool order_ready, hipEvent_t ordered) {
     const int H = st.image_height, W = st.image_width;
     const int gx = (W + TILE - 1) / TILE, gy = (H + TILE - 1) / TILE, ntiles = gx * gy;
-    if (tile_order != nullptr) hipLaunchKernelGGL(blend_order_kernel, dim3(F), dim3(1024), 0, stream, ranges, ntiles, tile_order);
+    if (tile_order != nullptr && !order_ready) hipLaunchKernelGGL(blend_order_kernel, dim3(F), dim3(1024), 0, stream, ranges, ntiles, tile_order);
     if (ordered != nullptr) (void)hipEventRecord(ordered, stream);
     hipLaunchKernelGGL(out_depth != nullptr ? blend_kernel<true> : blend_kernel<false>, dim3(ntiles, F), dim3(BLEND_THREADS), 0, stream, P, H, W,
                        gx, gy, st.bg[0], st.bg[1], st.bg[2], ranges, point_list, splats, subpixel_offset, out_color, out_alpha, out_depth,
diff --git a/gvfdiffusion_amd/csrc/rast_common.h b/gvfdiffusion_amd/csrc/rast_common.h
--- a/gvfdiffusion_amd/csrc/rast_common.h
+++ b/gvfdiffusion_amd/csrc/rast_common.h
@@ -269,6 +269,33 @@
     return m;
 }
 
+template <int NT>
+__device__ __forceinline__ void blend_order_block(const uint2* __restrict__ r, int ntiles, uint32_t* __restrict__ order, uint32_t* hist) {
+    const int t = threadIdx.x;
+    if (t < 64) hist[t] = 0u;
+    __syncthreads();
+    for (int tile = t; tile < ntiles; tile += NT) {
+        const uint32_t n = r[tile].y - r[tile].x;
+        atomicAdd(&hist[63u - min(63u, n >> 5)], 1u);
+    }
+    __syncthreads();
+    const bool reorder = hist[0] != 0u;
+    __syncthreads();
+    if (!reorder) {
+        for (int tile = t; tile < ntiles; tile += NT) order[tile] = (uint32_t)tile;
+        return;
+    }
+    if (t == 0) {
+        uint32_t run = 0u;
+        for (int c = 0; c < 64; ++c) { const uint32_t h = hist[c]; hist[c] = run; run += h; }
+    }
+    __syncthreads();
+    for (int tile = t; tile < ntiles; tile += NT) {
+        const uint32_t n = r[tile].y - r[tile].x;
+        order[atomicAdd(&hist[63u - min(63u, n >> 5)], 1u)] = (uint32_t)tile;
+    }
+}
+
 constexpr int BWD_ACC = 10;
 
 }
@@ -311,11 +338,11 @@
                     uint64_t** keys_sorted, uint32_t** vals_by_tile);
 
 int launch_tile_sort(hipStream_t stream, const uint2* ranges, uint64_t* keys, const uint32_t* vals, uint32_t* ids, uint32_t* cls,
-                     uint32_t nseg, int cls_state);
+                     uint32_t nseg, int cls_state, uint32_t* tile_order = nullptr, int ntiles = 0, int F = 0);
 int tile_sort_set_lds_limit();
 
 int launch_blend(hipStream_t stream, const GvfRastSettings& st, int P, int F, const uint2* ranges, const uint32_t* point_list,
                  const float4* splats, const float* subpixel_offset, float* out_color, float* out_alpha, float* out_depth,
-                 unsigned char* out_u8, const uint32_t* rec_of, uint32_t* tile_order, hipEvent_t ordered);
+                 unsigned char* out_u8, const uint32_t* rec_of, uint32_t* tile_order, bool order_ready, hipEvent_t ordered);
 }
 using namespace gvf_rast;
diff --git a/gvfdiffusion_amd/csrc/rast_front.hip b/gvfdiffusion_amd/csrc/rast_front.hip
--- a/gvfdiffusion_amd/csrc/rast_front.hip
+++ b/gvfdiffusion_amd/csrc/rast_front.hip
@@ -15,6 +15,177 @@
     int F;
     int delta_lds;
 };
+
+struct OrderRiders {
+    int blocks;
+    int P, nboxes;
+    const float* xyz;
+    uint32_t* boxes;
+    uint32_t* mm;
+    uint32_t* codes;
+    uint32_t* hist;
+    uint32_t* slice_sums;
+    uint32_t* order;
+};
+
+__device__ __forceinline__ uint32_t float_ordered(float f) {
+    const uint32_t u = __float_as_uint(f);
+    return (u & 0x80000000u) ? ~u : (u | 0x80000000u);
+}
+__device__ __forceinline__ float float_unordered(uint32_t o) {
+    return __uint_as_float((o & 0x80000000u) ? (o & 0x7fffffffu) : ~o);
+}
+
+__device__ __forceinline__ void bbox_block(int P, const float* __restrict__ xyz, int first, int stride, uint32_t* s_mm) {
+    if (threadIdx.x < 6) s_mm[threadIdx.x] = threadIdx.x < 3 ? 0xffffffffu : 0u;
+    __syncthreads();
+    uint32_t lo[3] = {0xffffffffu, 0xffffffffu, 0xffffffffu}, hi[3] = {0u, 0u, 0u};
+    for (int i = first + (int)threadIdx.x; i < P; i += stride) {
+#pragma unroll
+        for (int k = 0; k < 3; ++k) {
+            const float v = xyz[3 * (size_t)i + k];
+            if (v == v && fabsf(v) < 3.0e38f) {
+                const uint32_t o = float_ordered(v);
+                lo[k] = min(lo[k], o); hi[k] = max(hi[k], o);
+            }
+        }
+    }
+#pragma unroll
+    for (int k = 0; k < 3; ++k) {
+#pragma unroll
+        for (int d = 32; d >= 1; d >>= 1) {
+            lo[k] = min(lo[k], (uint32_t)__shfl_xor((int)lo[k], d, 64));
+            hi[k] = max(hi[k], (uint32_t)__shfl_xor((int)hi[k], d, 64));
+        }
+        if ((threadIdx.x & 63) == 0) { atomicMin(&s_mm[k], lo[k]); atomicMax(&s_mm[3 + k], hi[k]); }
+    }
+    __syncthreads();
+}
+
+__device__ __forceinline__ void bbox_from_partials(const uint32_t* __restrict__ boxes, int n, uint32_t (&box)[6]) {
+    const int lane = (int)(threadIdx.x & 63);
+#pragma unroll
+    for (int k = 0; k < 6; ++k) {
+        uint32_t v = k < 3 ? 0xffffffffu : 0u;
+        for (int j = lane; j < n; j += 64) v = k < 3 ? min(v, boxes[6 * j + k]) : max(v, boxes[6 * j + k]);
+#pragma unroll
+        for (int d = 32; d >= 1; d >>= 1) {
+            const uint32_t o = (uint32_t)__shfl_xor((int)v, d, 64);
+            v = k < 3 ? min(v, o) : max(v, o);
+        }
+        box[k] = v;
+    }
+}
+
+__device__ __forceinline__ uint32_t spread5(uint32_t v) {
+    return (v & 1u) | ((v & 2u) << 2) | ((v & 4u) << 4) | ((v & 8u) << 6) | ((v & 16u) << 8);
+}
+
+__device__ __forceinline__ uint32_t morton15(int i, const float* __restrict__ xyz, const uint32_t (&box)[6]) {
+    uint32_t code = 0;
+#pragma unroll
+    for (int k = 0; k < 3; ++k) {
+        const float lo = float_unordered(box[k]), hi = float_unordered(box[3 + k]);
+        const float v = xyz[3 * (size_t)i + k];
+        float q = (v - lo) / fmaxf(hi - lo, 1e-30f) * 32.0f;
+        q = (q == q) ? fminf(fmaxf(q, 0.0f), 31.0f) : 0.0f;
+        code |= spread5((uint32_t)q) << k;
+    }
+    return code;
+}
+
+__device__ __forceinline__ void morton_count_one(int i, int P, const float* __restrict__ xyz, const uint32_t (&box)[6],
+                                                 uint32_t* __restrict__ codes, uint32_t* __restrict__ hist) {
+    if (i >= P) return;
+    const uint32_t c = morton15(i, xyz, box);
+    codes[i] = c;
+    atomicAdd(&hist[c], 1u);
+}
+
+template <int NT>
+__device__ __forceinline__ void morton_scan_block(uint32_t* hist, uint32_t* s_w) {
+    constexpr int U = 4, GROUPS = MORTON_BINS / NT / 4 / U;
+    static_assert(MORTON_BINS % (NT * 4 * U) == 0, "whole groups of U vectors per thread");
+    const int t = threadIdx.x;
+    const unsigned lane = t & 63, w = t >> 6;
+    uint4* h = reinterpret_cast<uint4*>(hist) + (size_t)t * (GROUPS * U);
+    uint32_t s = 0;
+#pragma unroll 1
+    for (int g = 0; g < GROUPS; ++g) {
+        uint4 v[U];
+#pragma unroll
+        for (int u = 0; u < U; ++u) v[u] = h[g * U + u];
+#pragma unroll
+        for (int u = 0; u < U; ++u) s += (v[u].x + v[u].y) + (v[u].z + v[u].w);
+    }
+    const uint32_t incl = gvf_wave_incl_scan(s, lane);
+    if (lane == 63) s_w[w] = incl;
+    __syncthreads();
+    uint32_t run = incl - s;
+    for (unsigned k = 0; k < w; ++k) run += s_w[k];
+#pragma unroll 1
+    for (int g = 0; g < GROUPS; ++g) {
+        uint4 v[U];
+#pragma unroll
+        for (int u = 0; u < U; ++u) v[u] = h[g * U + u];
+#pragma unroll
+        for (int u = 0; u < U; ++u) {
+            uint32_t c = v[u].x; v[u].x = run; run += c;
+            c = v[u].y; v[u].y = run; run += c;
+            c = v[u].z; v[u].z = run; run += c;
+            c = v[u].w; v[u].w = run; run += c;
+            h[g * U + u] = v[u];
+        }
+    }
+}
+
+template <int NT>
+__device__ __forceinline__ void morton_scan_slice(uint32_t* slice, uint32_t* sum, uint32_t* s_w) {
+    static_assert(MORTON_BINS == MORTON_SCAN_SLICES * 2 * NT, "two counters per thread");
+    const int t = threadIdx.x;
+    const unsigned lane = t & 63, w = t >> 6;
+    uint2* h = reinterpret_cast<uint2*>(slice) + t;
+    const uint2 v = *h;
+    const uint32_t s = v.x + v.y, incl = gvf_wave_incl_scan(s, lane);
+    if (lane == 63) s_w[w] = incl;
+    __syncthreads();
+    uint32_t run = incl - s;
+    for (unsigned k = 0; k < w; ++k) run += s_w[k];
+    *h = make_uint2(run, run + v.x);
+    if (t == NT - 1) *sum = run + s;
+}
+
+__device__ __forceinline__ void morton_scatter_one(int i, int P, uint32_t* codes_rank, uint32_t* __restrict__ hist,
+                                                   uint32_t* __restrict__ order, const uint32_t* __restrict__ slice_sums = nullptr) {
+    static_assert(MORTON_SCAN_SLICES <= 64, "one slice total per lane");
+    const uint32_t code = i < P ? codes_rank[i] : 0u;
+    uint32_t base = 0u;
+    if (slice_sums != nullptr) {
+        const unsigned lane = threadIdx.x & 63;
+        const uint32_t tot = lane < (unsigned)MORTON_SCAN_SLICES ? slice_sums[lane] : 0u;
+        const uint32_t excl = gvf_wave_incl_scan(tot, lane) - tot;
+        base = (uint32_t)__shfl((int)excl, (int)(code / (uint32_t)(MORTON_BINS / MORTON_SCAN_SLICES)), 64);
+    }
+    if (i >= P) return;
+    const uint32_t slot = base + atomicAdd(&hist[code], 1u);
+    order[slot] = (uint32_t)i;
+    codes_rank[i] = slot;
+}
+
+__device__ __forceinline__ void bbox_rider(const OrderRiders& rd, uint32_t* s_mm) {
+    bbox_block(rd.P, rd.xyz, (int)blockIdx.x * PRE_THREADS, rd.blocks * PRE_THREADS, s_mm);
+    if (threadIdx.x < 6) rd.boxes[6 * blockIdx.x + threadIdx.x] = s_mm[threadIdx.x];
+}
+__device__ __forceinline__ void morton_count_rider(const OrderRiders& rd) {
+    uint32_t box[6];
+    bbox_from_partials(rd.boxes, rd.nboxes, box);
+    if (blockIdx.x == 0 && threadIdx.x == 0) {
+#pragma unroll
+        for (int k = 0; k < 6; ++k) rd.mm[k] = box[k];
+    }
+    for (int i = (int)blockIdx.x * PRE_THREADS + (int)threadIdx.x; i < rd.P; i += rd.blocks * PRE_THREADS)
+        morton_count_one(i, rd.P, rd.xyz, box, rd.codes, rd.hist);
+}
 
 __global__ __launch_bounds__(256) void activate_kernel(GvfGaussianActivation a, int P, int M,
                                                        const float* __restrict__ xyz_raw,
@@ -129,14 +300,23 @@
     const float* __restrict__ cov3D_precomp, const float* __restrict__ delta, float4* __restrict__ splats,
     uint32_t* __restrict__ tiles_touched,
     int32_t* __restrict__ radii, uint32_t* __restrict__ block_sums, REC* __restrict__ binrec,
-    const uint32_t* __restrict__ bin_slot ) {
+    const uint32_t* __restrict__ bin_slot ,
+    OrderRiders rd ) {
     static_assert(!(SHARED && WAVE_FRAMES), "the shared-activation launch keeps the 256-Gaussian mapping");
     extern __shared__ __attribute__((aligned(16))) float sh_lds[];
     constexpr int PRE_GPB = WAVE_FRAMES ? GVF_WAVE : PRE_THREADS;
+    int bx = blockIdx.x;
+    if (!SHARED) {
+        if (bx < rd.blocks) {
+            if (blockIdx.y == 0) morton_count_rider(rd);
+            return;
+        }
+        bx -= rd.blocks;
+    }
     const int t = threadIdx.x;
     const int P = pp.P, M = pp.M;
     const int nbx = (P + PRE_THREADS - 1) / PRE_THREADS;
-    const int bx = blockIdx.x, by = blockIdx.y;
+    const int by = blockIdx.y;
     const int row = WAVE_FRAMES ? (t & (GVF_WAVE - 1)) : t;
     const int i = bx * PRE_GPB + row;
 
@@ -408,25 +588,24 @@
         }
 }
 
-__device__ __forceinline__ uint32_t float_ordered(float f) {
-    const uint32_t u = __float_as_uint(f);
-    return (u & 0x80000000u) ? ~u : (u | 0x80000000u);
-}
-__device__ __forceinline__ float float_unordered(uint32_t o) {
-    return __uint_as_float((o & 0x80000000u) ? (o & 0x7fffffffu) : ~o);
-}
-
-__global__ __launch_bounds__(1024) void seg_sums_kernel(const uint32_t* __restrict__ cnt, int n, uint32_t* __restrict__ partial) {
+__global__ __launch_bounds__(SCAN_THREADS) void seg_sums_kernel(const uint32_t* __restrict__ cnt, int n, uint32_t* __restrict__ partial,
+                                                                OrderRiders rd) {
     __shared__ uint32_t wsum[16];
-    const int t = threadIdx.x, j0 = blockIdx.x * SCAN_CHUNK + 4 * t;
-    uint32_t s = 0;
-#pragma unroll
-    for (int k = 0; k < 4; ++k) s += j0 + k < n ? cnt[j0 + k] : 0u;
-#pragma unroll
-    for (int d = 32; d >= 1; d >>= 1) s += __shfl_xor(s, d, 64);
-    if ((t & 63) == 0) wsum[t >> 6] = s;
-    __syncthreads();
-    if (t == 0) { uint32_t tot = 0; for (int k = 0; k < 16; ++k) tot += wsum[k]; partial[blockIdx.x] = tot; }
+    const int t = threadIdx.x;
+    if (blockIdx.x >= (uint32_t)rd.blocks) {
+        const uint32_t blk = blockIdx.x - (uint32_t)rd.blocks;
+        const int j0 = blk * SCAN_CHUNK + 4 * t;
+        uint32_t s = 0;
+#pragma unroll
+        for (int k = 0; k < 4; ++k) s += j0 + k < n ? cnt[j0 + k] : 0u;
+#pragma unroll
+        for (int d = 32; d >= 1; d >>= 1) s += __shfl_xor(s, d, 64);
+        if ((t & 63) == 0) wsum[t >> 6] = s;
+        __syncthreads();
+        if (t == 0) { uint32_t tot = 0; for (int k = 0; k < 16; ++k) tot += wsum[k]; partial[blk] = tot; }
+        return;
+    }
+    morton_scatter_one((int)blockIdx.x * SCAN_THREADS + t, rd.P, rd.codes, rd.hist, rd.order, rd.slice_sums);
 }
 
 __global__ __launch_bounds__(1024) void seg_scan_kernel(const uint32_t* __restrict__ cnt, int n, int ntiles, int F,
@@ -597,10 +776,17 @@
                                                                  uint32_t* __restrict__ cursor,
                                                                  const uint32_t* __restrict__ total,
                                                                  uint64_t* __restrict__ payload, int ntiles,
-                                                                 const uint32_t* __restrict__ frame_base, uint32_t* __restrict__ num_rendered) {
+                                                                 const uint32_t* __restrict__ frame_base, uint32_t* __restrict__ num_rendered,
+                                                                 OrderRiders rd ) {
+    static_assert(MORTON_BINS == MORTON_SCAN_SLICES * 2 * BINX_THREADS, "a scan rider takes two counters per thread");
     __shared__ uint32_t s_tab[BINX_TAB];
+    if ((int)blockIdx.x < rd.blocks) {
+        if (blockIdx.y == 0)
+            morton_scan_slice<BINX_THREADS>(rd.hist + (size_t)blockIdx.x * (2 * BINX_THREADS), rd.slice_sums + blockIdx.x, s_tab);
+        return;
+    }
     const int t = threadIdx.x, f = blockIdx.y;
-    const int g0 = (int)blockIdx.x * BINX_PER_WG, g1 = min(P, g0 + BINX_PER_WG);
+    const int g0 = ((int)blockIdx.x - rd.blocks) * BINX_PER_WG, g1 = min(P, g0 + BINX_PER_WG);
     for (int e = t; e < ntiles; e += BINX_THREADS) s_tab[e] = 0u;
     __syncthreads();
     if constexpr (sizeof(REC) == 16) {
@@ -641,87 +827,30 @@
     }
 }
 
-__global__ __launch_bounds__(256) void bbox_kernel(int P, const float* __restrict__ xyz, uint32_t* __restrict__ mm) {
+__global__ __launch_bounds__(PRE_THREADS) void bbox_kernel(int P, const float* __restrict__ xyz, uint32_t* __restrict__ mm) {
     __shared__ uint32_t s_mm[6];
-    if (threadIdx.x < 6) s_mm[threadIdx.x] = threadIdx.x < 3 ? 0xffffffffu : 0u;
-    __syncthreads();
-    uint32_t lo[3] = {0xffffffffu, 0xffffffffu, 0xffffffffu}, hi[3] = {0u, 0u, 0u};
-    for (int i = blockIdx.x * blockDim.x + threadIdx.x; i < P; i += gridDim.x * blockDim.x) {
-#pragma unroll
-        for (int k = 0; k < 3; ++k) {
-            const float v = xyz[3 * (size_t)i + k];
-            if (v == v && fabsf(v) < 3.0e38f) {
-                const uint32_t o = float_ordered(v);
-                lo[k] = min(lo[k], o); hi[k] = max(hi[k], o);
-            }
-        }
-    }
-#pragma unroll
-    for (int k = 0; k < 3; ++k) {
-#pragma unroll
-        for (int d = 32; d >= 1; d >>= 1) {
-            lo[k] = min(lo[k], (uint32_t)__shfl_xor((int)lo[k], d, 64));
-            hi[k] = max(hi[k], (uint32_t)__shfl_xor((int)hi[k], d, 64));
-        }
-        if ((threadIdx.x & 63) == 0) { atomicMin(&s_mm[k], lo[k]); atomicMax(&s_mm[3 + k], hi[k]); }
-    }
-    __syncthreads();
+    bbox_block(P, xyz, (int)(blockIdx.x * blockDim.x), (int)(gridDim.x * blockDim.x), s_mm);
     if (threadIdx.x < 3) atomicMin(&mm[threadIdx.x], s_mm[threadIdx.x]);
     else if (threadIdx.x < 6) atomicMax(&mm[threadIdx.x], s_mm[threadIdx.x]);
 }
 
-__device__ __forceinline__ uint32_t spread5(uint32_t v) {
-    return (v & 1u) | ((v & 2u) << 2) | ((v & 4u) << 4) | ((v & 8u) << 6) | ((v & 16u) << 8);
-}
-
-
-__device__ __forceinline__ uint32_t morton15(int i, const float* __restrict__ xyz, const uint32_t* __restrict__ mm) {
-    uint32_t code = 0;
-#pragma unroll
-    for (int k = 0; k < 3; ++k) {
-        const float lo = float_unordered(mm[k]), hi = float_unordered(mm[3 + k]);
-        const float v = xyz[3 * (size_t)i + k];
-        float q = (v - lo) / fmaxf(hi - lo, 1e-30f) * 32.0f;
-        q = (q == q) ? fminf(fmaxf(q, 0.0f), 31.0f) : 0.0f;
-        code |= spread5((uint32_t)q) << k;
-    }
-    return code;
-}
-
-__global__ __launch_bounds__(256) void morton_count_kernel(int P, const float* __restrict__ xyz,
-                                                           const uint32_t* __restrict__ mm, uint32_t* __restrict__ codes,
-                                                           uint32_t* __restrict__ hist) {
-    const int i = blockIdx.x * blockDim.x + threadIdx.x;
-    if (i >= P) return;
-    const uint32_t c = morton15(i, xyz, mm);
-    codes[i] = c;
-    atomicAdd(&hist[c], 1u);
-}
-
-__global__ __launch_bounds__(1024) void morton_scan_kernel(uint32_t* __restrict__ hist) {
-    __shared__ uint32_t wsum[16];
-    const int t = threadIdx.x;
-    const unsigned lane = t & 63, w = t >> 6;
-    constexpr int PER = MORTON_BINS / 1024;
-    uint32_t v[PER], s = 0;
-#pragma unroll
-    for (int k = 0; k < PER; ++k) { v[k] = hist[t * PER + k]; s += v[k]; }
-    const uint32_t incl = gvf_wave_incl_scan(s, lane);
-    if (lane == 63) wsum[w] = incl;
-    __syncthreads();
-    uint32_t run = incl - s;
-    for (unsigned k = 0; k < w; ++k) run += wsum[k];
-#pragma unroll
-    for (int k = 0; k < PER; ++k) { hist[t * PER + k] = run; run += v[k]; }
-}
-
-__global__ __launch_bounds__(256) void morton_scatter_kernel(int P, uint32_t* codes_rank, uint32_t* __restrict__ hist,
-                                                             uint32_t* __restrict__ order) {
-    const int i = blockIdx.x * blockDim.x + threadIdx.x;
-    if (i >= P) return;
-    const uint32_t slot = atomicAdd(&hist[codes_rank[i]], 1u);
-    order[slot] = (uint32_t)i;
-    codes_rank[i] = slot;
+__global__ __launch_bounds__(PRE_THREADS) void morton_count_kernel(int P, const float* __restrict__ xyz,
+                                                                   const uint32_t* __restrict__ mm, uint32_t* __restrict__ codes,
+                                                                   uint32_t* __restrict__ hist) {
+    uint32_t box[6];
+#pragma unroll
+    for (int k = 0; k < 6; ++k) box[k] = mm[k];
+    morton_count_one((int)(blockIdx.x * blockDim.x + threadIdx.x), P, xyz, box, codes, hist);
+}
+
+__global__ __launch_bounds__(SCAN_THREADS) void morton_scan_kernel(uint32_t* __restrict__ hist) {
+    __shared__ uint32_t wsum[SCAN_THREADS / 64];
+    morton_scan_block<SCAN_THREADS>(hist, wsum);
+}
+
+__global__ __launch_bounds__(PRE_THREADS) void morton_scatter_kernel(int P, uint32_t* codes_rank, uint32_t* __restrict__ hist,
+                                                                     uint32_t* __restrict__ order) {
+    morton_scatter_one((int)(blockIdx.x * blockDim.x + threadIdx.x), P, codes_rank, hist, order);
 }
 
 __global__ __launch_bounds__(256) void ranges_kernel(const uint64_t* __restrict__ keys,
@@ -750,8 +879,15 @@
     uint32_t* mm;
     uint32_t layout;
 };
-__global__ void upload_frames_kernel(FrameChunk c, int count, GvfRastFrame* __restrict__ dst, CallTables tab) {
-    if (blockIdx.x == 0) {
+__global__ __launch_bounds__(PRE_THREADS) void upload_frames_kernel(FrameChunk c, int count, GvfRastFrame* __restrict__ dst, CallTables tab,
+                                                                    OrderRiders rd) {
+    __shared__ uint32_t s_mm[6];
+    if ((int)blockIdx.x < rd.blocks) {
+        bbox_rider(rd, s_mm);
+        return;
+    }
+    const uint32_t blk = blockIdx.x - (uint32_t)rd.blocks, nblk = gridDim.x - (uint32_t)rd.blocks;
+    if (blk == 0) {
         const int words = (int)(sizeof(GvfRastFrame) / 4) * count;
         const uint32_t* src = reinterpret_cast<const uint32_t*>(&c);
         for (int k = threadIdx.x; k < words; k += blockDim.x) reinterpret_cast<uint32_t*>(dst)[k] = src[k];
@@ -760,7 +896,7 @@
         if (tab.mm != nullptr && threadIdx.x == LAYOUT_WORD) tab.mm[LAYOUT_WORD] = tab.layout;
         return;
     }
-    const uint32_t t = (blockIdx.x - 1) * blockDim.x + threadIdx.x, nt = (gridDim.x - 1) * blockDim.x;
+    const uint32_t t = (blk - 1) * blockDim.x + threadIdx.x, nt = (nblk - 1) * blockDim.x;
     for (uint32_t k = t; k < tab.n_ranges; k += nt) tab.ranges[k] = 0u;
     for (uint32_t k = t; k < tab.n_tile_count; k += nt) tab.tile_count[k] = 0u;
     for (uint32_t k = t; k < tab.n_mhist; k += nt) tab.mhist[k] = 0u;
@@ -787,18 +923,29 @@
     uint4* binrec = nullptr;
     const uint32_t* bin_slot = nullptr;
 };
+OrderRiders order_riders(const RastCall& c, const RastPlan& plan, const Workspace& w, int blocks) {
+    OrderRiders rd = {};
+    if (blocks <= 0) return rd;
+    rd.blocks = blocks; rd.P = c.P; rd.nboxes = plan.bbox_riders;
+    rd.xyz = c.a0; rd.boxes = w.tiles_touched; rd.slice_sums = w.tiles_touched + 6 * MORTON_BOX_BLOCKS;
+    rd.mm = w.mm; rd.codes = w.order_alt; rd.hist = w.mhist; rd.order = w.order;
+    return rd;
+}
+
 template <bool SHARED, bool WAVE_FRAMES = false>
-void launch_preprocess(hipStream_t stream, const RastPlan& plan, const PreParams& pp, const Workspace& w, const PreArgs& a) {
+void launch_preprocess(hipStream_t stream, const RastPlan& plan, const PreParams& pp, const Workspace& w, const PreArgs& a,
+                       const OrderRiders& rd = OrderRiders{}) {
     const int32_t* g = WAVE_FRAMES ? plan.wf_grid : plan.pre_grid;
     const size_t lds = (size_t)(WAVE_FRAMES ? plan.wf_lds_bytes : plan.pre_lds_bytes);
+    const dim3 grid(g[0] + rd.blocks, g[1]);
     if (plan.rec8)
-        hipLaunchKernelGGL((preprocess_kernel<SHARED, WAVE_FRAMES, BinRec8>), dim3(g[0], g[1]), dim3(PRE_THREADS), lds, stream, pp, w.frames,
+        hipLaunchKernelGGL((preprocess_kernel<SHARED, WAVE_FRAMES, BinRec8>), grid, dim3(PRE_THREADS), lds, stream, pp, w.frames,
                            a.a0, a.a1, a.a2, a.a3, a.sh, a.colors_precomp, a.cov3D_precomp, a.delta, w.splats, a.tiles_touched, a.radii,
-                           a.block_sums, reinterpret_cast<BinRec8*>(a.binrec), a.bin_slot);
+                           a.block_sums, reinterpret_cast<BinRec8*>(a.binrec), a.bin_slot, rd);
     else
-        hipLaunchKernelGGL((preprocess_kernel<SHARED, WAVE_FRAMES, BinRec16>), dim3(g[0], g[1]), dim3(PRE_THREADS), lds, stream, pp, w.frames,
+        hipLaunchKernelGGL((preprocess_kernel<SHARED, WAVE_FRAMES, BinRec16>), grid, dim3(PRE_THREADS), lds, stream, pp, w.frames,
                            a.a0, a.a1, a.a2, a.a3, a.sh, a.colors_precomp, a.cov3D_precomp, a.delta, w.splats, a.tiles_touched, a.radii,
-                           a.block_sums, a.binrec, a.bin_slot);
+                           a.block_sums, a.binrec, a.bin_slot, rd);
 }
 
 template <typename REC>
@@ -806,8 +953,9 @@
     const REC* rec = reinterpret_cast<const REC*>(w.binrec);
     const int gather = plan.rec_gather ? 1 : 0;
     if (plan.index_count)
-        hipLaunchKernelGGL((bin_index_kernel<REC>), dim3(plan.binx_grid[0], plan.binx_grid[1]), dim3(BINX_THREADS), 0, stream, c.P, plan.gx, rec,
-                           w.tile_count, w.cursor, w.total, w.keys, plan.ntiles, nullptr, nullptr);
+        hipLaunchKernelGGL((bin_index_kernel<REC>), dim3(plan.binx_grid[0] + plan.scan_riders, plan.binx_grid[1]), dim3(BINX_THREADS), 0, stream,
+                           c.P, plan.gx, rec, w.tile_count, w.cursor, w.total, w.keys, plan.ntiles, nullptr, nullptr,
+                           order_riders(c, plan, w, plan.scan_riders));
     else
         hipLaunchKernelGGL((bin_kernel<false, REC>), dim3(plan.bin_grid[0], plan.bin_grid[1]), dim3(PRE_THREADS), 0, stream, c.P, plan.gx, plan.gy,
                            rec, order, w.tile_count, w.cursor, w.total, w.keys, nullptr, nullptr, gather, gather, c.F);
@@ -832,7 +980,7 @@
     const int pb = (c.P + 255) / 256;
     hipLaunchKernelGGL(bbox_kernel, dim3(bb), dim3(256), 0, stream, c.P, c.a0, w.mm);
     hipLaunchKernelGGL(morton_count_kernel, dim3(pb), dim3(256), 0, stream, c.P, c.a0, w.mm, w.order_alt, w.mhist);
-    hipLaunchKernelGGL(morton_scan_kernel, dim3(1), dim3(1024), 0, stream, w.mhist);
+    hipLaunchKernelGGL(morton_scan_kernel, dim3(1), dim3(SCAN_THREADS), 0, stream, w.mhist);
     hipLaunchKernelGGL(morton_scatter_kernel, dim3(pb), dim3(256), 0, stream, c.P, w.order_alt, w.mhist, w.order);
 }
 
@@ -885,7 +1033,9 @@
             tab.mhist = w.mhist; tab.n_mhist = plan.morton ? (uint32_t)MORTON_BINS : 0u;
             tab.cls = w.cls; tab.mm = w.mm; tab.layout = (uint32_t)plan.layout;
         }
-        hipLaunchKernelGGL(upload_frames_kernel, dim3(1 + (f0 == 0 ? plan.clear_blocks : 0)), dim3(256), 0, stream, ch, cnt, w.frames + f0, tab);
+        const OrderRiders rd = order_riders(c, plan, w, f0 == 0 ? plan.bbox_riders : 0);
+        hipLaunchKernelGGL(upload_frames_kernel, dim3(rd.blocks + 1 + (f0 == 0 ? plan.clear_blocks : 0)), dim3(PRE_THREADS), 0, stream, ch, cnt,
+                           w.frames + f0, tab, rd);
     }
     GVF_CHECK_LAUNCH();
     return GVF_OK;
@@ -894,10 +1044,9 @@
 int gvf_rast::front_end_bucket(hipStream_t stream, const RastCall& c, const RastPlan& plan, const Workspace& w, const hipEvent_t* marks) {
     const int P = c.P, F = c.F;
     prof_mark(stream, marks, 0);
-    const uint32_t* order = nullptr;
-    if (plan.morton) {
+    const uint32_t* order = plan.morton ? w.order : nullptr;
+    if (plan.morton && !plan.order_riders) {
         launch_morton_order(stream, c, w);
-        order = w.order;
         GVF_CHECK_LAUNCH();
     }
     prof_mark(stream, marks, 1);
@@ -908,15 +1057,17 @@
         PreArgs a = input_args(c);
         a.radii = c.out_radii == nullptr ? nullptr : w.radii;
         a.binrec = w.binrec;
-        if (plan.wave_frames) launch_preprocess<false, true>(stream, plan, pp, w, a);
-        else launch_preprocess<false>(stream, plan, pp, w, a);
+        const OrderRiders rd = order_riders(c, plan, w, plan.code_riders);
+        if (plan.wave_frames) launch_preprocess<false, true>(stream, plan, pp, w, a, rd);
+        else launch_preprocess<false>(stream, plan, pp, w, a, rd);
     }
     if (plan.rec8) launch_bin_count<BinRec8>(stream, c, plan, w, order);
     else launch_bin_count<BinRec16>(stream, c, plan, w, order);
     GVF_CHECK_LAUNCH();
     prof_mark(stream, marks, 2);
-    hipLaunchKernelGGL(seg_sums_kernel, dim3(plan.scan_blocks), dim3(1024), 0, stream, w.tile_count, plan.nseg, w.partial);
-    hipLaunchKernelGGL(seg_scan_kernel, dim3(plan.scan_blocks), dim3(1024), 0, stream, w.tile_count, plan.nseg, plan.ntiles, F,
+    hipLaunchKernelGGL(seg_sums_kernel, dim3(plan.scan_blocks + plan.scatter_riders), dim3(SCAN_THREADS), 0, stream, w.tile_count, plan.nseg,
+                       w.partial, order_riders(c, plan, w, plan.scatter_riders));
+    hipLaunchKernelGGL(seg_scan_kernel, dim3(plan.scan_blocks), dim3(SCAN_THREADS), 0, stream, w.tile_count, plan.nseg, plan.ntiles, F,
                        w.partial, plan.scan_blocks, w.ranges, w.cursor, w.frame_base, c.out_num_rendered, w.total,
                        (uint32_t)c.max_rendered, w.cls);
     if (c.max_rendered <= 0)
diff --git a/gvfdiffusion_amd/csrc/rast_plan.h b/gvfdiffusion_amd/csrc/rast_plan.h
--- a/gvfdiffusion_amd/csrc/rast_plan.h
+++ b/gvfdiffusion_amd/csrc/rast_plan.h
@@ -26,6 +26,9 @@
 constexpr int BINX_PER_WG = 8192;
 constexpr int BIN_REC8_MAX_GRID = 255;
 constexpr int MORTON_BINS = 1 << 15;
+constexpr int MORTON_BOX_BLOCKS = 128;
+constexpr int MORTON_SCAN_SLICES = 32;
+constexpr int SCAN_THREADS = 1024;
 constexpr int ORDER_TILES_MIN_SEGS = 2048;
 
 constexpr int LAYOUT_WORD = 6;
@@ -69,6 +72,7 @@
     bool pre_wave_frames = true;
     bool blend_order = true;
     bool bin_rec8 = true;
+    bool order_riders = true;
 };
 
 struct PlanInputs {
@@ -81,6 +85,8 @@
     int32_t di[ACT_MAX_SLICES];
     std::vector<int32_t> frame_slice;
     bool rec8;
+    bool order_riders, tile_order_rider;
+    int32_t bbox_riders, code_riders, scan_riders, scatter_riders;
 };
 
 inline int ceil_div(int a, int b) { return (a + b - 1) / b; }
@@ -115,6 +121,12 @@
     p.wave_frames = !p.shared && p.bucket && sw.pre_wave_frames;
     p.rec8 = p.bucket && sw.bin_rec8 && p.gx <= BIN_REC8_MAX_GRID && p.gy <= BIN_REC8_MAX_GRID;
     p.order_tiles = sw.blend_order && P > 0 && p.nb > 0 && in.max_rendered > 0 && (size_t)F * p.ntiles >= (size_t)ORDER_TILES_MIN_SEGS;
+    p.order_riders = sw.order_riders && in.fused && p.morton && p.rec_gather && p.index_count;
+    p.tile_order_rider = sw.order_riders && p.order_tiles && p.bucket;
+    p.bbox_riders = p.order_riders ? (p.nb < MORTON_BOX_BLOCKS ? p.nb : MORTON_BOX_BLOCKS) : 0;
+    p.code_riders = p.bbox_riders;
+    p.scan_riders = p.order_riders ? MORTON_SCAN_SLICES : 0;
+    p.scatter_riders = p.order_riders ? ceil_div(P, SCAN_THREADS) : 0;
 
     p.pre_grid[0] = p.nb; p.pre_grid[1] = ceil_div(F, PRE_FB);
     p.wf_grid[0] = ceil_div(P, WAVE); p.wf_grid[1] = ceil_div(F, PRE_WAVES * PRE_WAVE_FB);
diff --git a/gvfdiffusion_amd/csrc/rast_sort.hip b/gvfdiffusion_amd/csrc/rast_sort.hip
--- a/gvfdiffusion_amd/csrc/rast_sort.hip
+++ b/gvfdiffusion_amd/csrc/rast_sort.hip
@@ -236,11 +236,17 @@
 template <int MODE>
 __global__ __launch_bounds__(MODE == 3 ? 512 : 1024, MODE == 3 ? 2 : 1) void tile_sort_kernel(const uint2* __restrict__ ranges, uint64_t* __restrict__ keys,
                                  const uint32_t* __restrict__ vals, uint32_t* __restrict__ ids,
-                                 const uint32_t* __restrict__ cls, uint32_t nseg, uint32_t split = 0u ) {
+                                 const uint32_t* __restrict__ cls, uint32_t nseg, uint32_t split = 0u ,
+                                 uint32_t* __restrict__ tile_order = nullptr , int ntiles = 0) {
     __shared__ uint64_t s_small[MODE == 0 ? SORT_SMALL_N : 1];
     __shared__ uint32_t s_hist[MODE == 0 ? SORT_SMALL_N + 1 + BKT_AUX : (MODE == 1 || MODE == 3 ? BKT_LARGE_NB + 1 + BKT_AUX : 1)];
     extern __shared__ __attribute__((aligned(16))) uint64_t s_large[];
     if (MODE == 0) {
+        if (blockIdx.x >= nseg) {
+            const size_t f = blockIdx.x - nseg;
+            blend_order_block<256>(ranges + f * ntiles, ntiles, tile_order + f * ntiles, s_hist);
+            return;
+        }
         const uint2 rng = ranges[blockIdx.x];
         const int n = (int)(rng.y - rng.x);
         if (n <= 0 || n > SORT_SMALL_N) return;
@@ -337,11 +343,13 @@
 }
 
 int gvf_rast::launch_tile_sort(hipStream_t stream, const uint2* ranges, uint64_t* keys, const uint32_t* vals, uint32_t* ids, uint32_t* cls,
-                               uint32_t nseg, int cls_state) {
+                               uint32_t nseg, int cls_state, uint32_t* tile_order, int ntiles, int F) {
+    if (tile_order != nullptr && (ntiles <= 0 || F <= 0 || (uint64_t)F * (uint64_t)ntiles != (uint64_t)nseg)) return GVF_EINVAL;
     if (cls_state == 0 && hipMemsetAsync(cls, 0, 2 * sizeof(uint32_t), stream) != hipSuccess) return GVF_ELAUNCH;
     if (cls_state < 2)
         hipLaunchKernelGGL(classify_kernel, dim3((nseg + 255) / 256), dim3(256), 0, stream, ranges, nseg, cls);
-    hipLaunchKernelGGL(tile_sort_kernel<0>, dim3(nseg), dim3(256), 0, stream, ranges, keys, vals, ids, cls, nseg);
+    hipLaunchKernelGGL(tile_sort_kernel<0>, dim3(nseg + (tile_order != nullptr ? (uint32_t)F : 0u)), dim3(256), 0, stream, ranges, keys, vals, ids,
+                       cls, nseg, 0u, tile_order, ntiles);
     if (tile_sort_set_lds_limit() != GVF_OK) return GVF_ELAUNCH;
     hipLaunchKernelGGL(tile_sort_kernel<3>, dim3(SORT_MEDIUM_BLOCKS), dim3(512), SORT_MEDIUM_N * 8, stream, ranges, keys, vals, ids, cls,
                        nseg, 0u);
diff --git a/gvfdiffusion_amd/rasterizer.py b/gvfdiffusion_amd/rasterizer.py
--- a/gvfdiffusion_amd/rasterizer.py
+++ b/gvfdiffusion_amd/rasterizer.py
@@ -391,6 +391,30 @@
     return int(out.value)
 
 
+def order_riders(settings, frames, P, M, max_rendered, fused=True, has_sh=True, has_colors_precomp=False, has_cov3D_precomp=False,
+                 has_delta=True, has_subpixel_offset=False):
+    F = len(frames)
+    arr = frames if isinstance(frames, ctypes.Array) else (_lib.GvfRastFrame * F)(*frames)
+    out = ctypes.c_int(0)
+    _lib.check(_lib.lib().gvf_rast_order_riders(ctypes.byref(settings), arr, F, int(P), int(M), int(fused), int(has_sh),
+                                                int(has_colors_precomp), int(has_cov3D_precomp), int(has_delta), int(has_subpixel_offset),
+                                                int(max_rendered), ctypes.byref(out)), "gvf_rast_order_riders")
+    return bool(out.value)
+
+
+def morton_order(device=None):
+    import numpy as np
+    device = torch.device("cuda", torch.cuda.current_device()) if device is None else torch.device(device)
+    key = (device.index if device.index is not None else torch.cuda.current_device(), int(torch.cuda.current_stream(device).cuda_stream))
+    if key not in _LAST_CARVE:
+        raise _lib.GvfError("no batched rasteriser call on this stream yet")
+    _ws, base, nbytes, P, F, H, W, cap = _LAST_CARVE[key]
+    out = (ctypes.c_uint32 * P)()
+    _lib.check(_lib.lib().gvf_rast_morton_order(ctypes.c_void_p(base), nbytes, P, F, H, W, cap, out, _lib.current_stream(device)),
+               "gvf_rast_morton_order")
+    return np.frombuffer(out, dtype=np.uint32).astype(np.int64)
+
+
 def gaussian_activate(act, xyz_raw, features_dc, scaling_raw, rotation_raw, opacity_raw, delta=None):
     _lib.require_cuda(xyz_raw)
     dev = xyz_raw.device
diff --git a/include/gvf_rast.h b/include/gvf_rast.h
--- a/include/gvf_rast.h
+++ b/include/gvf_rast.h
@@ -149,6 +149,13 @@
 
 int gvf_rast_bin_record_bytes(const GvfRastSettings* settings_host, int* bytes);
 
+int gvf_rast_order_riders(const GvfRastSettings* settings_host, const GvfRastFrame* frames_host, int F, int P, int M, int fused,
+                          int has_sh, int has_colors_precomp, int has_cov3D_precomp, int has_delta, int has_subpixel_offset,
+                          int64_t max_rendered, int* riding);
+
+int gvf_rast_morton_order(const void* workspace, size_t workspace_bytes, int P, int F, int H, int W, int64_t max_rendered,
+                          uint32_t* order_host , void* stream);
+
 int gvf_rast_slice_groups(const GvfRastFrame* frames_host, int F, int has_delta, int max_slices, int32_t* table_host, int* n_slices);
 
 const char* gvf_version(void);
```

New measurement: 22260 frames/s. Within noise of the previous version (-0.0%).
